# oceanbase/oceanbase

Hardware: AMD Instinct MI355X
Metric: rows/sec, TPC-H lineitem scan->filter->agg (microblock decode + pushdown filter + group-by) (higher is better)
Workload: dtype int64; 1 GPU; tpch_q1_sf100_lineitem_scan_filter_agg; rows_per_gpu=600000000, total_rows=600000000, encoded_bytes_per_gpu=7341603792, n_blocks=453858, block_bytes=16384

## Files before the change

### include/obx.h

```cpp
#ifndef OBX_H_
#define OBX_H_

#include <stdint.h>
#include <stddef.h>

#ifdef __cplusplus
extern "C" {
#endif

enum {
  OBX_SUCCESS = 0,
  OBX_ITER_END = -4008,
  OBX_INVALID_ARGUMENT = -4002,
  OBX_NOT_SUPPORTED = -4007,
  OBX_BUF_NOT_ENOUGH = -4009,
  OBX_NO_GPU = -7001,
  OBX_INTERNAL_ERROR = -4016,
  OBX_PHYSIC_CHECKSUM_ERROR = -4108,
};

enum obx_encoding {
  OBX_ENC_RAW = 0,
  OBX_ENC_DICT = 1,
  OBX_ENC_RLE = 2,
  OBX_ENC_CONST = 3,
  OBX_ENC_INTEGER_BASE_DIFF = 4,
  OBX_ENC_STRING_DIFF = 5,
  OBX_ENC_HEX_PACKING = 6,
  OBX_ENC_STRING_PREFIX = 7,
  OBX_ENC_COLUMN_EQUAL = 8,
  OBX_ENC_COLUMN_SUBSTR = 9,
  OBX_ENC_MAX = 10,
  OBX_ENC_AUTO = 255,
};

enum obx_obj_type {
  OBX_T_INT = 5,
  OBX_T_INT32 = 4,
  OBX_T_DATE = 19,
  OBX_T_CHAR = 23,
  OBX_T_DECIMAL_INT = 50,
};

enum obx_white_op {
  OBX_OP_EQ = 0,
  OBX_OP_LE = 1,
  OBX_OP_LT = 2,
  OBX_OP_GE = 3,
  OBX_OP_GT = 4,
  OBX_OP_NE = 5,
  OBX_OP_BT = 6,
  OBX_OP_IN = 7,
  OBX_OP_NU = 8,
  OBX_OP_NN = 9,
  OBX_OP_BLACK = 10,
  OBX_OP_IN_SET = 11,
};

#define OBX_BX_MAX_PROG 24
#define OBX_BX_MAX_CONST 4
#define OBX_BX_MAX_COLS 4

enum obx_agg_kind {
  OBX_AGG_COUNT = 0,
  OBX_AGG_SUM = 1,
  OBX_AGG_MIN = 2,
  OBX_AGG_MAX = 3,
  OBX_AGG_SUM_PROD2 = 4,
  OBX_AGG_SUM_PROD3 = 5,
  OBX_AGG_SUM_MUL = 6,
};

typedef struct obx_col_schema {
  uint8_t obj_type;
  int8_t scale;
  uint8_t precision;
  uint8_t len;
} obx_col_schema;

typedef struct obx_blockset {
  const uint8_t *data;
  const uint64_t *block_offsets;
  uint32_t n_blocks;
  uint16_t n_cols;
  const obx_col_schema *cols;
  uint64_t total_rows;
} obx_blockset;

#define OBX_MAX_IN_LIST 8
typedef struct obx_filter_leaf {
  uint16_t col;
  uint8_t op;
  uint8_t n_in;
  int64_t lo;
  int64_t hi;
  int64_t in_list[OBX_MAX_IN_LIST];
  int64_t bconst[OBX_BX_MAX_CONST];
  uint16_t bcols[OBX_BX_MAX_COLS];
  uint8_t n_bprog;
  uint8_t n_bcols;
  uint8_t bprog[OBX_BX_MAX_PROG];
  uint8_t bpad[6];
} obx_filter_leaf;

#define OBX_TOK_AND 128
#define OBX_TOK_OR 129
#define OBX_MAX_PROG 15

typedef struct obx_filter_desc {
  uint16_t n_leaves;
  uint8_t n_prog;
  uint8_t prog[OBX_MAX_PROG];
  obx_filter_leaf leaves[8];
} obx_filter_desc;

typedef struct obx_agg_expr {
  uint8_t kind;
  uint16_t col_a;
  uint16_t col_b;
  uint16_t col_c;
} obx_agg_expr;

typedef struct obx_agg_desc {
  uint8_t n_group_cols;
  uint16_t group_cols[2];
  uint8_t n_aggs;
  obx_agg_expr aggs[8];
} obx_agg_desc;

typedef struct obx_agg_cell { uint64_t limb[4]; } obx_agg_cell;

#define OBX_MAX_GROUPS 64
#define OBX_MAX_KEY_BYTES 16
typedef struct obx_group_row {
  uint8_t key[OBX_MAX_KEY_BYTES];
  uint8_t key_len;
  uint64_t row_count;
  obx_agg_cell cells[8];
} obx_group_row;

typedef struct obx_agg_result {
  uint32_t n_groups;
  obx_group_row groups[OBX_MAX_GROUPS];
  uint64_t rows_scanned;
  uint64_t rows_passed;
} obx_agg_result;

typedef struct obx_batch {
  uint64_t *skip_bits;
  int64_t size;
  uint8_t end;
  uint8_t all_rows_active;
} obx_batch;


int64_t obx_encode_block(const obx_col_schema *cols, uint16_t n_cols,
                         const uint8_t *const *col_data,
                         const uint8_t *const *null_bitmaps,
                         uint32_t row_count, const uint8_t *enc_request,
                         uint8_t *out, int64_t out_cap);

uint64_t obx_crc32c(const uint8_t *buf, int64_t len);

int obx_decode_block(const obx_col_schema *cols, uint16_t n_cols,
                     const uint8_t *block, int64_t block_len,
                     const uint16_t *proj_cols, uint16_t n_proj,
                     uint8_t *const *out_cols, uint8_t *const *out_nulls,
                     uint32_t *row_count);

int obx_cpu_filter_block(const obx_col_schema *cols, uint16_t n_cols,
                         const uint8_t *block, int64_t block_len,
                         const obx_filter_desc *filter,
                         uint8_t *result_bits, uint32_t *row_count,
                         uint32_t *popcnt);

int obx_cpu_scan_filter_agg(const obx_blockset *bs,
                            const obx_filter_desc *filter,
                            const obx_agg_desc *agg,
                            int nthreads,
                            obx_agg_result *out);

int64_t obx_gen_lineitem(int config, uint64_t row_count, uint64_t seed,
                         uint32_t target_block_bytes,
                         uint64_t row_id_base,
                         uint8_t **out_data, uint64_t **out_offsets,
                         obx_col_schema *out_cols, uint16_t *out_n_cols);

typedef struct obx_gpu_ctx obx_gpu_ctx;

int obx_gpu_open(int device, obx_gpu_ctx **ctx);
int obx_gpu_close(obx_gpu_ctx *ctx);

int obx_gpu_load_blocks(obx_gpu_ctx *ctx, const obx_blockset *bs);

int obx_gpu_load_cs_blocks(obx_gpu_ctx *ctx, const obx_blockset *bs);

int obx_cs_host_parse(const uint8_t *buf, int64_t len, uint32_t *rows_out,
                      uint32_t *ncols_out);
int obx_gpu_free_blocks(obx_gpu_ctx *ctx, int handle);

int obx_gpu_filter(obx_gpu_ctx *ctx, int handle, const obx_filter_desc *filter,
                   int want_row_ids);
int obx_gpu_fetch_bitmap(obx_gpu_ctx *ctx, int handle, uint8_t *out, int64_t cap);
int obx_gpu_fetch_row_ids(obx_gpu_ctx *ctx, int handle, int32_t *out,
                          int64_t cap, uint64_t *n_out);
int obx_gpu_fetch_blk_counts(obx_gpu_ctx *ctx, int handle, uint32_t *out,
                             int64_t cap);

int obx_gpu_decode(obx_gpu_ctx *ctx, int handle, const uint16_t *proj_cols,
                   uint16_t n_proj);
int obx_gpu_fetch_col(obx_gpu_ctx *ctx, int handle, uint16_t col,
                      uint8_t *out, int64_t cap);

int obx_gpu_scan_project(obx_gpu_ctx *ctx, int handle,
                         const obx_filter_desc *filter,
                         const uint16_t *proj_cols, uint16_t n_proj,
                         int want_row_nos, uint64_t *n_rows);

int obx_gpu_fetch_proj(obx_gpu_ctx *ctx, int handle, uint16_t proj_idx,
                       uint64_t start, uint64_t count,
                       uint8_t *out, int64_t cap,
                       uint8_t *out_nulls, int64_t nulls_cap, uint64_t *n_out);

int obx_gpu_fetch_proj_row_nos(obx_gpu_ctx *ctx, int handle, uint64_t start,
                               uint64_t count, uint64_t *out, int64_t cap,
                               uint64_t *n_out);

double obx_gpu_last_proj_stage_ms(obx_gpu_ctx *ctx, int stage);

int obx_gpu_scan_filter_agg(obx_gpu_ctx *ctx, int handle,
                            const obx_filter_desc *filter,
                            const obx_agg_desc *agg,
                            obx_agg_result *out);

double obx_gpu_last_kernel_ms(obx_gpu_ctx *ctx);
double obx_gpu_last_prep_ms(obx_gpu_ctx *ctx);
int obx_gpu_last_jit(obx_gpu_ctx *ctx);
int obx_gpu_last_bdesc(obx_gpu_ctx *ctx);
int64_t obx_gpu_bdesc_builds(obx_gpu_ctx *ctx, int handle);
uint32_t obx_gpu_last_grid(obx_gpu_ctx *ctx);
uint64_t obx_gpu_total_rows(obx_gpu_ctx *ctx, int handle);
uint64_t obx_gpu_total_bytes(obx_gpu_ctx *ctx, int handle);
uint64_t obx_gpu_last_survivors(obx_gpu_ctx *ctx, int handle);

int obx_gpu_agg_fetch(obx_gpu_ctx *ctx, int handle, uint32_t start,
                      uint32_t count, obx_group_row *out, uint32_t *n_out,
                      uint64_t *n_total);
int obx_cpu_agg_fetch(uint32_t start, uint32_t count, obx_group_row *out,
                      uint32_t *n_out, uint64_t *n_total);

typedef struct obx_keyset_info {
  uint64_t n_keys_in;
  uint64_t n_distinct;
  uint64_t slots_or_bits;
  uint64_t bytes;
  int64_t min, max;
  uint8_t kind;
} obx_keyset_info;

int obx_gpu_keyset_create(obx_gpu_ctx *ctx, const int64_t *keys, uint64_t n,
                          int kind);
int obx_gpu_keyset_from_proj(obx_gpu_ctx *ctx, int handle, uint16_t proj_idx,
                             int kind);
int obx_gpu_keyset_free(obx_gpu_ctx *ctx, int set_id);
int obx_gpu_keyset_info(obx_gpu_ctx *ctx, int set_id, obx_keyset_info *out);
int obx_gpu_keyset_host_model(const int64_t *keys, uint64_t n, int kind,
                              const int64_t *probe, uint64_t m, uint8_t *hit,
                              obx_keyset_info *info);

#define OBX_COL_JOINED 0xFFF0u
typedef struct obx_keymap_info {
  uint64_t n_keys;
  uint64_t slots_or_span;
  uint64_t bytes;
  int64_t min, max;
  uint8_t kind;
  uint8_t payload_len, payload_type;
} obx_keymap_info;

int obx_gpu_keymap_create(obx_gpu_ctx *ctx, const int64_t *keys,
                          const uint8_t *payloads, uint64_t n,
                          const obx_col_schema *payload, int kind);
int obx_gpu_keymap_from_proj(obx_gpu_ctx *ctx, int handle, uint16_t key_idx,
                             uint16_t payload_idx, int kind);
int obx_gpu_keymap_free(obx_gpu_ctx *ctx, int map_id);
int obx_gpu_keymap_info(obx_gpu_ctx *ctx, int map_id, obx_keymap_info *out);
int obx_gpu_keymap_host_model(const int64_t *keys, const uint8_t *payloads,
                              uint64_t n, const obx_col_schema *payload,
                              int kind, const int64_t *probe, uint64_t m,
                              uint8_t *hit, uint64_t *out_payload,
                              obx_keymap_info *info);

typedef struct obx_join_desc { int32_t map_id; uint16_t probe_col; uint16_t pad; } obx_join_desc;
int obx_gpu_scan_join_agg(obx_gpu_ctx *ctx, int handle,
                          const obx_filter_desc *filter,
                          const obx_join_desc *join, const obx_agg_desc *agg,
                          obx_agg_result *out);

int64_t obx_jit_dump_src(const obx_filter_desc *filter,
                         const obx_agg_desc *agg,
                         const obx_col_schema *cols, uint16_t n_cols,
                         const uint8_t *col_flags, const int64_t *col_min,
                         const int64_t *col_max, const uint32_t *col_maxcnt,
                         const uint32_t *col_maxw, uint32_t max_block_rows,
                         int force_v1, char *out, int64_t cap);

#ifdef __cplusplus
}
#endif
#endif
```

### oceanbase_amd/csrc/obx_engine.cpp

```cpp
#include <cstdlib>
#include <cstring>
#include <algorithm>

#include "obx_host.h"

#define OBX_RESULT_BYTES(slots) (sizeof(gslot) * (slots) + 16 * 8)

extern "C" int obx_gpu_open(int device, obx_gpu_ctx **out) {
  int n = 0;
  hipError_t e = hipGetDeviceCount(&n);
  if (e != hipSuccess || n <= device) return OBX_NO_GPU;
  auto *ctx = new obx_gpu_ctx();
  ctx->device = device;
  HIP_TRY(hipSetDevice(device));
  HIP_TRY(hipStreamCreate(&ctx->stream));
  HIP_TRY(hipEventCreate(&ctx->ev_start));
  HIP_TRY(hipEventCreate(&ctx->ev_stop));
  HIP_TRY(hipEventCreate(&ctx->ev_p0));
  HIP_TRY(hipEventCreate(&ctx->ev_p1));
  HIP_TRY(hipEventCreate(&ctx->ev_mid));
  HIP_TRY(hipEventCreate(&ctx->ev_b0));
  HIP_TRY(hipEventCreate(&ctx->ev_b1));
  {
    hipDeviceProp_t prop;
    HIP_TRY(hipGetDeviceProperties(&prop, device));
    if (prop.multiProcessorCount > 0)
      ctx->n_cus = (uint32_t)prop.multiProcessorCount;
  }
  HIP_TRY(hipHostMalloc((void **)&ctx->h_result,
                        OBX_RESULT_BYTES(OBX_GTABLE_BIG), hipHostMallocDefault));
  *out = ctx;
  return OBX_SUCCESS;
}

extern "C" int obx_gpu_close(obx_gpu_ctx *ctx) {
  if (!ctx) return OBX_SUCCESS;
  (void)hipSetDevice(ctx->device);
  ctx->handles.clear();
  ctx->keysets.clear();
  ctx->keymaps.clear();
  (void)hipStreamDestroy(ctx->stream);
  for (hipEvent_t ev : {ctx->ev_start, ctx->ev_stop, ctx->ev_p0, ctx->ev_p1,
                        ctx->ev_mid, ctx->ev_b0, ctx->ev_b1})
    (void)hipEventDestroy(ev);
  (void)hipHostFree(ctx->h_result);
  delete ctx;
  return OBX_SUCCESS;
}

obx_handle::~obx_handle() {
  void *owned[] = {d_buf, d_blocks, d_bleaves, d_pleaves, d_gtable,
                   d_gtable_big, d_proj_scratch, d_bitmap, d_row_ids,
                   d_blk_counts, d_row_slot, d_minmax, d_sel_nulls,
                   d_sel_row_nos, d_blk_off, d_tile_sums, d_sel_bits};
  for (void *p : owned)
    if (p) (void)hipFree(p);
  for (uint8_t *p : d_decode_out)
    if (p) (void)hipFree(p);
  for (uint8_t *p : d_sel_out)
    if (p) (void)hipFree(p);
  for (bdesc_set &s : bdesc)
    if (s.d) (void)hipFree(s.d);
}

obx_handle *obx_handle_lookup(obx_gpu_ctx *ctx, int handle) {
  if (!ctx || handle < 0 || handle >= (int)ctx->handles.size()) return nullptr;
  return ctx->handles[handle].get();
}

__attribute__((target("sse4.2")))
static uint64_t host_crc32c(const uint8_t *buf, int64_t len) {
  uint64_t crc = 0;
  int64_t i = 0;
  for (; i + 8 <= len; i += 8) {
    uint64_t w;
    memcpy(&w, buf + i, 8);
    crc = __builtin_ia32_crc32di(crc, w);
  }
  for (; i < len; i++) crc = __builtin_ia32_crc32qi((uint32_t)crc, buf[i]);
  return crc;
}

#define OBX_JIT_GRID_WAVES 8
static uint32_t jit_grid_for(uint32_t n_blocks, uint32_t n_cus, int wpb) {
  uint64_t g = (uint64_t)(n_cus ? n_cus : 1) * (uint32_t)(wpb > 0 ? wpb : 1) *
               OBX_JIT_GRID_WAVES;
  if (const char *sg = getenv("OBX_JIT_SGRID")) {
    const long v = atol(sg);
    if (v >= 1 && (uint64_t)v < g) g = (uint64_t)v;
  }
  if (g > n_blocks) g = n_blocks;
  return g ? (uint32_t)g : 1;
}

static void gtable_init(gslot *gt, uint32_t n_slots, uint32_t tail_words,
                        uint32_t min_mask, uint32_t max_mask,
                        hipStream_t stream) {
  const uint32_t words =
      n_slots * (uint32_t)(sizeof(gslot) / 8) + tail_words;
  hipLaunchKernelGGL(k_gtable_init, dim3((words + OBX_WG_HOST - 1) / OBX_WG_HOST),
                     dim3(OBX_WG_HOST), 0, stream, (unsigned long long *)gt,
                     n_slots, tail_words, min_mask, max_mask);
}

static void summarize_col_classes(obx_handle &h) {
  const uint32_t nc = h.n_cols;
  const bool first = h.col_class.size() == nc;
  const uint8_t *cls = h.col_class.data() + h.col_class.size() - nc;
  const uint8_t *cnt = h.col_cnt.data() + h.col_cnt.size() - nc;
  for (uint32_t c = 0; c < nc; c++) {
    const uint8_t k = cls[c];
    if (first) h.col_grp16_every[c] = true;
    if ((k & 0xF) == 5) h.col_span_any[c] = true;
    if ((k & 0xF) != 1 || cnt[c] >= 16) h.col_grp16_every[c] = false;
    if ((k & 0xF) > 3 || (k & 0x10)) h.col_slow_any[c] = true;
    if (cnt[c] > h.col_cnt_max[c]) h.col_cnt_max[c] = cnt[c];
  }
}

void obx_fold_block(obx_handle &h, const dev_block &db) {
  const bool first = h.col_class.empty();
  if ((db.block_byte & 15) ||
      (uint64_t)db.block_len + 24 > OBX_LDS_STAGE_BYTES ||
      db.row_count > 4096 )
    h.lds_ok = false;
  for (uint16_t c = 0; c < h.n_cols; c++) {
    const dev_col &dc = db.cols[c];
    uint8_t cls;
    switch (dc.enc) {
      case OBX_D_RAW: cls = 0; break;
      case OBX_D_DICT: cls = 1; break;
      case OBX_D_INTDIFF: cls = 2; break;
      case OBX_D_CONST: cls = dc.runs == 0 ? 3 : 4; break;
      case OBX_D_EQUAL: case OBX_D_SUBSTR:
        cls = 5; break;
      default: cls = 4; break;
    }
    if (dc.flags & OBX_DF_STRING) cls |= 0x10;
    h.col_class.push_back(cls);
    h.col_cnt.push_back((uint8_t)(dc.count > 254 ? 255 : dc.count));
    if (first) {
      h.col_dict_every[c] = true;
      h.col_dict_any[c] = true;
      h.col_raw8_every[c] = true;
      h.col_rangefam_every[c] = true;
    }
    if ((cls & 0xF) != 1 || (cls & 0x10) || dc.count > 63)
      h.col_dict_every[c] = false;
    if ((cls & 0xF) != 1 || dc.count > 63)
      h.col_dict_any[c] = false;
    if (!(dc.enc == OBX_D_RAW && !(dc.flags & OBX_DF_BITPACK) &&
          !(dc.flags & OBX_DF_STRING) && !(dc.flags & OBX_DF_HAS_EXT) &&
          dc.width == 8 && (dc.data_bit & 63) == 0))
      h.col_raw8_every[c] = false;
    if (!((dc.enc == OBX_D_RAW || dc.enc == OBX_D_INTDIFF) &&
          !(dc.flags & OBX_DF_STRING) && !(dc.flags & OBX_DF_HAS_EXT)))
      h.col_rangefam_every[c] = false;
    if (dc.count > h.col_maxcnt[c]) h.col_maxcnt[c] = dc.count;
    if (dc.flags & OBX_DF_HAS_EXT) h.col_ext_any[c] = true;
    uint32_t w = 255;
    if (dc.enc == OBX_D_RAW || dc.enc == OBX_D_DICT || dc.enc == OBX_D_INTDIFF)
      w = (dc.flags & OBX_DF_BITPACK) ? dc.width : (uint32_t)dc.width * 8;
    if (w > h.col_maxw[c]) h.col_maxw[c] = w;
    uint64_t slot;
    if (!obx_bdesc_pack_col(&dc, db.block_byte, &slot))
      h.col_bdesc_unfit[c] = true;
  }
  summarize_col_classes(h);
  if (db.row_count > h.max_block_rows) h.max_block_rows = db.row_count;
  if (db.block_len > h.max_block_len) h.max_block_len = db.block_len;
  h.n_blocks++;
  h.total_rows += db.row_count;
}

static int parse_block(const obx_col_schema *cols, uint16_t n_cols,
                       const uint8_t *block, uint64_t dev_off,
                       uint64_t block_len, uint64_t row_start,
                       dev_block *out) {
  const obx_micro_header *h = (const obx_micro_header *)block;
  if (h->magic != OBX_MICRO_BLOCK_MAGIC) return OBX_INVALID_ARGUMENT;
  if (h->column_count != n_cols) return OBX_INVALID_ARGUMENT;
  if (h->data_zlength > (int64_t)block_len ||
      h->data_zlength < OBX_MICRO_HEADER_SIZE)
    return OBX_INVALID_ARGUMENT;
  if ((int64_t)host_crc32c(block + OBX_MICRO_HEADER_SIZE,
                           (int64_t)h->data_zlength - OBX_MICRO_HEADER_SIZE) !=
      h->data_checksum)
    return OBX_PHYSIC_CHECKSUM_ERROR;
  memset(out, 0, sizeof(*out));
  out->row_start_lo = (uint32_t)row_start;
  out->row_start_hi = (uint32_t)(row_start >> 32);
  out->row_count = h->row_count;
  out->block_len = (uint32_t)block_len;
  out->block_byte = dev_off;
  const uint64_t meta_base =
      dev_off + h->header_size + (uint64_t)n_cols * sizeof(obx_col_header);
  const obx_col_header *chp =
      (const obx_col_header *)(block + h->header_size);
  const uint8_t *meta_host = block + h->header_size +
                             (uint64_t)n_cols * sizeof(obx_col_header);
  const uint8_t evb = obx_hdr_extend_value_bit(h);

  for (uint16_t c = 0; c < n_cols; c++) {
    const obx_col_header *ch = &chp[c];
    dev_col *dc = &out->cols[c];
    const int sc = obx_store_class(ch->obj_type);
    const int64_t tss = obx_type_store_size(ch->obj_type);
    dc->enc = (uint8_t)ch->type;
    dc->datum_len = cols[c].len;
    dc->tss = (uint8_t)(tss > 0 ? tss : cols[c].len);
    dc->ext_width = evb;
    if (sc == OBX_SC_INT) dc->flags |= OBX_DF_SIGNED;
    if (sc == OBX_SC_STRING) dc->flags |= OBX_DF_STRING;
    const uint64_t col_base = meta_base + ch->offset;
    const uint8_t *col_host = meta_host + ch->offset;
    const int has_ext = (ch->attr & OBX_COL_ATTR_HAS_EXTEND_VALUE) ? 1 : 0;
    const int bp = (ch->attr & OBX_COL_ATTR_BIT_PACKING) ? 1 : 0;

    switch (ch->type) {
      case OBX_COL_RAW: {
        if (bp) dc->flags |= OBX_DF_BITPACK;
        dc->width = (uint8_t)ch->length;
        uint64_t ext_bits = has_ext ? (uint64_t)evb * h->row_count : 0;
        if (has_ext) {
          dc->flags |= OBX_DF_HAS_EXT;
          dc->ext_bit = col_base * 8;
        }
        if (bp) {
          dc->data_bit = col_base * 8 + ext_bits;
        } else {
          dc->data_bit = (col_base + (ext_bits + 7) / 8) * 8;
        }
        break;
      }
      case OBX_COL_DICT: {
        const obx_dict_meta *dm = (const obx_dict_meta *)col_host;
        if (bp) dc->flags |= OBX_DF_BITPACK;
        dc->width = dm->row_ref_size;
        dc->count = dm->count;
        dc->entry_len = (uint8_t)dm->data_size;
        dc->dict_byte = col_base + sizeof(obx_dict_meta);
        dc->data_bit = (col_base + ch->length) * 8;
        break;
      }
      case OBX_COL_RLE: {
        const obx_rle_meta *rm = (const obx_rle_meta *)col_host;
        dc->runs = rm->count;
        dc->rib = rm->attr & 7;
        dc->rfb = (rm->attr >> 3) & 7;
        dc->aux_byte = col_base + sizeof(obx_rle_meta);
        const obx_dict_meta *dm =
            (const obx_dict_meta *)(col_host + rm->offset);
        dc->count = dm->count;
        dc->entry_len = (uint8_t)dm->data_size;
        dc->dict_byte = col_base + rm->offset + sizeof(obx_dict_meta);
        break;
      }
      case OBX_COL_CONST: {
        const obx_const_meta *cm = (const obx_const_meta *)col_host;
        dc->runs = cm->count;
        dc->rib = cm->attr & 7;
        dc->rfb = cm->const_ref;
        if (cm->count == 0) {
          if (cm->const_ref > 0) {
            dc->count = 0;
          } else {
            dc->count = 1;
            int64_t cell = (sc == OBX_SC_INT) ? tss : cols[c].len;
            uint64_t v = 0;
            memcpy(&v, col_host + cm->offset, (size_t)cell);
            dc->base = (sc == OBX_SC_INT)
                           ? (int64_t)obx_sign_extend(v, tss, 1)
                           : (sc == OBX_SC_DECIMAL
                                  ? (int64_t)obx_sign_extend(v, cell, 1)
                                  : (int64_t)v);
          }
        } else {
          dc->aux_byte = col_base + sizeof(obx_const_meta);
          const obx_dict_meta *dm =
              (const obx_dict_meta *)(col_host + cm->offset);
          dc->count = dm->count;
          dc->entry_len = (uint8_t)dm->data_size;
          dc->dict_byte = col_base + cm->offset + sizeof(obx_dict_meta);
        }
        break;
      }
      case OBX_COL_INTEGER_BASE_DIFF: {
        const obx_intdiff_meta *im = (const obx_intdiff_meta *)col_host;
        if (bp) dc->flags |= OBX_DF_BITPACK;
        dc->width = im->length;
        uint64_t b = 0;
        memcpy(&b, col_host + sizeof(obx_intdiff_meta), (size_t)tss);
        dc->base = (int64_t)obx_sign_extend(b, tss, sc == OBX_SC_INT);
        uint64_t data0 = col_base + ch->length;
        uint64_t ext_bits = has_ext ? (uint64_t)evb * h->row_count : 0;
        if (has_ext) {
          dc->flags |= OBX_DF_HAS_EXT;
          dc->ext_bit = data0 * 8;
        }
        if (bp) dc->data_bit = data0 * 8 + ext_bits;
        else dc->data_bit = (data0 + (ext_bits + 7) / 8) * 8;
        break;
      }
      case OBX_COL_STRING_PREFIX: {
        const obx_sprefix_meta *pm = (const obx_sprefix_meta *)col_host;
        dc->count = pm->count;
        dc->entry_len = pm->hex_char_cnt;
        dc->rib = pm->pib;
        dc->dict_byte = col_base + sizeof(obx_sprefix_meta);
        dc->aux_byte = dc->dict_byte + pm->hex_char_cnt;
        {
          const uint8_t *ends = col_host + sizeof(obx_sprefix_meta) +
                                pm->hex_char_cnt;
          uint64_t prev = 0, min_pl = ~0ull;
          for (uint32_t j = 0; j < pm->count; j++) {
            uint64_t e2 = 0;
            memcpy(&e2, ends + (size_t)j * pm->pib, pm->pib);
            if (e2 - prev < min_pl) min_pl = e2 - prev;
            prev = e2;
          }
          uint32_t max_suffix = pm->string_size - (uint32_t)min_pl;
          dc->width = (uint8_t)(1 + (pm->hex_char_cnt
                                         ? (max_suffix + 1) / 2
                                         : max_suffix));
        }
        uint64_t data0 = col_base + ch->length;
        uint64_t ext_bits = has_ext ? (uint64_t)evb * h->row_count : 0;
        if (has_ext) {
          dc->flags |= OBX_DF_HAS_EXT;
          dc->ext_bit = data0 * 8;
        }
        dc->data_bit = (data0 + (ext_bits + 7) / 8) * 8;
        break;
      }
      case OBX_COL_SUBSTR: {
        const obx_substr_meta *sm3 = (const obx_substr_meta *)col_host;
        if (sm3->ref_col >= n_cols) return OBX_INVALID_ARGUMENT;
        dc->runs = sm3->exc_cnt;
        dc->rib = sm3->rib;
        dc->width = (uint8_t)sm3->ref_col;
        dc->base = sm3->start_pos;
        dc->dict_byte = col_base + sizeof(obx_substr_meta);
        dc->aux_byte = dc->dict_byte + (uint64_t)sm3->exc_cnt * sm3->rib;
        break;
      }
      case OBX_COL_EQUAL: {
        const obx_coleq_meta *em = (const obx_coleq_meta *)col_host;
        if (em->ref_col >= n_cols) return OBX_INVALID_ARGUMENT;
        dc->runs = em->exc_cnt;
        dc->rib = em->rib;
        dc->width = (uint8_t)em->ref_col;
        dc->dict_byte = col_base + sizeof(obx_coleq_meta);
        dc->aux_byte = dc->dict_byte + (uint64_t)em->exc_cnt * em->rib;
        break;
      }
      case OBX_COL_HEX_PACKING: {
        const obx_hex_meta *hm = (const obx_hex_meta *)col_host;
        dc->width = (uint8_t)((hm->string_size + 1) / 2);
        dc->count = hm->char_cnt;
        dc->dict_byte = col_base + sizeof(obx_hex_meta);
        uint64_t data0 = col_base + ch->length;
        uint64_t ext_bits = has_ext ? (uint64_t)evb * h->row_count : 0;
        if (has_ext) {
          dc->flags |= OBX_DF_HAS_EXT;
          dc->ext_bit = data0 * 8;
        }
        dc->data_bit = (data0 + (ext_bits + 7) / 8) * 8;
        break;
      }
      case OBX_COL_STRING_DIFF: {
        const obx_sdiff_meta *sm = (const obx_sdiff_meta *)col_host;
        dc->runs = sm->diff_desc_cnt;
        dc->entry_len = sm->hex_char_cnt;
        dc->dict_byte = col_base + sizeof(obx_sdiff_meta);
        const uint8_t *descs = col_host + sizeof(obx_sdiff_meta);
        uint32_t diff_len = 0;
        for (uint32_t i = 0; i < sm->diff_desc_cnt; i++)
          if (descs[i] & 1) diff_len += descs[i] >> 1;
        dc->rib = (uint8_t)diff_len;
        dc->width = (uint8_t)(sm->hex_char_cnt ? (diff_len + 1) / 2
                                               : diff_len);
        dc->aux_byte = dc->dict_byte + sm->diff_desc_cnt +
                       sm->hex_char_cnt;
        uint64_t data0 = col_base + ch->length;
        uint64_t ext_bits = has_ext ? (uint64_t)evb * h->row_count : 0;
        if (has_ext) {
          dc->flags |= OBX_DF_HAS_EXT;
          dc->ext_bit = data0 * 8;
        }
        dc->data_bit = (data0 + (ext_bits + 7) / 8) * 8;
        break;
      }
      default:
        return OBX_NOT_SUPPORTED;
    }
// ... 521 lines not shown
      ln[i] = (uint8_t)h.cols[c].len;
      po[i] = h.d_decode_out[c];
    }
    if (!h.d_proj_scratch)
      HIP_TRY(hipMalloc(&h.d_proj_scratch,
                        OBX_DEV_MAX_COLS * (8 + 2 + 1) + 16));
    uint8_t *base = (uint8_t *)h.d_proj_scratch;
    uint8_t *outp = base;
    uint8_t *pcp = base + OBX_DEV_MAX_COLS * 8;
    uint8_t *lnp = pcp + OBX_DEV_MAX_COLS * 2;
    HIP_TRY(hipMemcpy(outp, po, sizeof(void *) * n_proj,
                      hipMemcpyHostToDevice));
    HIP_TRY(hipMemcpy(pcp, pc, sizeof(uint16_t) * n_proj,
                      hipMemcpyHostToDevice));
    HIP_TRY(hipMemcpy(lnp, ln, n_proj, hipMemcpyHostToDevice));
    hipLaunchKernelGGL(k_decode_multi, dim3(grid_for(h.n_blocks)),
                       dim3(OBX_WG_HOST), 0, ctx->stream, h.d_buf,
                       h.d_blocks, h.n_blocks, (const uint16_t *)pcp,
                       lnp, (uint32_t)n_proj, (uint8_t *const *)outp,
                       (uint8_t *const *)nullptr);
  } else {
    for (uint16_t i = 0; i < n_proj; i++) {
      uint16_t c = proj_cols[i];
      if (c >= h.n_cols) return OBX_INVALID_ARGUMENT;
      if (!h.d_decode_out[c])
        HIP_TRY(hipMalloc(&h.d_decode_out[c], h.total_rows * h.cols[c].len));
      auto kfn = h.lds_ok ? k_decode_lds : k_decode;
      hipLaunchKernelGGL(kfn, dim3(grid_for(h.n_blocks)), dim3(OBX_WG_HOST), 0,
                         ctx->stream, h.d_buf, h.d_blocks, h.n_blocks,
                         (uint32_t)c, (uint32_t)h.cols[c].len,
                         h.d_decode_out[c], (uint8_t *)nullptr);
    }
  }
  return end_timed(ctx, false);
}

extern "C" int obx_gpu_fetch_col(obx_gpu_ctx *ctx, int handle, uint16_t col,
                                 uint8_t *out, int64_t cap) {
  obx_handle *hp = obx_handle_lookup(ctx, handle);
  if (!hp) return OBX_INVALID_ARGUMENT;
  obx_handle &h = *hp;
  if (col >= h.n_cols || !h.d_decode_out[col]) return OBX_INVALID_ARGUMENT;
  int64_t bytes = (int64_t)h.total_rows * h.cols[col].len;
  if (cap < bytes) return OBX_BUF_NOT_ENOUGH;
  HIP_TRY(hipMemcpy(out, h.d_decode_out[col], bytes, hipMemcpyDeviceToHost));
  return OBX_SUCCESS;
}

template <class T>
static int grow(T *&p, uint64_t &cap, uint64_t need, size_t unit) {
  if (need <= cap) return OBX_SUCCESS;
  (void)hipFree(p);
  p = nullptr;
  cap = 0;
  HIP_TRY(hipMalloc(&p, need * unit));
  cap = need;
  return OBX_SUCCESS;
}

extern "C" int obx_gpu_scan_project(obx_gpu_ctx *ctx, int handle,
                                    const obx_filter_desc *filter,
                                    const uint16_t *proj_cols, uint16_t n_proj,
                                    int want_row_nos, uint64_t *n_rows) {
  obx_handle *hp = obx_handle_lookup(ctx, handle);
  if (!hp) return OBX_INVALID_ARGUMENT;
  obx_handle &h = *hp;
  h.sel_n_proj = 0;
  if (!proj_cols || n_proj == 0 || n_proj > OBX_DEV_MAX_COLS)
    return OBX_INVALID_ARGUMENT;
  for (uint16_t i = 0; i < n_proj; i++)
    if (proj_cols[i] >= h.n_cols) return OBX_INVALID_ARGUMENT;
  HIP_TRY(hipSetDevice(ctx->device));

  const bool filtered = filter && filter->n_leaves;
  uint64_t total = h.total_rows;
  ctx->last_proj_ms[0] = ctx->last_proj_ms[1] = ctx->last_proj_ms[2] = 0.0;
  if (filtered) {
    int rc = run_filter(ctx, h, filter, 1);
    if (rc != OBX_SUCCESS) return rc;
    ctx->last_proj_ms[0] = ctx->last_ms;
    total = h.last_survivors;
  } else {
    ctx->last_jit = 0;
  }

  if (total > 0) {
    proj_args pa;
    memset(&pa, 0, sizeof(pa));
    pa.n_proj = n_proj;
    for (uint16_t i = 0; i < n_proj; i++) {
      const uint16_t c = proj_cols[i];
      int rc = grow(h.d_sel_out[i], h.sel_out_cap[i], total * h.cols[c].len, 1);
      if (rc != OBX_SUCCESS) return rc;
      pa.out[i] = h.d_sel_out[i];
      pa.col[i] = c;
      pa.len[i] = h.cols[c].len;
    }
    int rc = grow(h.d_sel_nulls, h.sel_nulls_cap, total, 1);
    if (rc != OBX_SUCCESS) return rc;
    if (want_row_nos) {
      rc = grow(h.d_sel_row_nos, h.sel_row_nos_cap, total, sizeof(uint64_t));
      if (rc != OBX_SUCCESS) return rc;
    }
    const uint32_t n_tiles = (h.n_blocks + OBX_PROJ_TILE - 1) / OBX_PROJ_TILE;
    if (filtered && !h.d_blk_off) {
      HIP_TRY(hipMalloc(&h.d_blk_off, ((uint64_t)h.n_blocks + 1) * 8));
      HIP_TRY(hipMalloc(&h.d_tile_sums, (uint64_t)n_tiles * 8));
    }

    HIP_TRY(hipEventRecord(ctx->ev_start, ctx->stream));
    if (filtered) {
      hipLaunchKernelGGL(k_project_tile_sums, dim3(n_tiles), dim3(OBX_WG_HOST),
                         0, ctx->stream, h.d_blk_counts, h.n_blocks,
                         h.d_tile_sums);
      hipLaunchKernelGGL(k_project_offsets, dim3(n_tiles), dim3(OBX_WG_HOST),
                         0, ctx->stream, h.d_blk_counts, h.n_blocks,
                         h.d_tile_sums, h.d_blk_off);
    }
    HIP_TRY(hipEventRecord(ctx->ev_mid, ctx->stream));
    hipLaunchKernelGGL(h.lds_ok ? k_project_sel_lds : k_project_sel,
                       dim3(grid_for(h.n_blocks)), dim3(OBX_WG_HOST), 0,
                       ctx->stream, h.d_buf, h.d_blocks, h.n_blocks,
                       filtered ? h.d_row_ids : (const int32_t *)nullptr,
                       filtered ? h.d_blk_counts : (const uint32_t *)nullptr,
                       filtered ? h.d_blk_off : (const uint64_t *)nullptr, pa,
                       h.d_sel_nulls,
                       want_row_nos ? h.d_sel_row_nos : (uint64_t *)nullptr,
                       total);
    rc = end_timed(ctx, false);
    if (rc != OBX_SUCCESS) return rc;
    float ms = 0;
    HIP_TRY(hipEventElapsedTime(&ms, ctx->ev_start, ctx->ev_mid));
    ctx->last_proj_ms[1] = ms;
    HIP_TRY(hipEventElapsedTime(&ms, ctx->ev_mid, ctx->ev_stop));
    ctx->last_proj_ms[2] = ms;
  }
  ctx->last_ms = ctx->last_proj_ms[0] + ctx->last_proj_ms[1] +
                 ctx->last_proj_ms[2];

  memcpy(h.sel_cols, proj_cols, sizeof(uint16_t) * n_proj);
  h.sel_has_row_nos = want_row_nos != 0;
  h.sel_rows = total;
  h.sel_n_proj = n_proj;
  if (n_rows) *n_rows = total;
  return OBX_SUCCESS;
}

static uint64_t sel_window(const obx_handle &h, uint64_t start,
                           uint64_t count) {
  if (start >= h.sel_rows) return 0;
  return count < h.sel_rows - start ? count : h.sel_rows - start;
}

extern "C" int obx_gpu_fetch_proj(obx_gpu_ctx *ctx, int handle,
                                  uint16_t proj_idx, uint64_t start,
                                  uint64_t count, uint8_t *out, int64_t cap,
                                  uint8_t *out_nulls, int64_t nulls_cap,
                                  uint64_t *n_out) {
  obx_handle *hp = obx_handle_lookup(ctx, handle);
  if (!hp) return OBX_INVALID_ARGUMENT;
  obx_handle &h = *hp;
  if (proj_idx >= h.sel_n_proj) return OBX_INVALID_ARGUMENT;
  const uint64_t n = sel_window(h, start, count);
  if (n_out) *n_out = n;
  if (n == 0) return OBX_SUCCESS;
  const uint64_t len = h.cols[h.sel_cols[proj_idx]].len;
  const uint64_t null_bytes = (n + 7) / 8;
  if (out && (cap < 0 || (uint64_t)cap < n * len)) return OBX_BUF_NOT_ENOUGH;
  if (out_nulls && (nulls_cap < 0 || (uint64_t)nulls_cap < null_bytes))
    return OBX_BUF_NOT_ENOUGH;
  HIP_TRY(hipSetDevice(ctx->device));
  if (out)
    HIP_TRY(hipMemcpyAsync(out, h.d_sel_out[proj_idx] + start * len, n * len,
                           hipMemcpyDeviceToHost, ctx->stream));
  if (out_nulls) {
    int rc = grow(h.d_sel_bits, h.sel_bits_cap, null_bytes, 1);
    if (rc != OBX_SUCCESS) return rc;
    uint64_t g = (null_bytes + OBX_WG_HOST - 1) / OBX_WG_HOST;
    if (g > 4096) g = 4096;
    hipLaunchKernelGGL(k_project_pack_nulls, dim3((uint32_t)g),
                       dim3(OBX_WG_HOST), 0, ctx->stream, h.d_sel_nulls,
                       start, n, (uint32_t)proj_idx, h.d_sel_bits);
    HIP_TRY(hipMemcpyAsync(out_nulls, h.d_sel_bits, null_bytes,
                           hipMemcpyDeviceToHost, ctx->stream));
  }
  HIP_TRY(hipStreamSynchronize(ctx->stream));
  return OBX_SUCCESS;
}

extern "C" int obx_gpu_fetch_proj_row_nos(obx_gpu_ctx *ctx, int handle,
                                          uint64_t start, uint64_t count,
                                          uint64_t *out, int64_t cap,
                                          uint64_t *n_out) {
  obx_handle *hp = obx_handle_lookup(ctx, handle);
  if (!hp) return OBX_INVALID_ARGUMENT;
  obx_handle &h = *hp;
  if (!h.sel_n_proj || !h.sel_has_row_nos) return OBX_INVALID_ARGUMENT;
  const uint64_t n = sel_window(h, start, count);
  if (n_out) *n_out = n;
  if (n == 0 || !out) return OBX_SUCCESS;
  if (cap < 0 || (uint64_t)cap < n) return OBX_BUF_NOT_ENOUGH;
  HIP_TRY(hipSetDevice(ctx->device));
  HIP_TRY(hipMemcpyAsync(out, h.d_sel_row_nos + start, n * sizeof(uint64_t),
                         hipMemcpyDeviceToHost, ctx->stream));
  HIP_TRY(hipStreamSynchronize(ctx->stream));
  return OBX_SUCCESS;
}

extern "C" double obx_gpu_last_proj_stage_ms(obx_gpu_ctx *ctx, int stage) {
  return ctx && stage >= 0 && stage < 3 ? ctx->last_proj_ms[stage] : -1.0;
}

static int table_to_rows(obx_handle &h, const gslot *gt, size_t n_gt,
                         const unsigned long long *cnt, uint8_t key_len,
                         const obx_agg_desc *agg, obx_agg_result *out) {
  unsigned long long passed = cnt[0];
  for (int i2 = 8; i2 < 16; i2++) passed += cnt[i2];

  memset(out, 0, sizeof(*out));
  out->rows_scanned = h.total_rows;
  out->rows_passed = passed;
  std::vector<const gslot *> live;
  for (size_t i = 0; i < n_gt; i++)
    if (gt[i].key != OBX_KEY_EMPTY) live.push_back(&gt[i]);
  std::sort(live.begin(), live.end(), [](const gslot *a, const gslot *b) {
    uint8_t ka[8], kb[8];
    memcpy(ka, &a->key, 8);
    memcpy(kb, &b->key, 8);
    return memcmp(ka, kb, 8) < 0;
  });
  h.last_rows.assign(live.size(), obx_group_row());
  for (size_t i = 0; i < live.size(); i++) {
    obx_group_row *g = &h.last_rows[i];
    memcpy(g->key, &live[i]->key, 8);
    g->key_len = key_len;
    g->row_count = live[i]->count;
    uint32_t na = agg ? agg->n_aggs : 0;
    for (uint32_t a = 0; a < na; a++) {
      uint8_t kind = agg->aggs[a].kind;
      if (kind == OBX_AGG_COUNT && agg->aggs[a].col_a == UINT16_MAX) {
        g->cells[a].limb[0] = live[i]->count;
        g->cells[a].limb[1] = g->cells[a].limb[2] = g->cells[a].limb[3] = 0;
      } else if (kind == OBX_AGG_MIN || kind == OBX_AGG_MAX) {
        int64_t v = live[i]->cells[a][1] ? (int64_t)live[i]->cells[a][0] : 0;
        g->cells[a].limb[0] = (uint64_t)v;
        uint64_t s = v < 0 ? ~0ull : 0ull;
        g->cells[a].limb[1] = g->cells[a].limb[2] = g->cells[a].limb[3] = s;
      } else {
        for (int l = 0; l < 4; l++)
          g->cells[a].limb[l] = live[i]->cells[a][l];
      }
    }
  }
  if (h.last_rows.size() > OBX_MAX_GROUPS) {
    out->n_groups = (uint32_t)h.last_rows.size();
    return OBX_BUF_NOT_ENOUGH;
  }
  out->n_groups = (uint32_t)h.last_rows.size();
  for (size_t i = 0; i < h.last_rows.size(); i++)
    out->groups[i] = h.last_rows[i];
  return OBX_SUCCESS;
}

template <class LAUNCH>
static int rerun_direct(obx_gpu_ctx *ctx, obx_handle &h,
                        const dev_plan_hdr &ph, uint32_t min_mask,
                        uint32_t max_mask, size_t *n_gt,
                        unsigned long long cnt[16], LAUNCH launch) {
  if (ph.n_prog != 0) return OBX_BUF_NOT_ENOUGH;
  if (!h.d_gtable_big)
    HIP_TRY(hipMalloc(&h.d_gtable_big, OBX_RESULT_BYTES(OBX_GTABLE_BIG)));
  unsigned long long *big_counters =
      (unsigned long long *)(h.d_gtable_big + OBX_GTABLE_BIG);
  gtable_init(h.d_gtable_big, OBX_GTABLE_BIG, 16, min_mask, max_mask,
              ctx->stream);
  launch(h.d_gtable_big, big_counters);
  HIP_TRY(hipMemcpyAsync(ctx->h_result, h.d_gtable_big,
                         OBX_RESULT_BYTES(OBX_GTABLE_BIG),
                         hipMemcpyDeviceToHost, ctx->stream));
  HIP_TRY(hipStreamSynchronize(ctx->stream));
  *n_gt = OBX_GTABLE_BIG;
  memcpy(cnt, (const gslot *)ctx->h_result + OBX_GTABLE_BIG,
         16 * sizeof(cnt[0]));
  if (cnt[2] != 0) return OBX_BUF_NOT_ENOUGH;
  return OBX_SUCCESS;
}


struct minmax_masks { uint32_t min = 0, max = 0; };
template <class KIND_OF>
static minmax_masks agg_minmax_masks(uint32_t n_aggs, KIND_OF kind_of) {
  minmax_masks m;
  for (uint32_t a = 0; a < n_aggs; a++) {
    if (kind_of(a) == OBX_AGG_MIN) m.min |= 1u << a;
    else if (kind_of(a) == OBX_AGG_MAX) m.max |= 1u << a;
  }
  return m;
}

static void reset_last_scan(obx_gpu_ctx *ctx) {
  ctx->last_jit = 0;
  ctx->last_grid = 0;
  ctx->last_bdesc = 0;
  ctx->bdesc_built = false;
}

template <class LAUNCH>
static int finish_agg_scan(obx_gpu_ctx *ctx, obx_handle &h,
                           const dev_plan_hdr &ph, minmax_masks mm,
                           uint8_t key_len, const obx_agg_desc *agg,
                           obx_agg_result *out, LAUNCH launch_direct) {
  int rc = end_timed(ctx, true, h.d_gtable,
                     OBX_RESULT_BYTES(OBX_GTABLE_SLOTS));
  if (rc != OBX_SUCCESS) return rc;
  const gslot *gt = (const gslot *)ctx->h_result;
  size_t n_gt = OBX_GTABLE_SLOTS;
  unsigned long long cnt[16];
  memcpy(cnt, gt + OBX_GTABLE_SLOTS, sizeof(cnt));
  if (cnt[1] != 0) {
    rc = rerun_direct(ctx, h, ph, mm.min, mm.max, &n_gt, cnt, launch_direct);
    if (rc != OBX_SUCCESS) return rc;
  }
  return table_to_rows(h, gt, n_gt, cnt, key_len, agg, out);
}

extern "C" int obx_gpu_scan_filter_agg(obx_gpu_ctx *ctx, int handle,
                                       const obx_filter_desc *filter,
                                       const obx_agg_desc *agg,
                                       obx_agg_result *out) {
  obx_handle *hp = obx_handle_lookup(ctx, handle);
  if (!hp || !out) return OBX_INVALID_ARGUMENT;
  obx_handle &h = *hp;
  HIP_TRY(hipSetDevice(ctx->device));
  h.last_rows.clear();
  dev_plan_hdr ph;
  dev_leaf plv[OBX_DEV_MAX_LEAVES];
  int rc = prep_query(ctx, h, filter, agg, ph, plv);
  if (rc != OBX_SUCCESS) return rc;
  reset_last_scan(ctx);

  const minmax_masks mm = agg_minmax_masks(
      ph.n_aggs, [&](uint32_t a) { return ph.aggs[a].kind; });
  gtable_init(h.d_gtable, OBX_GTABLE_SLOTS, 16, mm.min, mm.max, ctx->stream);

  const bool use_pipeline = getenv("OBX_PIPELINE_AGG") != nullptr;
  if (use_pipeline) {
    uint64_t bm_words = (h.total_rows + 63) / 64 + 1;
    if (!h.d_bitmap) HIP_TRY(hipMalloc(&h.d_bitmap, bm_words * 8));
    HIP_TRY(hipMemsetAsync(h.d_bitmap, 0, bm_words * 8, ctx->stream));
    if (!h.d_row_slot) HIP_TRY(hipMalloc(&h.d_row_slot, h.total_rows + 1));

    HIP_TRY(hipEventRecord(ctx->ev_start, ctx->stream));
    hipLaunchKernelGGL(generic_filter_kernel(h, ph),
                       dim3(grid_for(h.n_blocks)), dim3(OBX_WG_HOST), 0,
                       ctx->stream, h.d_buf, h.d_blocks, h.n_blocks,
                       h.d_pleaves, h.d_bleaves, ph, h.d_bitmap,
                       (int32_t *)nullptr, (uint32_t *)nullptr, h.d_counters);
    hipLaunchKernelGGL(k_group_pass, dim3(grid_for(h.n_blocks)),
                       dim3(OBX_WG_HOST), 0, ctx->stream, h.d_buf, h.d_blocks,
                       h.n_blocks, ph, h.d_bitmap, h.d_row_slot, h.d_gtable,
                       h.d_counters);
    for (uint32_t a = 0; a < ph.n_aggs;) {
      const dev_agg &ag = ph.aggs[a];
      if (ag.kind == OBX_AGG_COUNT && ag.ia == 0xFF) { a++; continue; }
      const bool fuse = obx_fuse_p3(ph.aggs, ph.n_aggs, a);
      hipLaunchKernelGGL(k_agg_pass, dim3(grid_for(h.n_blocks)),
                         dim3(OBX_WG_HOST), 0, ctx->stream, h.d_buf,
                         h.d_blocks, h.n_blocks, ph, a, h.d_bitmap,
                         h.d_row_slot, h.d_gtable);
      a += fuse ? 2 : 1;
    }
  } else {
    jit_entry *je = jit_prepare(h, ph, plv);
    ctx->last_jit = je ? g_jit_kind : 0;
    const obx_bdesc *bd = nullptr;
    if (je && je->bdesc) {
      HIP_TRY(hipEventRecord(ctx->ev_b0, ctx->stream));
      bd = bdesc_get(h, je->bd_cols, ctx->stream, &ctx->bdesc_built);
      if (!bd) return OBX_INTERNAL_ERROR;
      HIP_TRY(hipEventRecord(ctx->ev_b1, ctx->stream));
    }
    ctx->last_bdesc = bd != nullptr;
    HIP_TRY(hipEventRecord(ctx->ev_start, ctx->stream));
    if (je) {
      if (jit_launch(je, h, bd, ctx->stream, &ctx->last_grid) != 0)
        return OBX_INTERNAL_ERROR;
    } else {
      auto kfn = h.lds_ok
                     ? (ph.n_prog ? k_scan_filter_agg_prog_lds
                                  : k_scan_filter_agg_lds)
                     : (ph.n_prog ? k_scan_filter_agg_prog : k_scan_filter_agg);
      hipLaunchKernelGGL(kfn, dim3(grid_for(h.n_blocks)), dim3(OBX_WG_HOST), 0,
                         ctx->stream, h.d_buf, h.d_blocks, h.n_blocks,
                         h.d_pleaves, h.d_bleaves, ph, h.d_gtable,
                         h.d_counters);
    }
  }
  uint8_t key_len = 0;
  if (agg)
    for (int g = 0; g < agg->n_group_cols; g++)
      key_len += h.cols[agg->group_cols[g]].len;
  return finish_agg_scan(
      ctx, h, ph, mm, key_len, agg, out,
      [&](gslot *big, unsigned long long *big_counters) {
        hipLaunchKernelGGL(k_scan_agg_direct, dim3(grid_for(h.n_blocks)),
                           dim3(OBX_WG_HOST), 0, ctx->stream, h.d_buf,
                           h.d_blocks, h.n_blocks, h.d_pleaves, h.d_bleaves,
                           ph, big, big_counters);
      });
}

extern "C" int obx_gpu_scan_join_agg(obx_gpu_ctx *ctx, int handle,
                                     const obx_filter_desc *filter,
                                     const obx_join_desc *join,
                                     const obx_agg_desc *agg,
                                     obx_agg_result *out) {
  obx_handle *hp = obx_handle_lookup(ctx, handle);
  if (!hp || !out || !join) return OBX_INVALID_ARGUMENT;
  obx_handle &h = *hp;
  h.last_rows.clear();
  const obx_keymap *km = obx_keymap_lookup(ctx, join->map_id);
  if (!km || join->probe_col >= h.n_cols) return OBX_INVALID_ARGUMENT;
  const uint8_t probe_len = h.cols[join->probe_col].len;
  if (probe_len == 0 || probe_len > 8) return OBX_NOT_SUPPORTED;

  dev_join dj;
  memset(&dj, 0, sizeof(dj));
  dj.km = km->view;
  dj.pay_len = km->info.payload_len;
  obx_agg_desc plan, eff;
  memset(&plan, 0, sizeof(plan));
  memset(&eff, 0, sizeof(eff));
  uint8_t key_len = 0;
  if (agg) {
    if (agg->n_group_cols > 2 || agg->n_aggs > OBX_DEV_MAX_AGGS)
      return OBX_INVALID_ARGUMENT;
    eff = *agg;
    for (int g = 0; g < agg->n_group_cols; g++) {
      if (agg->group_cols[g] == OBX_COL_JOINED) {
        if (dj.pay_group) return OBX_INVALID_ARGUMENT;
        dj.pay_group = 1;
        dj.pay_pos = (uint8_t)g;
        key_len += dj.pay_len;
      } else {
        if (agg->group_cols[g] >= h.n_cols) return OBX_INVALID_ARGUMENT;
        plan.group_cols[plan.n_group_cols++] = agg->group_cols[g];
        key_len += h.cols[agg->group_cols[g]].len;
      }
    }
    if (dj.pay_group) {
      dj.real_len = plan.n_group_cols ? h.cols[plan.group_cols[0]].len : 0;
      if (dj.pay_len + dj.real_len > 7) return OBX_NOT_SUPPORTED;
    }
    plan.n_aggs = agg->n_aggs;
    for (int a = 0; a < agg->n_aggs; a++) {
      const obx_agg_expr &e = agg->aggs[a];
      plan.aggs[a] = e;
      const bool prod = e.kind == OBX_AGG_SUM_PROD2 ||
                        e.kind == OBX_AGG_SUM_PROD3 ||
                        e.kind == OBX_AGG_SUM_MUL;
      if (e.col_b == OBX_COL_JOINED || e.col_c == OBX_COL_JOINED)
        return OBX_INVALID_ARGUMENT;
      if (e.col_a != OBX_COL_JOINED) continue;
      if (prod || e.kind > OBX_AGG_SUM_MUL) return OBX_INVALID_ARGUMENT;
      plan.aggs[a].kind = OBX_AGG_COUNT;
      plan.aggs[a].col_a = UINT16_MAX;
      if (e.kind == OBX_AGG_COUNT) {
        eff.aggs[a].col_a = UINT16_MAX;
      } else {
        dj.own_mask |= (uint8_t)(1u << a);
      }
    }
  }

  HIP_TRY(hipSetDevice(ctx->device));
  dev_plan_hdr ph;
  int rc = prep_query(ctx, h, filter, &plan, ph);
  if (rc != OBX_SUCCESS) return rc;
  uint32_t pi = 0;
  while (pi < ph.n_need && ph.need_cols[pi] != join->probe_col) pi++;
  if (pi == ph.n_need) {
    if (ph.n_need >= OBX_DEV_MAX_NEED) return OBX_NOT_SUPPORTED;
    ph.need_cols[ph.n_need++] = join->probe_col;
  }
  dj.probe_idx = (uint8_t)pi;
  for (uint32_t a = 0; a < ph.n_aggs; a++)
    dj.kind[a] = ((dj.own_mask >> a) & 1) ? agg->aggs[a].kind : ph.aggs[a].kind;
  reset_last_scan(ctx);

  const minmax_masks mm = agg_minmax_masks(
      ph.n_aggs, [&](uint32_t a) { return dj.kind[a]; });
  gtable_init(h.d_gtable, OBX_GTABLE_SLOTS, 16, mm.min, mm.max, ctx->stream);
  HIP_TRY(hipEventRecord(ctx->ev_start, ctx->stream));
  auto kfn = h.lds_ok
                 ? (ph.n_prog ? k_scan_join_agg_prog_lds : k_scan_join_agg_lds)
                 : (ph.n_prog ? k_scan_join_agg_prog : k_scan_join_agg);
  hipLaunchKernelGGL(kfn, dim3(grid_for(h.n_blocks)), dim3(OBX_WG_HOST), 0,
                     ctx->stream, h.d_buf, h.d_blocks, h.n_blocks, h.d_pleaves,
                     h.d_bleaves, ph, dj, h.d_gtable, h.d_counters);
  return finish_agg_scan(
      ctx, h, ph, mm, key_len, agg ? &eff : nullptr, out,
      [&](gslot *big, unsigned long long *big_counters) {
        hipLaunchKernelGGL(k_scan_join_agg_direct, dim3(grid_for(h.n_blocks)),
                           dim3(OBX_WG_HOST), 0, ctx->stream, h.d_buf,
                           h.d_blocks, h.n_blocks, h.d_pleaves, h.d_bleaves,
                           ph, dj, big, big_counters);
      });
}

extern "C" uint64_t obx_crc32c(const uint8_t *buf, int64_t len) {
  return host_crc32c(buf, len);
}

extern "C" int64_t obx_jit_dump_src_ex(
    const obx_filter_desc *filter, const obx_agg_desc *agg,
    const obx_col_schema *cols, uint16_t n_cols, const uint8_t *col_flags,
    const int64_t *col_min, const int64_t *col_max,
    const uint32_t *col_maxcnt, const uint32_t *col_maxw,
    uint32_t max_block_rows, int force_v1, uint32_t n_blocks, uint32_t n_cus,
    uint32_t *grid_out, char *out, int64_t cap) {
  if (!cols || n_cols > OBX_DEV_MAX_COLS) return OBX_INVALID_ARGUMENT;
  if (grid_out) *grid_out = 0;
  for (uint16_t i = 0; filter && i < filter->n_leaves && i < 8; i++)
    if (filter->leaves[i].op == OBX_OP_IN_SET) return 0;
  obx_handle h;
  h.n_cols = n_cols;
  h.n_blocks = n_blocks ? n_blocks : 1;
  if (n_cus) h.n_cus = n_cus;
  h.max_block_rows = max_block_rows ? max_block_rows : 4096;
  h.max_block_len = OBX_LDS_STAGE_BYTES - 32;
  memcpy(h.cols, cols, sizeof(obx_col_schema) * n_cols);
  for (uint16_t c = 0; c < n_cols; c++) {
    h.col_dict_every[c] = (col_flags[c] & 1) != 0;
    h.col_ext_any[c] = (col_flags[c] & 2) != 0;
    h.col_known[c] = (col_flags[c] & 4) != 0;
    h.col_raw8_every[c] = (col_flags[c] & 8) != 0;
    h.col_rangefam_every[c] = (col_flags[c] & 16) != 0;
    h.col_dict_any[c] = h.col_dict_every[c] ||
        (obx_store_class(cols[c].obj_type) == OBX_SC_STRING &&
         (col_flags[c] & 1));
    h.col_dict_stable[c] = (col_flags[c] & 32) != 0 && h.col_dict_any[c];
    h.col_min[c] = col_min[c];
    h.col_max[c] = col_max[c];
    h.col_maxcnt[c] = col_maxcnt[c];
    h.col_maxw[c] = col_maxw ? col_maxw[c] : 255;
    h.col_bdesc_unfit[c] = col_maxcnt[c] > 0xFFFFu;
    uint8_t cls = h.col_dict_every[c] ? 1 : 0;
    if (obx_store_class(cols[c].obj_type) == OBX_SC_STRING) cls |= 0x10;
    h.col_class.push_back(cls);
    h.col_cnt.push_back(
        (uint8_t)(h.col_maxcnt[c] > 254 ? 255 : h.col_maxcnt[c]));
  }
  summarize_col_classes(h);
  dev_plan_hdr ph;
  dev_leaf pl[OBX_DEV_MAX_LEAVES];
  int rc = build_plan(nullptr, h, filter, agg, ph, pl);
  if (rc != OBX_SUCCESS) return rc;
  if (!agg) {
    jit_fstrategy fst;
    if (!jit_build_fstrategy(h, ph, pl, fst)) return 0;
    if (getenv("OBX_DUMP_RID") && fst.fstage) {
      fst.frid = 1;
      fst.fnch = (uint16_t)((h.max_block_rows + 63) / 64);
    }
    std::string fsrc = jit_gen_source_filter(ph, fst);
    if (out && cap > (int64_t)fsrc.size()) {
      memcpy(out, fsrc.data(), fsrc.size());
      out[fsrc.size()] = 0;
    }
    return (int64_t)fsrc.size();
  }
  jit_scan_choice c;
  if (!jit_scan_choose(h, ph, pl, force_v1 != 0, c)) return 0;
  if (c.kind == 2 && grid_out)
    *grid_out = jit_grid_for(h.n_blocks, h.n_cus, c.st.wpb);
  std::string src = jit_scan_source(ph, c);
  if (out && cap > (int64_t)src.size()) {
    memcpy(out, src.data(), src.size());
    out[src.size()] = 0;
  }
  return (int64_t)src.size();
}

extern "C" int64_t obx_jit_dump_src(
    const obx_filter_desc *filter, const obx_agg_desc *agg,
    const obx_col_schema *cols, uint16_t n_cols, const uint8_t *col_flags,
    const int64_t *col_min, const int64_t *col_max,
    const uint32_t *col_maxcnt, const uint32_t *col_maxw,
    uint32_t max_block_rows, int force_v1,
    char *out, int64_t cap) {
  return obx_jit_dump_src_ex(filter, agg, cols, n_cols, col_flags, col_min,
                             col_max, col_maxcnt, col_maxw, max_block_rows,
                             force_v1, 1, 0, nullptr, out, cap);
}

extern "C" int obx_jit_probe_blocks(
    const obx_filter_desc *filter, const obx_agg_desc *agg,
    const obx_col_schema *cols, uint16_t n_cols, const uint8_t *col_class,
    const uint8_t *col_cnt, uint32_t n_blocks) {
  if (!cols || !col_class || !col_cnt || n_cols > OBX_DEV_MAX_COLS)
    return OBX_INVALID_ARGUMENT;
  obx_handle h;
  h.n_cols = n_cols;
  h.n_blocks = n_blocks;
  memcpy(h.cols, cols, sizeof(obx_col_schema) * n_cols);
  for (size_t b = 0; b < n_blocks; b++) {
    h.col_class.insert(h.col_class.end(), col_class + b * n_cols,
                       col_class + (b + 1) * n_cols);
    h.col_cnt.insert(h.col_cnt.end(), col_cnt + b * n_cols,
                     col_cnt + (b + 1) * n_cols);
    summarize_col_classes(h);
  }
  dev_plan_hdr ph;
  dev_leaf pl[OBX_DEV_MAX_LEAVES];
  int rc = build_plan(nullptr, h, filter, agg, ph, pl);
  if (rc != OBX_SUCCESS) return rc;
  jit_shape js;
  return jit_plan_shape(ph, js) && jit_blocks_ok(h, ph, js) ? 1 : 0;
}

extern "C" int obx_probe_load_facts(const obx_blockset *bs, int is_cs,
                                    uint64_t *handle_out, uint32_t *col_out) {
  if (!bs || !handle_out || !col_out) return OBX_INVALID_ARGUMENT;
  obx_handle h;
  std::vector<dev_block> blocks;
  int rc = is_cs ? obx_cs_host_load(bs, h, blocks, nullptr)
                 : obx_pax_host_load(bs, h, blocks);
  if (rc != OBX_SUCCESS) return rc;
  const uint64_t hf[7] = {h.n_blocks, h.n_cols, h.total_rows, h.total_bytes,
                          h.lds_ok, h.max_block_rows, h.max_block_len};
  memcpy(handle_out, hf, sizeof(hf));
  for (uint16_t c = 0; c < h.n_cols; c++) {
    const bool f[10] = {h.col_dict_every[c], h.col_dict_any[c],
                        h.col_dict_stable[c], h.col_grp16_every[c],
                        h.col_raw8_every[c], h.col_rangefam_every[c],
                        h.col_ext_any[c], h.col_slow_any[c], h.col_span_any[c],
                        h.col_bdesc_unfit[c]};
    uint32_t *o = col_out + 4 * c;
    o[0] = 0;
    for (int i = 0; i < 10; i++) o[0] |= (uint32_t)f[i] << i;
    o[1] = h.col_maxcnt[c];
    o[2] = h.col_maxw[c];
    o[3] = h.col_cnt_max[c];
  }
  return OBX_SUCCESS;
}

extern "C" double obx_gpu_last_kernel_ms(obx_gpu_ctx *ctx) {
  return ctx ? ctx->last_ms : -1.0;
}

extern "C" double obx_gpu_last_prep_ms(obx_gpu_ctx *ctx) {
  return ctx ? ctx->last_prep_ms : -1.0;
}

extern "C" int obx_gpu_last_jit(obx_gpu_ctx *ctx) {
  return ctx ? ctx->last_jit : 0;
}

extern "C" int obx_gpu_last_bdesc(obx_gpu_ctx *ctx) {
  return ctx ? ctx->last_bdesc : 0;
}

extern "C" int64_t obx_gpu_bdesc_builds(obx_gpu_ctx *ctx, int handle) {
  obx_handle *h = obx_handle_lookup(ctx, handle);
  return h ? (int64_t)h->bdesc_builds : -1;
}

extern "C" int obx_bdesc_probe(const dev_block *blk, const uint16_t *cols,
                               uint32_t n_cols, obx_bdesc *out) {
  if (!blk || !cols || !out || n_cols > OBX_DEV_MAX_NEED)
    return OBX_INVALID_ARGUMENT;
  for (uint32_t i = 0; i < n_cols; i++)
    if (cols[i] >= OBX_DEV_MAX_COLS) return OBX_INVALID_ARGUMENT;
  return obx_bdesc_pack(blk, cols, n_cols, out);
}

extern "C" uint32_t obx_gpu_last_grid(obx_gpu_ctx *ctx) {
  return ctx ? ctx->last_grid : 0;
}

extern "C" uint64_t obx_gpu_total_rows(obx_gpu_ctx *ctx, int handle) {
  const obx_handle *h = obx_handle_lookup(ctx, handle);
  return h ? h->total_rows : 0;
}
extern "C" uint64_t obx_gpu_total_bytes(obx_gpu_ctx *ctx, int handle) {
  const obx_handle *h = obx_handle_lookup(ctx, handle);
  return h ? h->total_bytes : 0;
}
extern "C" uint64_t obx_gpu_last_survivors(obx_gpu_ctx *ctx, int handle) {
  const obx_handle *h = obx_handle_lookup(ctx, handle);
  return h ? h->last_survivors : 0;
}

extern "C" int obx_gpu_agg_fetch(obx_gpu_ctx *ctx, int handle,
                                 uint32_t start, uint32_t count,
                                 obx_group_row *out, uint32_t *n_out,
                                 uint64_t *n_total) {
  obx_handle *hp = obx_handle_lookup(ctx, handle);
  if (!hp || !out) return OBX_INVALID_ARGUMENT;
  obx_handle &h = *hp;
  uint64_t total = h.last_rows.size();
  if (n_total) *n_total = total;
  uint32_t n = 0;
  for (; n < count && start + n < total; n++) out[n] = h.last_rows[start + n];
  if (n_out) *n_out = n;
  return OBX_SUCCESS;
}
```

### oceanbase_amd/csrc/obx_host.h

```cpp
#ifndef OBX_HOST_H_
#define OBX_HOST_H_

#include <hip/hip_runtime.h>

#include <cstddef>
#include <cstdio>
#include <map>
#include <memory>
#include <vector>

#include "obx_dev.h"
#include "obx_keymap.h"
#include "obx_keyset.h"
#include "obx_project.h"

#define OBX_WG_HOST 256

#include "../../include/obx.h"
#include "../../oracle/obx_format.h"

extern "C" __global__ void k_decode_lds(
    const uint8_t *, const dev_block *, uint32_t, uint32_t, uint32_t,
    uint8_t *, uint8_t *);
extern "C" __global__ void k_decode_multi(
    const uint8_t *, const dev_block *, uint32_t, const uint16_t *,
    const uint8_t *, uint32_t, uint8_t *const *, uint8_t *const *);
extern "C" __global__ void k_scan_agg_direct(
    const uint8_t *, const dev_block *, uint32_t, const dev_leaf *,
    const blk_leaf *, const dev_plan_hdr, gslot *, unsigned long long *);
extern "C" __global__ void k_scan_filter_agg(
    const uint8_t *, const dev_block *, uint32_t, const dev_leaf *,
    const blk_leaf *, const dev_plan_hdr, gslot *, unsigned long long *);
extern "C" __global__ void k_scan_filter_agg_lds(
    const uint8_t *, const dev_block *, uint32_t, const dev_leaf *,
    const blk_leaf *, const dev_plan_hdr, gslot *, unsigned long long *);
extern "C" __global__ void k_filter(
    const uint8_t *, const dev_block *, uint32_t, const dev_leaf *,
    const blk_leaf *, const dev_plan_hdr, uint64_t *, int32_t *, uint32_t *,
    unsigned long long *);
extern "C" __global__ void k_filter_lds(
    const uint8_t *, const dev_block *, uint32_t, const dev_leaf *,
    const blk_leaf *, const dev_plan_hdr, uint64_t *, int32_t *, uint32_t *,
    unsigned long long *);
extern "C" __global__ void k_scan_filter_agg_prog(
    const uint8_t *, const dev_block *, uint32_t, const dev_leaf *,
    const blk_leaf *, const dev_plan_hdr, gslot *, unsigned long long *);
extern "C" __global__ void k_scan_filter_agg_prog_lds(
    const uint8_t *, const dev_block *, uint32_t, const dev_leaf *,
    const blk_leaf *, const dev_plan_hdr, gslot *, unsigned long long *);
extern "C" __global__ void k_filter_prog(
    const uint8_t *, const dev_block *, uint32_t, const dev_leaf *,
    const blk_leaf *, const dev_plan_hdr, uint64_t *, int32_t *, uint32_t *,
    unsigned long long *);
extern "C" __global__ void k_filter_prog_lds(
    const uint8_t *, const dev_block *, uint32_t, const dev_leaf *,
    const blk_leaf *, const dev_plan_hdr, uint64_t *, int32_t *, uint32_t *,
    unsigned long long *);
extern "C" __global__ void k_decode(
    const uint8_t *, const dev_block *, uint32_t, uint32_t, uint32_t,
    uint8_t *, uint8_t *);
extern "C" __global__ void k_group_pass(
    const uint8_t *, const dev_block *, uint32_t, const dev_plan_hdr,
    const uint64_t *, uint8_t *, gslot *, unsigned long long *);
extern "C" __global__ void k_agg_pass(
    const uint8_t *, const dev_block *, uint32_t, const dev_plan_hdr,
    uint32_t, const uint64_t *, const uint8_t *, gslot *);
extern "C" __global__ void k_lower_leaves(
    const uint8_t *, const dev_block *, uint32_t, const dev_leaf *, uint32_t,
    uint32_t, const int64_t *, blk_leaf *);
extern "C" __global__ void k_col_minmax(
    const uint8_t *, const dev_block *, uint32_t, uint32_t, int64_t *);
extern "C" __global__ void k_gtable_init(
    unsigned long long *, uint32_t, uint32_t, uint32_t, uint32_t);
extern "C" __global__ void k_pack_bdesc(const dev_block *, uint32_t,
                                        const obx_bdesc_cols, obx_bdesc *);
static_assert(sizeof(obx_bdesc) == 128 && alignof(obx_bdesc) == 128 &&
                  offsetof(obx_bdesc, slot) == 16,
              "k_pack_bdesc writes obx_bdesc as 16 u64 words");

extern "C" __global__ void k_project_tile_sums(const uint32_t *, uint32_t,
                                               uint64_t *);
extern "C" __global__ void k_project_offsets(const uint32_t *, uint32_t,
                                             const uint64_t *, uint64_t *);
extern "C" __global__ void k_project_sel(
    const uint8_t *, const dev_block *, uint32_t, const int32_t *,
    const uint32_t *, const uint64_t *, const proj_args, uint8_t *,
    uint64_t *, uint64_t);
extern "C" __global__ void k_project_sel_lds(
    const uint8_t *, const dev_block *, uint32_t, const int32_t *,
    const uint32_t *, const uint64_t *, const proj_args, uint8_t *,
    uint64_t *, uint64_t);
extern "C" __global__ void k_project_pack_nulls(const uint8_t *, uint64_t,
                                                uint64_t, uint32_t, uint8_t *);

extern "C" __global__ void k_keyset_minmax(
    const uint8_t *, uint32_t, uint32_t, const uint8_t *, uint32_t, uint64_t,
    unsigned long long *);
extern "C" __global__ void k_keyset_insert(
    const uint8_t *, uint32_t, uint32_t, const uint8_t *, uint32_t, uint64_t,
    uint64_t *, uint64_t, int64_t, uint32_t, uint32_t, unsigned long long *);

extern "C" __global__ void k_keymap_minmax(
    const uint8_t *, uint32_t, uint32_t, const uint8_t *, uint32_t, uint32_t,
    uint64_t, unsigned long long *);
extern "C" __global__ void k_keymap_insert(
    const uint8_t *, uint32_t, uint32_t, const uint8_t *, uint32_t, uint32_t,
    const uint8_t *, uint32_t, uint64_t, uint64_t *, uint64_t *, uint64_t,
    int64_t, uint32_t, uint32_t, unsigned long long *);

extern "C" __global__ void k_scan_join_agg(
    const uint8_t *, const dev_block *, uint32_t, const dev_leaf *,
    const blk_leaf *, const dev_plan_hdr, const dev_join, gslot *,
    unsigned long long *);
extern "C" __global__ void k_scan_join_agg_lds(
    const uint8_t *, const dev_block *, uint32_t, const dev_leaf *,
    const blk_leaf *, const dev_plan_hdr, const dev_join, gslot *,
    unsigned long long *);
extern "C" __global__ void k_scan_join_agg_prog(
    const uint8_t *, const dev_block *, uint32_t, const dev_leaf *,
    const blk_leaf *, const dev_plan_hdr, const dev_join, gslot *,
    unsigned long long *);
extern "C" __global__ void k_scan_join_agg_prog_lds(
    const uint8_t *, const dev_block *, uint32_t, const dev_leaf *,
    const blk_leaf *, const dev_plan_hdr, const dev_join, gslot *,
    unsigned long long *);
extern "C" __global__ void k_scan_join_agg_direct(
    const uint8_t *, const dev_block *, uint32_t, const dev_leaf *,
    const blk_leaf *, const dev_plan_hdr, const dev_join, gslot *,
    unsigned long long *);

#define HIP_TRY(x)                                        \
  do {                                                    \
    hipError_t _e = (x);                                  \
    if (_e != hipSuccess) {                               \
      fprintf(stderr, "obx: HIP error %s at %s:%d\n",     \
              hipGetErrorString(_e), __FILE__, __LINE__); \
      return OBX_INTERNAL_ERROR;                          \
    }                                                     \
  } while (0)

template <class T>
struct dev_tmp {
  T *p = nullptr;
  dev_tmp() = default;
  dev_tmp(const dev_tmp &) = delete;
  dev_tmp &operator=(const dev_tmp &) = delete;
  ~dev_tmp() { if (p) (void)hipFree(p); }
};

struct obx_handle {
  obx_handle() = default;
  obx_handle(const obx_handle &) = delete;
  obx_handle &operator=(const obx_handle &) = delete;
  ~obx_handle();

  uint8_t *d_buf = nullptr;
  dev_block *d_blocks = nullptr;
  uint32_t n_blocks = 0;
  uint16_t n_cols = 0;
  uint64_t total_rows = 0;
  uint64_t total_bytes = 0;
  obx_col_schema cols[OBX_DEV_MAX_COLS];
  blk_leaf *d_bleaves = nullptr;
  uint32_t bleaves_cap = 0;
  dev_leaf *d_pleaves = nullptr;
  gslot *d_gtable = nullptr;
  unsigned long long *d_counters = nullptr;
  uint64_t *d_bitmap = nullptr;
  int32_t *d_row_ids = nullptr;
  uint32_t *d_blk_counts = nullptr;
  uint8_t *d_row_slot = nullptr;
  uint8_t *d_decode_out[OBX_DEV_MAX_COLS] = {};
  uint64_t last_survivors = 0;
  gslot *d_gtable_big = nullptr;
  void *d_proj_scratch = nullptr;
  uint8_t *d_sel_out[OBX_DEV_MAX_COLS] = {};
  uint64_t sel_out_cap[OBX_DEV_MAX_COLS] = {};
  uint8_t *d_sel_nulls = nullptr;
  uint64_t *d_sel_row_nos = nullptr;
  uint64_t sel_nulls_cap = 0, sel_row_nos_cap = 0;
  uint64_t *d_blk_off = nullptr;
  uint64_t *d_tile_sums = nullptr;
  uint8_t *d_sel_bits = nullptr;
  uint64_t sel_bits_cap = 0;
  uint16_t sel_cols[OBX_DEV_MAX_COLS] = {};
  uint16_t sel_n_proj = 0;
  bool sel_has_row_nos = false;
  uint64_t sel_rows = 0;
  std::vector<obx_group_row> last_rows;
  uint32_t n_cus = 256;

  bool lds_ok = true;
  uint32_t max_block_rows = 0;
  uint32_t max_block_len = 0;
  std::vector<uint8_t> col_class, col_cnt;
  bool col_span_any[OBX_DEV_MAX_COLS] = {};
  bool col_grp16_every[OBX_DEV_MAX_COLS] = {};
  bool col_slow_any[OBX_DEV_MAX_COLS] = {};
  uint32_t col_cnt_max[OBX_DEV_MAX_COLS] = {};
  mutable std::map<uint32_t, uint32_t> pair_cells_max;
  bool col_dict_every[OBX_DEV_MAX_COLS] = {};
  bool col_dict_any[OBX_DEV_MAX_COLS] = {};
  bool col_dict_stable[OBX_DEV_MAX_COLS] = {};
  bool col_ext_any[OBX_DEV_MAX_COLS] = {};
  bool col_raw8_every[OBX_DEV_MAX_COLS] = {};
  bool col_rangefam_every[OBX_DEV_MAX_COLS] = {};
  uint32_t col_maxcnt[OBX_DEV_MAX_COLS] = {};
  uint32_t col_maxw[OBX_DEV_MAX_COLS] = {};
  bool col_bdesc_unfit[OBX_DEV_MAX_COLS] = {};

#define OBX_BDESC_SETS 4
  struct bdesc_set {
    obx_bdesc_cols cols = {};
    obx_bdesc *d = nullptr;
    uint64_t born = 0;
  } bdesc[OBX_BDESC_SETS];
  uint64_t bdesc_builds = 0;

  int64_t *d_minmax = nullptr;
  int64_t col_min[OBX_DEV_MAX_COLS] = {};
  int64_t col_max[OBX_DEV_MAX_COLS] = {};
  bool col_known[OBX_DEV_MAX_COLS] = {};
};

struct obx_keyset {
  obx_keyset() = default;
  obx_keyset(const obx_keyset &) = delete;
  obx_keyset &operator=(const obx_keyset &) = delete;
  ~obx_keyset() { if (d_words) (void)hipFree(d_words); }

  uint64_t *d_words = nullptr;
  obx_keyset_dev view = {};
  obx_keyset_info info = {};
};

struct obx_keymap {
  obx_keymap() = default;
  obx_keymap(const obx_keymap &) = delete;
  obx_keymap &operator=(const obx_keymap &) = delete;
  ~obx_keymap() { if (d_table) (void)hipFree(d_table); }

  uint64_t *d_table = nullptr;
  obx_keymap_dev view = {};
  obx_keymap_info info = {};
};

struct obx_gpu_ctx {
  int device = 0;
  hipStream_t stream = nullptr;
  hipEvent_t ev_start = nullptr, ev_stop = nullptr;
  hipEvent_t ev_p0 = nullptr, ev_p1 = nullptr;
  hipEvent_t ev_mid = nullptr;
  hipEvent_t ev_b0 = nullptr, ev_b1 = nullptr;
  bool bdesc_built = false;
  double last_ms = 0.0;
  double last_prep_ms = 0.0;
  int last_jit = 0;
  int last_bdesc = 0;
  double last_proj_ms[3] = {0.0, 0.0, 0.0};
  uint32_t last_grid = 0;
  uint32_t n_cus = 256;
  uint8_t *h_result = nullptr;
  std::vector<std::unique_ptr<obx_handle>> handles;
  std::vector<std::unique_ptr<obx_keyset>> keysets;
  std::vector<std::unique_ptr<obx_keymap>> keymaps;
};

const obx_keyset *obx_keyset_lookup(const obx_gpu_ctx *ctx, int64_t set_id);
const obx_keymap *obx_keymap_lookup(const obx_gpu_ctx *ctx, int64_t map_id);
obx_handle *obx_handle_lookup(obx_gpu_ctx *ctx, int handle);

static inline uint32_t grid_for(uint32_t n_blocks) {
  uint32_t g = n_blocks < 4096u ? n_blocks : 4096u;
  return g ? g : 1;
}


void obx_fold_block(obx_handle &h, const dev_block &db);

int obx_finish_load(obx_gpu_ctx *ctx, std::unique_ptr<obx_handle> h,
                    const std::vector<dev_block> &blocks);

int obx_pax_host_load(const obx_blockset *bs, obx_handle &h,
                      std::vector<dev_block> &blocks);
struct obx_cs_plan;
int obx_cs_host_load(const obx_blockset *bs, obx_handle &h,
                     std::vector<dev_block> &blocks,
                     obx_cs_plan *plan );

#endif
```

### oceanbase_amd/csrc/obx_jit.inc

```

#include <hip/hiprtc.h>

#include <cstdarg>
#include <map>
#include <string>

__attribute__((format(printf, 2, 0))) static void jit_vemit(std::string &s,
                                                            const char *fmt,
                                                            va_list ap) {
  va_list ap2;
  va_copy(ap2, ap);
  const int n = vsnprintf(nullptr, 0, fmt, ap2);
  va_end(ap2);
  if (n <= 0) return;
  const size_t at = s.size();
  s.resize(at + (size_t)n + 1);
  vsnprintf(&s[at], (size_t)n + 1, fmt, ap);
  s.resize(at + (size_t)n);
}

__attribute__((format(printf, 2, 3))) static void jit_emit(std::string &s,
                                                           const char *fmt,
                                                           ...) {
  va_list ap;
  va_start(ap, fmt);
  jit_vemit(s, fmt, ap);
  va_end(ap);
}

__attribute__((format(printf, 1, 2))) static std::string jit_fmt(
    const char *fmt, ...) {
  std::string s;
  va_list ap;
  va_start(ap, fmt);
  jit_vemit(s, fmt, ap);
  va_end(ap);
  return s;
}

struct jit_entry {
  hipModule_t mod = nullptr;
  hipFunction_t fn = nullptr;
  int wpb = 0;
  bool bdesc = false;
  obx_bdesc_cols bd_cols = {};
};

struct jit_shape {
  int n_vc = 0;
  uint8_t vcol[4] = {0xFF, 0xFF, 0xFF, 0xFF};
  int n_wa = 0;
  uint8_t agg_wa[OBX_DEV_MAX_AGGS];
  uint8_t agg_f2 = 0;
  bool has_mm = false;
  int slot(const dev_plan_hdr &ph, uint8_t need_idx) const {
    if (need_idx == 0xFF) return -1;
    for (int j = 0; j < n_vc; j++)
      if (vcol[j] == ph.need_cols[need_idx]) return j;
    return -1;
  }
};

enum { JL_NONE = 0, JL_RANGE = 1, JL_MASK = 2, JL_SET = 3 };
static uint8_t jit_leaf_kind(const obx_handle &h, const dev_leaf &lf) {
  const bool mask_ok = lf.op != OBX_OP_BLACK || lf.n_bcols == 1;
  if (h.col_dict_any[lf.col] && mask_ok) return JL_MASK;
  if (!h.col_rangefam_every[lf.col]) return JL_NONE;
  if (lf.op <= OBX_OP_BT) return JL_RANGE;
  return lf.op == OBX_OP_IN_SET ? JL_SET : JL_NONE;
}

struct jit_stream {
  std::string w, W, m, base, off;
  std::string field(bool packed) const {
    return packed ? jit_fmt("((%s >> (k * %s)) & %s)", w.c_str(), W.c_str(),
                            m.c_str())
                  : jit_fmt("jit_bread(%1$s, %2$s + r * %3$s, %3$s)",
                            base.c_str(), off.c_str(), W.c_str());
  }
};

struct jit_leaf_ops {
  int i;
  std::string mask, lo, hi, inv, none;
};

static void jit_emit_range_test(std::string &s, int pad,
                                const jit_leaf_ops &o,
                                const std::string &field, bool chain) {
  const std::string in(pad, ' ');
  if (chain)
    jit_emit(s,
             "%1$sif (live && !l%2$d_all) {\n"
             "%1$s  uint64_t v = %3$s ^ %4$s;\n"
             "%1$s  live = ((v - %5$s) <= (%6$s - %5$s)) != (bool)%7$s;\n"
             "%1$s}\n",
             in.c_str(), o.i, field.c_str(), o.mask.c_str(), o.lo.c_str(),
             o.hi.c_str(), o.inv.c_str());
  else
    jit_emit(s,
             "%1$suint64_t v%2$d = %3$s ^ %4$s;\n"
             "%1$sconst bool lf%2$d = !%8$s &&\n"
             "%1$s    (l%2$d_all || (((v%2$d - %5$s) <= (%6$s - %5$s)) != "
             "(bool)%7$s));\n",
             in.c_str(), o.i, field.c_str(), o.mask.c_str(), o.lo.c_str(),
             o.hi.c_str(), o.inv.c_str(), o.none.c_str());
}

static void jit_emit_mask_test(std::string &s, int pad, const jit_leaf_ops &o,
                               const std::string &field, bool chain) {
  const std::string in(pad, ' ');
  if (chain)
    jit_emit(s,
             "%1$sif (live)\n"
             "%1$s  live = (%2$s >>\n"
             "%1$s          (uint32_t)%3$s) & 1;\n",
             in.c_str(), o.mask.c_str(), field.c_str());
  else
    jit_emit(s,
             "%1$sconst bool lf%4$d = (%2$s >>\n"
             "%1$s    (uint32_t)%3$s) & 1;\n",
             in.c_str(), o.mask.c_str(), field.c_str(), o.i);
}

#include "obx_jit_scan_v1.inc"
#include "obx_jit_scan.inc"
#include "obx_jit_filter.inc"

static const char *OBX_JIT_SRC_DEV_H =
#include "obx_embed_dev_h.inc"
    ;
static const char *OBX_JIT_SRC_COMMON_H =
#include "obx_embed_common_h.inc"
    ;
static const char *OBX_JIT_SRC_JIT_DEV_H =
#include "obx_embed_jit_dev_h.inc"
    ;
static const char *OBX_JIT_SRC_KEYSET_H =
#include "obx_embed_keyset_h.inc"
    ;

static std::map<std::string, jit_entry> g_jit_cache;
static int g_jit_kind = 0;

static bool jit_plan_shape(const dev_plan_hdr &ph, jit_shape &js) {
  if (ph.n_prog || ph.n_aggs == 0) return false;
  auto vc_add = [&](uint8_t need_idx) -> bool {
    if (need_idx == 0xFF) return true;
    uint8_t col = ph.need_cols[need_idx];
    for (int j = 0; j < js.n_vc; j++)
      if (js.vcol[j] == col) return true;
    if (js.n_vc >= 4) return false;
    js.vcol[js.n_vc++] = col;
    return true;
  };
  for (uint32_t a = 0; a < ph.n_aggs; a++) {
    const dev_agg &g = ph.aggs[a];
    js.agg_wa[a] = 0xFF;
    if (g.kind == OBX_AGG_COUNT && g.ia == 0xFF) continue;
    if (g.kind == OBX_AGG_MIN || g.kind == OBX_AGG_MAX) {
      js.has_mm = true;
      if (!vc_add(g.ia)) return false;
      continue;
    }
    if (g.kind != OBX_AGG_COUNT && g.kind != OBX_AGG_SUM &&
        g.kind != OBX_AGG_SUM_PROD2 && g.kind != OBX_AGG_SUM_PROD3 &&
        g.kind != OBX_AGG_SUM_MUL)
      return false;
    bool f2 = (g.kind == OBX_AGG_SUM_PROD2 && a + 1 < ph.n_aggs &&
               ph.aggs[a + 1].kind == OBX_AGG_SUM_PROD3 &&
               ph.aggs[a + 1].ia == g.ia && ph.aggs[a + 1].ib == g.ib);
    js.agg_wa[a] = (uint8_t)js.n_wa;
    if (!vc_add(g.ia) || !vc_add(g.ib) ||
        !vc_add(f2 ? ph.aggs[a + 1].ic : g.ic))
      return false;
    if (f2) {
      js.agg_f2 |= (uint8_t)(1u << a);
      js.agg_wa[a + 1] = (uint8_t)(js.n_wa + 1);
      a++;
    }
    js.n_wa += f2 ? 2 : 1;
  }
  return js.n_wa <= 8;
}

static uint32_t jit_pair_cells_max(const obx_handle &h, uint8_t c0,
                                   uint8_t c1) {
  const uint32_t key = ((uint32_t)c0 << 16) | c1;
  auto it = h.pair_cells_max.find(key);
  if (it != h.pair_cells_max.end()) return it->second;
  const uint32_t nc = h.n_cols;
  uint32_t mx = 0;
  for (uint32_t b = 0; b < h.n_blocks; b++) {
    const uint8_t *cnt = &h.col_cnt[(size_t)b * nc];
    uint32_t cells = ((uint32_t)cnt[c0] + 1) * ((uint32_t)cnt[c1] + 1);
    if (cells > mx) mx = cells;
  }
  h.pair_cells_max[key] = mx;
  return mx;
}

static bool jit_blocks_ok(const obx_handle &h, const dev_plan_hdr &ph,
                          const jit_shape &js) {
  if (!h.lds_ok || h.col_class.empty()) return false;
  uint8_t gcol[2] = {0xFF, 0xFF};
  uint32_t cells = 1;
  for (uint32_t g = 0; g < ph.n_group_cols; g++) {
    gcol[g] = ph.need_cols[ph.group_idx[g]];
    if (!h.col_grp16_every[gcol[g]]) return false;
    cells *= h.col_cnt_max[gcol[g]] + 1;
  }
  if (cells > 16 && (ph.n_group_cols < 2 ||
                     jit_pair_cells_max(h, gcol[0], gcol[1]) > 16))
    return false;
  for (int j = 0; j < js.n_vc; j++)
    if (h.col_slow_any[js.vcol[j]]) return false;
  return true;
}

template <class GenSrc>
static jit_entry *jit_get(const std::string &key, GenSrc &&gen_src,
                          const char *kernel, const char *dump_name,
                          int wpb) {
  auto it = g_jit_cache.find(key);
  if (it != g_jit_cache.end())
    return it->second.fn ? &it->second : nullptr;
  jit_entry &ent = g_jit_cache[key];
  ent.wpb = wpb;
  const std::string src = gen_src();
  if (const char *dump_dir = getenv("OBX_JIT_DUMP")) {
    FILE *f = fopen((std::string(dump_dir) + "/" + dump_name).c_str(), "w");
    if (!f) f = fopen((std::string("/tmp/") + dump_name).c_str(), "w");
    if (f) { fwrite(src.data(), 1, src.size(), f); fclose(f); }
  }
  hiprtcProgram prog;
  const char *hdrs[4] = {OBX_JIT_SRC_COMMON_H, OBX_JIT_SRC_DEV_H,
                         OBX_JIT_SRC_JIT_DEV_H, OBX_JIT_SRC_KEYSET_H};
  const char *hdr_names[4] = {"obx_dev_common.h", "obx_dev.h",
                              "obx_jit_dev.h", "obx_keyset.h"};
  if (hiprtcCreateProgram(&prog, src.c_str(), dump_name, 4, hdrs,
                          hdr_names) != HIPRTC_SUCCESS)
    return nullptr;
  const char *opts[] = {"--offload-arch=gfx950", "-O3", "-std=c++17",
                        "-DOBX_HIPRTC=1"};
  if (hiprtcCompileProgram(prog, 4, opts) != HIPRTC_SUCCESS) {
    size_t lsz = 0;
    hiprtcGetProgramLogSize(prog, &lsz);
    if (lsz > 1) {
      std::string log(lsz, '\0');
      hiprtcGetProgramLog(prog, &log[0]);
      fprintf(stderr, "obx: JIT compile failed (%s):\n%s\n", kernel,
              log.c_str());
    }
    hiprtcDestroyProgram(&prog);
    return nullptr;
  }
  size_t csz = 0;
  hiprtcGetCodeSize(prog, &csz);
  std::string code(csz, '\0');
  hiprtcGetCode(prog, &code[0]);
  hiprtcDestroyProgram(&prog);
  if (hipModuleLoadData(&ent.mod, code.data()) != hipSuccess ||
      hipModuleGetFunction(&ent.fn, ent.mod, kernel) != hipSuccess) {
    fprintf(stderr, "obx: JIT module load failed (%s)\n", kernel);
    ent.fn = nullptr;
    return nullptr;
  }
  return &ent;
}

struct jit_scan_choice {
  int kind = 0;
  jit_shape js;
  jit_strategy st;
  jit_v1_strategy v1;
};

static int jit_scan_choose(const obx_handle &h, const dev_plan_hdr &ph,
                           const dev_leaf *pl, bool force_v1,
                           jit_scan_choice &c) {
  if (!jit_plan_shape(ph, c.js) || !jit_blocks_ok(h, ph, c.js)) return 0;
  if (!force_v1) jit_build_strategy(h, ph, c.js, pl, c.st);
  if (!c.st.ok && c.js.has_mm) return 0;
  if (!c.st.ok)
    if (const char *w = getenv("OBX_JIT_WPB")) c.v1.wpb = w;
  return c.kind = c.st.ok ? 2 : 1;
}

static std::string jit_scan_key(const dev_plan_hdr &ph,
                                const jit_scan_choice &c) {
  return jit_plan_sig(ph) +
         (c.kind == 2 ? jit_strategy_sig(ph, c.st) : jit_v1_sig(c.v1));
}

static std::string jit_scan_source(const dev_plan_hdr &ph,
                                   const jit_scan_choice &c) {
  return c.kind == 2 ? jit_gen_source_v2(ph, c.js, c.st)
                     : jit_gen_source(ph, c.js, c.v1);
}

static jit_entry *jit_prepare(const obx_handle &h, const dev_plan_hdr &ph,
                              const dev_leaf *pl) {
  const char *e = getenv("OBX_JIT");
  if (e && e[0] == '0') return nullptr;
  jit_scan_choice c;
  if (!jit_scan_choose(h, ph, pl, false, c)) return nullptr;
  g_jit_kind = c.kind;
  jit_entry *je = jit_get(
      jit_scan_key(ph, c), [&] { return jit_scan_source(ph, c); },
      "k_jit_scan", "obx_jit_src.hip", c.kind == 2 ? c.st.wpb : 0);
  if (je && c.kind == 2) {
    je->bdesc = c.st.bdesc != 0;
    je->bd_cols = c.st.bd_cols;
  }
  return je;
}

static jit_entry *jit_prepare_filter(const obx_handle &h,
                                     const dev_plan_hdr &ph,
                                     const dev_leaf *pl, int want_row_ids) {
  const char *e = getenv("OBX_JIT");
  if (e && e[0] == '0') return nullptr;
  jit_fstrategy st;
  if (!jit_build_fstrategy(h, ph, pl, st)) return nullptr;
  if (want_row_ids) {
    uint32_t nch = ((h.max_block_rows ? h.max_block_rows : 4096) + 63) / 64;
    if (!st.fstage || nch > 256) return nullptr;
    st.frid = 1;
    st.fnch = (uint16_t)nch;
  }
  return jit_get(
      jit_fstrategy_sig(ph, st), [&] { return jit_gen_source_filter(ph, st); },
      "k_jit_filter", "obx_jit_filter_src.hip", 0);
}

static int jit_launch(jit_entry *je, obx_handle &h, const obx_bdesc *bd,
                      hipStream_t stream, uint32_t *grid_out) {
  const uint32_t grid = je->wpb ? jit_grid_for(h.n_blocks, h.n_cus, je->wpb)
                                : grid_for(h.n_blocks);
  *grid_out = grid;
  void *args[8] = {&h.d_buf,     &h.d_blocks, &h.n_blocks,   &h.d_pleaves,
                   &h.d_bleaves, &h.d_gtable, &h.d_counters, &bd};
  return hipModuleLaunchKernel(je->fn, grid, 1, 1, OBX_WG_HOST, 1, 1, 0,
                               stream, args, nullptr) == hipSuccess
             ? 0
             : -1;
}
```

### oceanbase_amd/csrc/obx_jit_scan.inc

```

enum { JV_CTX = 0, JV_REF = 1 };
enum {
  JA_COUNT_STAR = 0,
  JA_I64 = 1,
  JA_HIST = 2,
  JA_HCOUNT = 3,
  JA_I64_COUNT = 4,
  JA_MM = 5,
  JA_HISTMM = 6,
};

struct jit_vtab {
  uint8_t vc = 0;
  uint8_t kind = 0;
  int64_t one = 0;
  uint32_t dim = 0;
};

struct jit_agg_ids {
  int8_t v[OBX_DEV_MAX_AGGS];
  jit_agg_ids() { for (int8_t &x : v) x = -1; }
  int8_t &operator[](size_t a) { return v[a]; }
  const int8_t &operator[](size_t a) const { return v[a]; }
};

struct jit_strategy {
  bool ok = false;
  uint8_t vmode[4] = {};
  uint8_t vext[4] = {};
  uint8_t vraw8[4] = {};
  uint32_t vdim[4] = {};
  uint8_t astrat[OBX_DEV_MAX_AGGS] = {};
  jit_agg_ids wa64;
  jit_agg_ids amm;
  int n_mm = 0;
  jit_agg_ids ahist;
  jit_agg_ids atab_b;
  jit_agg_ids atab_c;
  jit_agg_ids aval_a;
  jit_agg_ids atab_a;
  int n_w64 = 0;
  int n_hist = 0;
  uint8_t hist_vc[4] = {};
  int8_t hist_tab[4] = {};
  uint32_t hist_off[4] = {};
  uint32_t hist_total = 0;
  int n_tab = 0;
  jit_vtab tabs[6] = {};
  uint8_t leaf_inline = 0;
  uint8_t leaf_kind[8] = {};
  uint16_t leaf_cols[8] = {};
  uint8_t r = 1;
  uint8_t stripes = 4;
  uint32_t stage_bytes = OBX_LDS_STAGE_BYTES + 32;
  uint8_t leaf_multi[8] = {};
  uint8_t g_multi[2] = {};
  uint8_t v_multi[4] = {};
  uint8_t leaf_m32[8] = {};
  uint8_t g_m32[2] = {};
  uint8_t v_m32[4] = {};
  int8_t cnt_hist = -1;
  uint32_t jcells = 16;
  uint8_t jws_on = 0;
  int8_t jws_ja = -1;
  int8_t jws_a0 = -1, jws_a1 = -1;
  uint32_t jws_d0 = 1, jws_d1 = 1;
  uint32_t jws_cells = 16;
  uint8_t jws_member[OBX_DEV_MAX_AGGS] = {};
  jit_agg_ids jws_f0;
  jit_agg_ids jws_f1;
  int8_t ctab_agg = -1;
  uint32_t ctab_db = 0, ctab_dc = 0;
  uint32_t lds_bytes = 0;
  int wpb = 7;
  uint8_t bdesc = 0;
  obx_bdesc_cols bd_cols = {};
};

static int jit_bd_slot(const jit_strategy &st, uint16_t col) {
  for (uint32_t i = 0; i < st.bd_cols.n; i++)
    if (st.bd_cols.c[i] == col) return (int)i;
  return -1;
}

static bool jit_col_maxabs(const obx_handle &h, uint16_t col, uint64_t *out) {
  if (!h.col_known[col]) return false;
  if (h.col_min[col] > h.col_max[col]) { *out = 0; return true; }
  uint64_t a = h.col_min[col] == INT64_MIN
                   ? (uint64_t)INT64_MAX + 1
                   : (uint64_t)(h.col_min[col] < 0 ? -h.col_min[col]
                                                   : h.col_min[col]);
  uint64_t b2 = (uint64_t)(h.col_max[col] < 0 ? -h.col_max[col]
                                              : h.col_max[col]);
  *out = a > b2 ? a : b2;
  return true;
}

static uint64_t jit_sat_mul(uint64_t a, uint64_t b2) {
  if (a == 0 || b2 == 0) return 0;
  unsigned __int128 p = (unsigned __int128)a * b2;
  const uint64_t SAT = 1ull << 63;
  return p > SAT ? SAT : (uint64_t)p;
}

static int jit_tab_get(jit_strategy &st, uint8_t vc, uint8_t kind,
                       int64_t one, uint32_t dim) {
  for (int t = 0; t < st.n_tab; t++)
    if (st.tabs[t].vc == vc && st.tabs[t].kind == kind &&
        st.tabs[t].one == one)
      return t;
  if (st.n_tab >= 6) return -1;
  st.tabs[st.n_tab] = {vc, kind, one, dim};
  return st.n_tab++;
}

static int jit_hist_get(jit_strategy &st, uint8_t vc, uint32_t dim) {
  for (int t = 0; t < st.n_hist; t++)
    if (st.hist_vc[t] == vc) return t;
  if (st.n_hist >= 4) return -1;
  st.hist_vc[st.n_hist] = vc;
  st.hist_off[st.n_hist] = st.hist_total;
  st.hist_tab[st.n_hist] = -1;
  st.hist_total += st.jcells * dim;
  return st.n_hist++;
}

static bool jit_build_strategy(const obx_handle &h, const dev_plan_hdr &ph,
                               const jit_shape &js, const dev_leaf *pl,
                               jit_strategy &st) {
  const char *e = getenv("OBX_JIT_V2");
  if (e && e[0] == '0') return false;
  if (pl && ph.n_leaves >= 1 && ph.n_leaves <= 4) {
    st.leaf_inline = 1;
    for (uint32_t i = 0; i < ph.n_leaves; i++) {
      const uint8_t kind = jit_leaf_kind(h, pl[i]);
      if (kind != JL_RANGE && kind != JL_MASK) { st.leaf_inline = 0; break; }
      st.leaf_kind[i] = kind;
      st.leaf_cols[i] = pl[i].col;
    }
    if (!st.leaf_inline)
      for (uint32_t i = 0; i < 8; i++) st.leaf_kind[i] = 0;
  }
  uint64_t max_term = 0;
  const uint64_t BOUND = 1ull << 62;

  {
    uint32_t cells = 1;
    for (uint32_t g2 = 0; g2 < ph.n_group_cols; g2++)
      cells *= h.col_maxcnt[ph.need_cols[ph.group_idx[g2]]] + 1;
    if (cells < 1) cells = 1;
    if (cells > 16) cells = 16;
    st.jcells = cells;
  }

  for (int j = 0; j < js.n_vc; j++) {
    uint16_t col = js.vcol[j];
    if (h.col_dict_stable[col] && h.col_dict_every[col]) {
      st.vmode[j] = JV_REF;
      st.vdim[j] = h.col_maxcnt[col] + 1;
    } else {
      st.vmode[j] = JV_CTX;
      st.vext[j] = h.col_ext_any[col] ? 1 : 0;
      st.vraw8[j] = h.col_raw8_every[col] ? 1 : 0;
    }
  }
  for (uint32_t g2 = 0; g2 < ph.n_group_cols; g2++)
    if (!h.col_dict_stable[ph.need_cols[ph.group_idx[g2]]]) return false;
  auto maxabs_of = [&](uint8_t need_idx, uint64_t *out) -> bool {
    if (need_idx == 0xFF) return false;
    return jit_col_maxabs(h, ph.need_cols[need_idx], out);
  };

  for (uint32_t a = 0; a < ph.n_aggs; a++) {
    const dev_agg &g = ph.aggs[a];
    const int ja = js.slot(ph, g.ia), jb = js.slot(ph, g.ib),
              jc = js.slot(ph, g.ic);
    uint64_t ma = 0, mb = 0, mc = 0;
    switch (g.kind) {
      case OBX_AGG_COUNT:
        if (g.ia == 0xFF) { st.astrat[a] = JA_COUNT_STAR; break; }
        if (ja >= 0 && st.vmode[ja] == JV_REF) {
          int hid = jit_hist_get(st, (uint8_t)ja, st.vdim[ja]);
          if (hid < 0) return false;
          st.astrat[a] = JA_HCOUNT;
          st.ahist[a] = (int8_t)hid;
        } else if (ja >= 0 && !st.vext[ja]) {
          st.astrat[a] = JA_COUNT_STAR;
        } else if (ja >= 0) {
          st.astrat[a] = JA_I64_COUNT;
          st.wa64[a] = (int8_t)st.n_w64++;
          st.aval_a[a] = (int8_t)ja;
        } else {
          return false;
        }
        break;
      case OBX_AGG_SUM:
        if (ja < 0) return false;
        if (st.vmode[ja] == JV_REF) {
          int hid = jit_hist_get(st, (uint8_t)ja, st.vdim[ja]);
          if (hid < 0) return false;
          st.astrat[a] = JA_HIST;
          st.ahist[a] = (int8_t)hid;
        } else {
          if (!maxabs_of(g.ia, &ma)) return false;
          if (ma > max_term) max_term = ma;
          st.astrat[a] = JA_I64;
          st.wa64[a] = (int8_t)st.n_w64++;
          st.aval_a[a] = (int8_t)ja;
        }
        break;
      case OBX_AGG_SUM_PROD2:
      case OBX_AGG_SUM_PROD3:
      case OBX_AGG_SUM_MUL: {
        if (ja < 0 || jb < 0) return false;
        if (!maxabs_of(g.ia, &ma) || !maxabs_of(g.ib, &mb)) return false;
        uint64_t oneb = (uint64_t)(g.one_b < 0 ? -g.one_b : g.one_b);
        uint64_t onec = (uint64_t)(g.one_c < 0 ? -g.one_c : g.one_c);
        uint64_t term;
        if (g.kind == OBX_AGG_SUM_MUL) {
          term = jit_sat_mul(ma, mb);
        } else {
          term = jit_sat_mul(ma, oneb + mb);
          if (g.kind == OBX_AGG_SUM_PROD3) {
            if (jc < 0 || !maxabs_of(g.ic, &mc)) return false;
            term = jit_sat_mul(term, onec + mc);
          }
        }
        if (term > max_term) max_term = term;
        st.astrat[a] = JA_I64;
        st.wa64[a] = (int8_t)st.n_w64++;
        st.aval_a[a] = (int8_t)ja;
        if (st.vmode[ja] == JV_REF) {
          int t = jit_tab_get(st, (uint8_t)ja, 0, 0, st.vdim[ja]);
          if (t < 0) return false;
          st.atab_a[a] = (int8_t)t;
        }
        if (st.vmode[jb] == JV_REF) {
          uint8_t kind = (g.kind == OBX_AGG_SUM_MUL) ? 0 : 1;
          int t = jit_tab_get(st, (uint8_t)jb, kind,
                              kind ? g.one_b : 0, st.vdim[jb]);
          if (t < 0) return false;
          st.atab_b[a] = (int8_t)t;
        }
        if (g.kind == OBX_AGG_SUM_PROD3 && st.vmode[jc] == JV_REF) {
          int t = jit_tab_get(st, (uint8_t)jc, 2, g.one_c, st.vdim[jc]);
          if (t < 0) return false;
          st.atab_c[a] = (int8_t)t;
        }
        break;
      }
      case OBX_AGG_MIN:
      case OBX_AGG_MAX:
        if (ja < 0) return false;
        if (st.vmode[ja] == JV_REF) {
          int hid = jit_hist_get(st, (uint8_t)ja, st.vdim[ja]);
          if (hid < 0) return false;
          st.astrat[a] = JA_HISTMM;
          st.ahist[a] = (int8_t)hid;
          int tt = jit_tab_get(st, (uint8_t)ja, 0, 0, st.vdim[ja]);
          if (tt < 0) return false;
          st.atab_a[a] = (int8_t)tt;
        } else {
          st.astrat[a] = JA_MM;
          st.amm[a] = (int8_t)st.n_mm++;
          st.aval_a[a] = (int8_t)ja;
        }
        break;
      default:
        return false;
    }
    if (st.n_w64 > 8 || st.n_mm > 8) return false;
  }

  for (uint32_t a = 0; a < ph.n_aggs; a++) {
    if (st.astrat[a] != JA_HIST) continue;
    int t2 = st.ahist[a];
    if (st.hist_tab[t2] < 0) {
      int tt = jit_tab_get(st, st.hist_vc[t2], 0, 0,
                           st.vdim[st.hist_vc[t2]]);
      if (tt < 0) return false;
      st.hist_tab[t2] = (int8_t)tt;
    }
  }

  {
    const char *je = getenv("OBX_JIT_JWS");
    bool allow = !je || je[0] != '0';
    int8_t axes[2] = {-1, -1};
    uint8_t cand[OBX_DEV_MAX_AGGS] = {};
    int n_cand = 0, n_axed = 0;
    int8_t wja = -1;
    bool ok2 = true;
    for (uint32_t a = 0; allow && a < ph.n_aggs; a++) {
      if (st.astrat[a] != JA_I64 || st.aval_a[a] < 0 || st.atab_a[a] >= 0)
        continue;
      const dev_agg &g = ph.aggs[a];
      bool m = false;
      if (g.kind == OBX_AGG_SUM) m = true;
      else if (g.kind == OBX_AGG_SUM_MUL || g.kind == OBX_AGG_SUM_PROD2)
        m = st.atab_b[a] >= 0;
      else if (g.kind == OBX_AGG_SUM_PROD3)
        m = st.atab_b[a] >= 0 && st.atab_c[a] >= 0;
      if (!m) continue;
      if (wja < 0) wja = st.aval_a[a];
      else if (wja != st.aval_a[a]) continue;
      cand[a] = 1;
      n_cand++;
      int8_t tb[2] = {st.atab_b[a], g.kind == OBX_AGG_SUM_PROD3
                                        ? st.atab_c[a] : (int8_t)-1};
      for (int q = 0; q < 2; q++) {
        if (tb[q] < 0) continue;
        int8_t vc = (int8_t)st.tabs[tb[q]].vc;
        if (axes[0] < 0) axes[0] = vc;
        else if (axes[0] != vc && axes[1] < 0) axes[1] = vc;
        else if (axes[0] != vc && axes[1] != vc) ok2 = false;
      }
      if (tb[0] >= 0 || tb[1] >= 0) n_axed++;
    }
    if (allow && axes[1] >= 0) {
      auto adim = [&](int8_t vc) {
        uint32_t d = st.vdim[vc];
        return d ? d : 1;
      };
      const uint32_t cells0 = st.jcells;
      if ((uint64_t)cells0 * adim(axes[0]) * adim(axes[1]) * 8 > 2048) {
        int use[2] = {0, 0};
        for (uint32_t a = 0; a < ph.n_aggs; a++) {
          if (!cand[a]) continue;
          const dev_agg &g = ph.aggs[a];
          int8_t tb2[2] = {st.atab_b[a], g.kind == OBX_AGG_SUM_PROD3
                                             ? st.atab_c[a] : (int8_t)-1};
          bool on[2] = {false, false};
          for (int q = 0; q < 2; q++)
            if (tb2[q] >= 0)
              on[(int8_t)st.tabs[tb2[q]].vc == axes[1] ? 1 : 0] = true;
          if (on[0] && !on[1]) use[0]++;
          if (on[1] && !on[0]) use[1]++;
        }
        int8_t keep = use[1] > use[0] ? axes[1] : axes[0];
        n_cand = 0; n_axed = 0;
        for (uint32_t a = 0; a < ph.n_aggs; a++) {
          if (!cand[a]) continue;
          const dev_agg &g = ph.aggs[a];
          int8_t tb2[2] = {st.atab_b[a], g.kind == OBX_AGG_SUM_PROD3
                                             ? st.atab_c[a] : (int8_t)-1};
          bool ok3 = true, axed = false;
          for (int q = 0; q < 2; q++) {
            if (tb2[q] < 0) continue;
            if ((int8_t)st.tabs[tb2[q]].vc != keep) ok3 = false;
            else axed = true;
          }
          if (!ok3) { cand[a] = 0; continue; }
          n_cand++;
          if (axed) n_axed++;
        }
        axes[0] = keep;
        axes[1] = -1;
      }
    }
    if (allow && ok2 && n_cand >= 2 && n_axed >= 1 && axes[0] >= 0) {
      auto axis_dim = [&](int8_t vc) -> uint32_t {
        uint32_t d = st.vdim[vc];
        return d ? d : 1;
      };
      uint32_t d0 = axis_dim(axes[0]);
      uint32_t d1 = axes[1] >= 0 ? axis_dim(axes[1]) : 1;
      const uint32_t cells = st.jcells;
      if ((uint64_t)cells * d0 * d1 * 8 <= 24u * 1024u) {
        st.jws_on = 1;
        st.jws_ja = wja;
        st.jws_a0 = axes[0];
        st.jws_a1 = axes[1];
        st.jws_d0 = d0;
        st.jws_d1 = d1;
        st.jws_cells = cells;
        for (uint32_t a = 0; a < ph.n_aggs; a++) {
          if (!cand[a]) continue;
          st.jws_member[a] = 1;
          const dev_agg &g = ph.aggs[a];
          int8_t tb2[2] = {st.atab_b[a], g.kind == OBX_AGG_SUM_PROD3
                                             ? st.atab_c[a] : (int8_t)-1};
          for (int q = 0; q < 2; q++) {
            if (tb2[q] < 0) continue;
            if ((int8_t)st.tabs[tb2[q]].vc == st.jws_a0)
              st.jws_f0[a] = tb2[q];
            else
              st.jws_f1[a] = tb2[q];
          }
        }
        int nn = 0;
        for (uint32_t a = 0; a < ph.n_aggs; a++) {
          if (st.jws_member[a]) { st.wa64[a] = -1; continue; }
          if (st.wa64[a] >= 0) st.wa64[a] = (int8_t)nn++;
        }
        st.n_w64 = nn;
      }
    }
  }

  {
    const char *ce = getenv("OBX_JIT_CTAB");
    const bool allow = !ce || ce[0] != '0';
    for (uint32_t a = 0; allow && a < ph.n_aggs && st.ctab_agg < 0; a++) {
      const dev_agg &g = ph.aggs[a];
      if (g.kind != OBX_AGG_SUM_PROD3 || st.astrat[a] != JA_I64 ||
          st.jws_member[a] || st.wa64[a] < 0 || st.atab_a[a] >= 0 ||
          st.atab_b[a] < 0 || st.atab_c[a] < 0)
        continue;
      if (a > 0 && (js.agg_f2 & (1u << (a - 1))) && !st.jws_member[a - 1])
        continue;
      const uint16_t ca = ph.need_cols[g.ia], cb = ph.need_cols[g.ib],
                     cc = ph.need_cols[g.ic];
      if (!h.col_known[ca] || !h.col_known[cb] || !h.col_known[cc]) continue;
      const bool empty_b = h.col_min[cb] > h.col_max[cb],
                 empty_c = h.col_min[cc] > h.col_max[cc];
      if (h.col_min[ca] > h.col_max[ca] || empty_b || empty_c) continue;
      if (h.col_min[ca] < 0 || h.col_max[ca] > (int64_t)0xffffffffll)
        continue;
      const __int128 fb_lo = (__int128)g.one_b - h.col_max[cb],
                     fb_hi = (__int128)g.one_b - h.col_min[cb],
                     fc_lo = (__int128)g.one_c + h.col_min[cc],
                     fc_hi = (__int128)g.one_c + h.col_max[cc];
      if (fb_lo < 0 || fc_lo < 0 || fb_hi > 0xffffffffll ||
          fc_hi > 0xffffffffll || fb_hi * fc_hi > 0xffffffffll)
        continue;
      const uint32_t db = st.tabs[st.atab_b[a]].dim,
                     dc = st.tabs[st.atab_c[a]].dim;
      if ((uint64_t)db * dc > 1024) continue;
      st.ctab_agg = (int8_t)a;
      st.ctab_db = db;
      st.ctab_dc = dc;
    }
  }

  if (st.leaf_inline || ph.n_leaves == 0) {
    const char *re = getenv("OBX_JIT_R");
    int r = re ? atoi(re) : 4;
    if (r != 1 && r != 2 && r != 4 && r != 8) r = 4;
    st.r = (uint8_t)r;
    if (st.r > 1) {
      const char *ne = getenv("OBX_JIT_M32");
      const uint32_t w32 = (ne && ne[0] == '0') ? 0 : 32;
      for (uint32_t i = 0; i < ph.n_leaves; i++) {
        const uint32_t rw = h.col_maxw[st.leaf_cols[i]] * st.r;
        st.leaf_multi[i] = rw <= 64 ? 1 : 0;
        st.leaf_m32[i] = rw <= w32 ? 1 : 0;
      }
      for (uint32_t g2 = 0; g2 < ph.n_group_cols; g2++) {
        const uint32_t rw =
            h.col_maxw[ph.need_cols[ph.group_idx[g2]]] * st.r;
        st.g_multi[g2] = rw <= 64 ? 1 : 0;
        st.g_m32[g2] = rw <= w32 ? 1 : 0;
      }
      for (int j = 0; j < js.n_vc; j++) {
        const uint32_t rw = h.col_maxw[js.vcol[j]] * st.r;
        st.v_multi[j] = (st.vmode[j] == JV_REF && rw <= 64) ? 1 : 0;
        st.v_m32[j] = (st.vmode[j] == JV_REF && rw <= w32) ? 1 : 0;
      }
    }
  }
  for (int t = 0; t < st.n_hist; t++)
    if (st.cnt_hist < 0 ||
        st.vdim[st.hist_vc[t]] < st.vdim[st.hist_vc[st.cnt_hist]])
      st.cnt_hist = (int8_t)t;

  if (ph.n_leaves > 0 && !st.leaf_inline) return false;

  {
    const char *se = getenv("OBX_JIT_STRIPES");
    int sn = se ? atoi(se) : 4;
    if (sn != 1 && sn != 2 && sn != 4 && sn != 8 && sn != 16) sn = 4;
    st.stripes = (uint8_t)sn;
  }
  st.stage_bytes = ((h.max_block_len + 24 + 63) / 64) * 64;
  if (st.stage_bytes > OBX_LDS_STAGE_BYTES + 32)
    st.stage_bytes = OBX_LDS_STAGE_BYTES + 32;
  if (st.stage_bytes < st.jcells * ph.n_aggs * 16)
    st.stage_bytes = ((st.jcells * ph.n_aggs * 16 + 63) / 64) * 64;
  uint32_t lds = st.stage_bytes;
  lds += (uint32_t)st.n_w64 * st.jcells * 8 * st.stripes;
  lds += (uint32_t)st.n_mm * st.jcells * 16;
  lds += st.hist_total * 4;
  for (int t = 0; t < st.n_tab; t++) lds += st.tabs[t].dim * 8;
  if (st.ctab_agg >= 0) lds += st.ctab_db * st.ctab_dc * 4;
  lds += 16 * 8 + 16 * 4;
  if (st.jws_on)
    lds += st.jws_cells * st.jws_d0 * st.jws_d1 * 8;
  if (st.cnt_hist < 0) lds += st.jcells * 4 * st.stripes;
  lds += 64;
  st.lds_bytes = lds;
  st.wpb = (int)(163840 / (lds > 1 ? lds : 1));
  if (st.wpb > 8) st.wpb = 8;
  const char *we = getenv("OBX_JIT_WPB");
  if (we) {
    int w = atoi(we);
    if (w >= 2 && w <= 8 && w < st.wpb) st.wpb = w;
  }
  if (st.wpb < 2) return false;
  {
    const uint32_t grid = jit_grid_for(h.n_blocks, h.n_cus, st.wpb);
    const uint64_t maxrows =
        (uint64_t)((h.n_blocks + grid - 1) / grid) *
        (h.max_block_rows ? h.max_block_rows : 4096);
    if (jit_sat_mul(max_term, maxrows) >= BOUND) return false;
  }
  {
    const char *be = getenv("OBX_JIT_BDESC");
    bool on = !be || be[0] != '0';
    obx_bdesc_cols bc = {};
    auto add = [&](uint16_t col) {
      for (uint32_t i = 0; i < bc.n; i++)
        if (bc.c[i] == col) return;
      if (bc.n >= OBX_DEV_MAX_NEED || h.col_bdesc_unfit[col]) {
        on = false;
        return;
      }
      bc.c[bc.n++] = col;
    };
    for (uint32_t i = 0; on && i < ph.n_need; i++) add(ph.need_cols[i]);
    for (uint32_t i = 0; on && i < ph.n_leaves; i++) add(st.leaf_cols[i]);
    if (on) {
      st.bdesc = 1;
      st.bd_cols = bc;
    }
  }
  st.ok = true;
  return true;
}

static std::string jit_strategy_sig(const dev_plan_hdr &ph,
                                    const jit_strategy &st) {
  std::string k = "V2|";
  jit_emit(k, "w%dh%dt%dp%dli%dr%dch%ds%du%uc%um%d|", st.n_w64, st.n_hist,
           st.n_tab, st.wpb, st.leaf_inline, st.r, st.cnt_hist, st.stripes,
           st.stage_bytes, st.jcells, st.n_mm);
  for (int i = 0; i < 8; i++)
    jit_emit(k, "m%d%d%d|", st.leaf_multi[i] + 2 * st.leaf_m32[i],
             i < 2 ? st.g_multi[i] + 2 * st.g_m32[i] : 0,
             i < 4 ? st.v_multi[i] + 2 * st.v_m32[i] : 0);
  for (int i = 0; i < 8; i++)
    jit_emit(k, "L%d:%u|", st.leaf_kind[i], st.leaf_cols[i]);
  for (int j = 0; j < 4; j++)
    jit_emit(k, "v%d:%u:%u:%u|", st.vmode[j], st.vdim[j], st.vext[j],
             st.vraw8[j]);
  for (uint32_t a = 0; a < ph.n_aggs; a++)
    jit_emit(k, "a%d:%d:%d:%d:%d:%d:%d:%d|", st.astrat[a], st.wa64[a],
             st.ahist[a], st.atab_b[a], st.atab_c[a], st.atab_a[a],
             st.amm[a], st.aval_a[a]);
  for (int t = 0; t < st.n_tab; t++)
    jit_emit(k, "T%u:%u:%lld:%u|", st.tabs[t].vc, st.tabs[t].kind,
             (long long)st.tabs[t].one, st.tabs[t].dim);
  for (int t = 0; t < st.n_hist; t++)
    jit_emit(k, "H%u:%d:%u|", st.hist_vc[t], st.hist_tab[t], st.hist_off[t]);
  jit_emit(k, "C%d:%u:%u|", st.ctab_agg, st.ctab_db, st.ctab_dc);
  jit_emit(k, "B%d", st.bdesc);
  for (uint32_t i = 0; i < st.bd_cols.n; i++)
    jit_emit(k, ":%u", st.bd_cols.c[i]);
  k += "|";
  if (st.jws_on) {
    jit_emit(k, "J%d:%d:%d:%u:%u:%u|", st.jws_ja, st.jws_a0, st.jws_a1,
             st.jws_d0, st.jws_d1, st.jws_cells);
    for (uint32_t a = 0; a < ph.n_aggs; a++)
      jit_emit(k, "j%d:%d:%d|", st.jws_member[a], st.jws_f0[a],
               st.jws_f1[a]);
  }
  return k;
}


static jit_stream jit_v2_leaf_stream(int i) {
  return {jit_fmt("wl%d", i), jit_fmt("l%dW", i), jit_fmt("lm%d", i),
          "bv.base", jit_fmt("l%do", i)};
}
static jit_stream jit_v2_group_stream(int g) {
  return {jit_fmt("wgr%d", g), jit_fmt("gW%d", g), jit_fmt("gm%d", g),
          "bv.base", jit_fmt("go%d", g)};
}
static jit_stream jit_v2_value_stream(int j) {
  return {jit_fmt("wx%d", j), jit_fmt("xW%d", j), jit_fmt("xm%d", j),
          "bv.base", jit_fmt("xo%d", j)};
}

static void jit_v2_emit_mask(std::string &s, const jit_stream &sm, bool m32) {
  jit_emit(s,
           m32 ? "    const uint32_t %s = (1u << %s) - 1;\n"
               : "    const uint64_t %s = (1ull << %s) - 1;\n",
           sm.m.c_str(), sm.W.c_str());
}

static void jit_v2_emit_packed_read(std::string &s, const jit_stream &sm,
                                    bool m32, int R) {
  if (m32)
    jit_emit(s,
             "      uint32_t %s = jit_bread32(bv.base, %s + rbase * %s);\n",
             sm.w.c_str(), sm.off.c_str(), sm.W.c_str());
  else
    jit_emit(s,
             "      uint64_t %1$s = jit_bread(bv.base, %2$s + rbase * %3$s, "
             "%4$d * %3$s);\n",
             sm.w.c_str(), sm.off.c_str(), sm.W.c_str(), R);
}

static void jit_v2_emit_ref(std::string &s, const std::string &name,
                            const std::string &count, const jit_stream &sm,
                            bool packed) {
  jit_emit(s,
           "        uint32_t %1$s = (uint32_t)%2$s;\n"
           "        if (%1$s > %3$s) %1$s = %3$s;\n",
           name.c_str(), sm.field(packed).c_str(), count.c_str());
}

static std::string jit_v2_operand(int tab, int j, char sign, int64_t one) {
  if (tab >= 0) return jit_fmt("vt%d[x%d]", tab, j);
  if (!sign) return jit_fmt("(nu%1$d ? 0ll : v%1$d)", j);
  return jit_fmt("(nu%1$d ? 0ll : (%2$lldll %3$c v%1$d))", j, (long long)one,
                 sign);
}

static const char *jit_v2_is_min(const dev_agg &g) {
  return g.kind == OBX_AGG_MIN ? "true" : "false";
}

struct jit_v2_facc {
  uint32_t sum = 0, min = 0, max = 0;
  bool any() const { return (sum | min | max) != 0; }
};
static jit_v2_facc jit_v2_facc_of(const dev_plan_hdr &ph,
                                  const jit_strategy &st) {
  jit_v2_facc f;
  for (uint32_t a = 0; a < ph.n_aggs; a++) {
    if (st.astrat[a] == JA_HIST || st.astrat[a] == JA_HCOUNT ||
        (st.jws_on && st.jws_member[a]))
      f.sum |= 1u << a;
    else if (st.astrat[a] == JA_HISTMM)
      (ph.aggs[a].kind == OBX_AGG_MIN ? f.min : f.max) |= 1u << a;
  }
  return f;
}


static void jit_v2_prologue(const dev_plan_hdr &ph, const jit_shape &,
                            const jit_strategy &st, std::string &s) {
  s += "#include \"obx_dev_common.h\"\n"
       "#include \"obx_jit_dev.h\"\n\n";
  jit_emit(s,
           "#define NL %d\n#define NG %d\n#define NW64 %d\n"
           "#define NAGGS %u\n#define HTOT %u\n#define NSTRIPE %u\n"
           "#define JSTAGE %u\n#define JC %u\n\n",
           (int)ph.n_leaves, (int)ph.n_group_cols,
           st.n_w64 > 0 ? st.n_w64 : 1, (unsigned)ph.n_aggs,
           st.hist_total > 0 ? st.hist_total : 1, (unsigned)st.stripes,
           (unsigned)st.stage_bytes, st.jcells);
  if (st.bdesc)
    jit_emit(s,
             "#define NBS %u\n"
             "/* what the block loop needs of one block, in registers: the\n"
             "   packed descriptor's header and column slots, and the\n"
             "   block's lowered leaf tests. Wave-uniform, whole words:\n"
             "   scalar loads. */\n"
             "struct jmeta {\n"
             "  uint64_t byte;\n"
             "  uint32_t len, rows;\n"
             "  uint64_t s[NBS];\n"
             "  jit_leafw lf[NL ? NL : 1];\n"
             "};\n"
             "__device__ __forceinline__ void jit_load_meta(\n"
             "    jmeta &m, const obx_bdesc *__restrict__ bdesc,\n"
             "    const blk_leaf *__restrict__ bleaves, uint32_t blk) {\n"
             "  const obx_bdesc &d = bdesc[blk];\n"
             "  m.byte = d.block_byte;\n"
             "  m.len = d.block_len;\n"
             "  m.rows = d.row_count;\n"
             "#pragma unroll\n"
             "  for (uint32_t i = 0; i < NBS; i++) m.s[i] = d.slot[i];\n"
             "#pragma unroll\n"
             "  for (uint32_t i = 0; i < NL; i++)\n"
             "    m.lf[i] = jit_load_leafw(bleaves + (uint64_t)blk * NL + "
             "i);\n"
             "}\n\n",
             st.bd_cols.n);
  jit_emit(s,
           "/* Persistent-accumulator scan (the whole-kernel generalization\n"
           "   of the storage group-by pushdown, ObVectorStore::do_group_by):\n"
           "   the dicts are byte-identical in every micro block (verified\n"
           "   at load), so histograms, value tables and group keys are\n"
           "   global-dict-keyed, live in LDS for the kernel's lifetime,\n"
           "   and merge into the global table exactly once. Per block:\n"
           "   stage to LDS, sweep rows, nothing else. */\n"
           "extern \"C\" __global__ __launch_bounds__(256, %d) void "
           "k_jit_scan(\n"
           "    const uint8_t *__restrict__ buf, const dev_block "
           "*__restrict__ blocks,\n"
           "    uint32_t n_blocks, const dev_leaf *__restrict__ "
           "plan_leaves,\n"
           "    const blk_leaf *__restrict__ bleaves, gslot *__restrict__ "
           "gtable,\n"
           "    unsigned long long *__restrict__ counters,\n"
           "    const obx_bdesc *__restrict__ bdesc) {\n",
           st.wpb);
}

static void jit_v2_lds(const dev_plan_hdr &ph, const jit_shape &,
                       const jit_strategy &st, std::string &s) {
  s += "  __shared__ __attribute__((aligned(16))) uint8_t "
       "lds_blk[JSTAGE];\n"
       "  __shared__ unsigned long long wacc64[NW64][JC][NSTRIPE];\n"
       "  __shared__ uint32_t hist[HTOT];\n";
  if (st.n_mm > 0)
    jit_emit(s,
             "  /* CAS min/max cells: [slot][cell][val, valid] */\n"
             "  __shared__ unsigned long long wmm[%d][JC][2];\n",
             st.n_mm);
  s += "  __shared__ uint64_t keytab[16];\n"
       "  __shared__ int cslot[16];\n";
  if (st.jws_on)
    jit_emit(s, "  __shared__ unsigned long long jws[%uu * %uu * %uu];\n",
             st.jws_cells, st.jws_d0, st.jws_d1);
  if (st.cnt_hist < 0)
    s += "  __shared__ uint32_t wcnt[JC][NSTRIPE];\n";
  for (int t = 0; t < st.n_tab; t++)
    jit_emit(s, "  __shared__ long long vt%d[%u];\n", t, st.tabs[t].dim);
  if (st.ctab_agg >= 0)
    jit_emit(s,
             "  /* combined factor table [xb][xc] of the narrowed PROD3 */\n"
             "  __shared__ uint32_t vtc[%uu * %uu];\n",
             st.ctab_db, st.ctab_dc);
  s += "  const uint32_t tid = threadIdx.x, lane = tid & 63, wv = tid >> "
       "6;\n"
       "  uint32_t lane_cnt = 0;\n"
       "  const uint32_t stripe = lane & (NSTRIPE - 1);\n"
       "\n"
       "  for (uint32_t i = tid; i < NW64 * JC * NSTRIPE; i += WG)\n"
       "    (&wacc64[0][0][0])[i] = 0;\n";
  for (uint32_t a = 0; a < ph.n_aggs; a++) {
    if (st.amm[a] < 0) continue;
    jit_emit(s,
             "  for (uint32_t i = tid; i < JC; i += WG) {\n"
             "    wmm[%1$d][i][0] = (unsigned long long)%2$s;\n"
             "    wmm[%1$d][i][1] = 0;\n"
             "  }\n",
             st.amm[a],
             ph.aggs[a].kind == OBX_AGG_MIN ? "INT64_MAX" : "INT64_MIN");
  }
  s += "  for (uint32_t i = tid; i < HTOT; i += WG) hist[i] = 0;\n";
  if (st.jws_on)
    jit_emit(s,
             "  for (uint32_t i = tid; i < %uu * %uu * %uu; i += WG)\n"
             "    jws[i] = 0;\n",
             st.jws_cells, st.jws_d0, st.jws_d1);
  if (st.cnt_hist < 0)
    s += "  for (uint32_t i = tid; i < JC * NSTRIPE; i += WG)\n"
         "    (&wcnt[0][0])[i] = 0;\n";
}

static void jit_v2_emit_key_part(const dev_plan_hdr &ph, int g,
                                 std::string &s) {
  const std::string keep =
      ph.group_len[g] >= 8
          ? "~0ull"
          : jit_fmt("((1ull << (8 * %u)) - 1)", (unsigned)ph.group_len[g]);
  if (g == 0)
    jit_emit(s,
             "    for (uint32_t cell = tid; cell < fcells; cell += WG) {\n"
             "      uint32_t r0 = %s;\n"
             "      uint64_t key = 0;\n"
             "      if (r0 >= gb0->count) key |= 1ull << 56;\n"
             "      else {\n"
             "        int64_t kv = dict_entry(bv0, *gb0, r0);\n"
             "        key |= (uint64_t)kv & %s;\n"
             "      }\n",
             ph.n_group_cols > 1 ? "cell % fdim0" : "cell", keep.c_str());
  else
    jit_emit(s,
             "      uint32_t r1 = cell / fdim0;\n"
             "      if (r1 >= gb1->count) key |= 1ull << 57;\n"
             "      else {\n"
             "        int64_t kv1 = dict_entry(bv0, *gb1, r1);\n"
             "        key |= ((uint64_t)kv1 & %s) << (8 * %u);\n"
             "      }\n",
             keep.c_str(), (unsigned)ph.group_len[0]);
}

static void jit_v2_tables(const dev_plan_hdr &ph, const jit_shape &js,
                          const jit_strategy &st, std::string &s) {
  const int NG = ph.n_group_cols;
  s += "  {\n"
       "    const dev_block &b0 = blocks[0];\n"
       "    blk_view bv0;\n"
       "    bv0.base = buf + b0.block_byte;\n"
       "    bv0.bit_bias = b0.block_byte * 8;\n"
       "    bv0.rbase_bit = 0;\n";
  for (int t = 0; t < st.n_tab; t++) {
    const jit_vtab &vt = st.tabs[t];
    const std::string ex =
        vt.kind == 0 ? "e2"
                     : jit_fmt("%lldll %c e2", (long long)vt.one,
                               vt.kind == 1 ? '-' : '+');
    jit_emit(s,
             "    {\n"
             "      const dev_col *tb = &b0.cols[%u];\n"
             "      for (uint32_t e = tid; e <= tb->count && e < %uu; e += "
             "WG) {\n"
             "        long long v2 = 0;\n"
             "        if (e < tb->count) {\n"
             "          long long e2 = dict_entry(bv0, *tb, e);\n"
             "          v2 = %s;\n"
             "        }\n"
             "        vt%d[e] = v2;\n"
             "      }\n"
             "    }\n",
             (unsigned)js.vcol[vt.vc], vt.dim, ex.c_str(), t);
  }
  if (st.ctab_agg >= 0) {
    const dev_agg &g = ph.aggs[st.ctab_agg];
    jit_emit(s,
             "    {\n"
             "      const dev_col *tb = &b0.cols[%1$u], *tc = &b0.cols[%2$u];\n"
             "      for (uint32_t e = tid; e < %3$uu * %4$uu; e += WG) {\n"
             "        const uint32_t eb = e / %4$uu, ec = e %% %4$uu;\n"
             "        long long fb = 0, fc = 0; /* null slots: factor 0 */\n"
             "        if (eb < tb->count) fb = %5$lldll - dict_entry(bv0, *tb, "
             "eb);\n"
             "        if (ec < tc->count) fc = %6$lldll + dict_entry(bv0, *tc, "
             "ec);\n"
             "        vtc[e] = (uint32_t)(fb * fc);\n"
             "      }\n"
             "    }\n",
             (unsigned)ph.need_cols[g.ib], (unsigned)ph.need_cols[g.ic],
             st.ctab_db, st.ctab_dc, (long long)g.one_b, (long long)g.one_c);
  }
  if (NG > 0) {
    jit_emit(s,
             "    const dev_col *gb0 = &b0.cols[%u];\n"
             "    const uint32_t fdim0 = gb0->count + 1;\n",
             (unsigned)ph.need_cols[ph.group_idx[0]]);
    if (NG > 1)
      jit_emit(s,
               "    const dev_col *gb1 = &b0.cols[%u];\n"
               "    const uint32_t fdim1 = gb1->count + 1;\n"
               "    const uint32_t fcells = fdim0 * fdim1;\n",
               (unsigned)ph.need_cols[ph.group_idx[1]]);
    else
      s += "    const uint32_t fcells = fdim0;\n";
    for (int g = 0; g < NG; g++) jit_v2_emit_key_part(ph, g, s);
    s += "      keytab[cell] = key;\n"
         "    }\n";
  } else {
    s += "    if (tid == 0) keytab[0] = 0;\n";
  }
  s += "  }\n"
       "  __syncthreads();\n"
       "\n";
}

static void jit_v2_block_head_bdesc(const dev_plan_hdr &ph,
                                    const jit_shape &js,
                                    const jit_strategy &st, std::string &s) {
  const int NG = ph.n_group_cols;
  const int NL = ph.n_leaves;
  s += "  for (uint32_t blk = blockIdx.x; blk < n_blocks; blk += "
       "gridDim.x) {\n"
       "    jmeta cm;\n"
       "    jit_load_meta(cm, bdesc, bleaves, blk);\n"
       "    uint8_t blk_verdict = 1;\n";
  for (int i = 0; i < NL; i++)
    jit_emit(s,
             "    {\n"
             "      const uint8_t c = jit_leaf_class(\n"
             "          cm.lf[%d], OBX_BD_FLAGS(cm.s[%d]));\n"
             "      if (c == 0) blk_verdict = 0;\n"
             "      else if (c == 2 && blk_verdict) blk_verdict = 2;\n"
             "    }\n",
             i, jit_bd_slot(st, st.leaf_cols[i]));
  s += "    if (blk_verdict == 0) continue;\n"
       "    __syncthreads(); /* drain previous block's LDS reads */\n"
       "    stage2(buf, cm.byte, cm.len, lds_blk);\n"
       "    asm volatile(\"s_waitcnt vmcnt(0)\" ::: \"memory\");\n"
       "    __syncthreads();\n"
       "    const uint64_t blk_bit = cm.byte * 8;\n"
       "    blk_view bv;\n"
       "    bv.base = lds_blk;\n"
       "    bv.bit_bias = blk_bit;\n"
       "    bv.rbase_bit = 0;\n"
       "    const uint32_t rows = cm.rows;\n"
       "\n";
  for (int g = 0; g < NG && g < 2; g++)
    jit_emit(s,
             "    const uint32_t go%1$d = OBX_BD_OFF(cm.s[%2$d]);\n"
             "    const uint32_t gW%1$d = OBX_BD_WIDTH(cm.s[%2$d]);\n"
             "    const uint32_t gn%1$d = OBX_BD_COUNT(cm.s[%2$d]);\n",
             g, jit_bd_slot(st, ph.need_cols[ph.group_idx[g]]));
  if (NG > 1) s += "    const uint32_t dim0 = gn0 + 1;\n";
  for (int j = 0; j < js.n_vc; j++) {
    const int k = jit_bd_slot(st, js.vcol[j]);
    if (st.vmode[j] == JV_REF)
      jit_emit(s,
               "    const uint32_t xo%1$d = OBX_BD_OFF(cm.s[%2$d]);\n"
               "    const uint32_t xW%1$d = OBX_BD_WIDTH(cm.s[%2$d]);\n"
               "    const uint32_t xn%1$d = OBX_BD_COUNT(cm.s[%2$d]);\n",
               j, k);
    else if (st.vraw8[j])
      jit_emit(s, "    const uint32_t vb%d = OBX_BD_OFF(cm.s[%d]) >> 3;\n", j,
               k);
    else
      jit_emit(s,
               "    const col_ctx c%d =\n"
               "        make_col_ctx(blocks[blk].cols[%u], blk_bit);\n",
               j, (unsigned)js.vcol[j]);
  }
}

static void jit_v2_block_head_blocks(const dev_plan_hdr &ph,
                                     const jit_shape &js,
                                     const jit_strategy &st, std::string &s) {
  const int NG = ph.n_group_cols;
  s += "  for (uint32_t blk = blockIdx.x; blk < n_blocks; blk += "
       "gridDim.x) {\n"
       "    const dev_block &cur = blocks[blk];\n"
       "    const blk_leaf *bl = bleaves + (uint64_t)blk * (NL ? NL : "
       "1);\n"
       "    uint8_t blk_verdict = 1;\n"
       "    for (uint32_t i = 0; i < NL; i++) {\n"
       "      uint8_t c = leaf_class(cur, plan_leaves[i], bl[i]);\n"
       "      if (c == 0) { blk_verdict = 0; break; }\n"
       "      if (c == 2) blk_verdict = 2;\n"
       "    }\n"
       "    if (blk_verdict == 0) continue;\n"
       "    __syncthreads(); /* drain previous block's LDS reads */\n"
       "    stage2(buf, cur, lds_blk);\n"
       "    asm volatile(\"s_waitcnt vmcnt(0)\" ::: \"memory\");\n"
       "    __syncthreads();\n"
       "    const uint64_t blk_bit = cur.block_byte * 8;\n"
       "    blk_view bv;\n"
       "    bv.base = lds_blk;\n"
       "    bv.bit_bias = blk_bit;\n"
       "    bv.rbase_bit = 0;\n"
       "    const uint32_t rows = cur.row_count;\n"
       "\n";
  for (int g = 0; g < NG && g < 2; g++) {
    jit_emit(s,
             "    const dev_col *gd%1$d = &cur.cols[%2$u];\n"
             "    const uint32_t go%1$d = (uint32_t)(gd%1$d->data_bit - "
             "blk_bit);\n"
             "    const uint32_t gW%1$d = PW(*gd%1$d);\n"
             "    const uint32_t gn%1$d = gd%1$d->count;\n",
             g, (unsigned)ph.need_cols[ph.group_idx[g]]);
    if (g == 1) s += "    const uint32_t dim0 = gn0 + 1;\n";
  }
  for (int j = 0; j < js.n_vc; j++) {
    const unsigned col = js.vcol[j];
    if (st.vmode[j] == JV_REF)
      jit_emit(s,
               "    const uint32_t xo%1$d =\n"
               "        (uint32_t)(cur.cols[%2$u].data_bit - blk_bit);\n"
               "    const uint32_t xW%1$d = PW(cur.cols[%2$u]);\n"
               "    const uint32_t xn%1$d = cur.cols[%2$u].count;\n",
               j, col);
    else if (st.vraw8[j])
      jit_emit(s,
               "    const uint32_t vb%d =\n"
               "        (uint32_t)((cur.cols[%u].data_bit >> 3) - "
               "cur.block_byte);\n",
               j, col);
    else
      jit_emit(s,
               "    const col_ctx c%d = make_col_ctx(cur.cols[%u], "
               "blk_bit);\n",
               j, col);
  }
}

static void jit_v2_leaf_preambles(const dev_plan_hdr &ph, const jit_shape &js,
                                  const jit_strategy &st, std::string &s) {
  const int NG = ph.n_group_cols;
  for (int i = 0; i < (int)ph.n_leaves; i++) {
    if (st.bdesc)
      jit_emit(s,
               "    const blk_leaf lb%1$d = jit_leaf_of(cm.lf[%1$d]);\n"
               "    const uint32_t l%1$do = OBX_BD_OFF(cm.s[%2$d]);\n"
               "    const uint32_t l%1$dW = OBX_BD_WIDTH(cm.s[%2$d]);\n",
               i, jit_bd_slot(st, st.leaf_cols[i]));
    else
      jit_emit(s,
               "    const blk_leaf lb%1$d = bl[%1$d];\n"
               "    const uint32_t l%1$do =\n"
               "        (uint32_t)(cur.cols[%2$u].data_bit - blk_bit);\n"
               "    const uint32_t l%1$dW = PW(cur.cols[%2$u]);\n",
               i, (unsigned)st.leaf_cols[i]);
    if (st.leaf_kind[i] == JL_RANGE)
      jit_emit(s,
               "    const bool l%1$d_all = lb%1$d.mode == OBX_LEAF_ALL;\n", i);
    if (st.r > 1 && st.leaf_multi[i])
      jit_v2_emit_mask(s, jit_v2_leaf_stream(i), st.leaf_m32[i]);
  }
  if (st.r <= 1) return;
  for (int g = 0; g < NG && g < 2; g++)
    if (st.g_multi[g])
      jit_v2_emit_mask(s, jit_v2_group_stream(g), st.g_m32[g]);
  for (int j = 0; j < js.n_vc; j++)
    if (st.v_multi[j])
      jit_v2_emit_mask(s, jit_v2_value_stream(j), st.v_m32[j]);
}

static void jit_v2_accumulate(const dev_plan_hdr &ph, const jit_shape &js,
                              const jit_strategy &st, std::string &s) {
  s += "        lane_cnt += live ? 1u : 0u;\n"
       "        if (live) {\n";
  if (st.cnt_hist < 0)
    s += "          atomicAdd(&wcnt[cell][stripe], 1u);\n";
  for (int t = 0; t < st.n_hist; t++) {
    const int j = st.hist_vc[t];
    jit_emit(s, "          atomicAdd(&hist[%uu + cell * %uu + x%d], 1u);\n",
             st.hist_off[t], st.vdim[j], j);
  }
  if (st.jws_on) {
    auto axis = [](int j, uint32_t d) {
      return jit_fmt("(x%1$d < %2$uu ? x%1$d : %3$uu)", j, d, d - 1);
    };
    const std::string idx =
        st.jws_a1 >= 0
            ? jit_fmt("cell * %uu + %s * %uu + %s", st.jws_d0 * st.jws_d1,
                      axis(st.jws_a0, st.jws_d0).c_str(), st.jws_d1,
                      axis(st.jws_a1, st.jws_d1).c_str())
            : jit_fmt("cell * %uu + %s", st.jws_d0,
                      axis(st.jws_a0, st.jws_d0).c_str());
    jit_emit(s,
             "          if (!nu%1$d)\n"
             "            atomicAdd(&jws[%2$s],\n"
             "                      (unsigned long long)v%1$d);\n",
             st.jws_ja, idx.c_str());
  }
  for (uint32_t a = 0; a < ph.n_aggs; a++) {
    const dev_agg &g = ph.aggs[a];
    if (st.jws_member[a]) continue;
    if (st.astrat[a] == JA_I64_COUNT) {
      jit_emit(s,
               "          if (!nu%d)\n"
               "            atomicAdd(&wacc64[%d][cell][stripe], 1ull);\n",
               st.aval_a[a], st.wa64[a]);
      continue;
    }
    if (st.astrat[a] == JA_MM) {
      jit_emit(s,
               "          if (!nu%1$d) {\n"
               "            cas_minmax(&wmm[%2$d][cell][0], v%1$d, %3$s);\n"
               "            wmm[%2$d][cell][1] = 1;\n"
               "          }\n",
               st.aval_a[a], st.amm[a], jit_v2_is_min(g));
      continue;
    }
    if (st.astrat[a] != JA_I64) continue;
    const int ja = st.aval_a[a], jb = js.slot(ph, g.ib),
              jc = js.slot(ph, g.ic);
    const std::string va = st.atab_a[a] >= 0
                               ? jit_fmt("vt%d[x%d]", st.atab_a[a], ja)
                               : jit_fmt("v%d", ja);
    switch (g.kind) {
      case OBX_AGG_SUM:
        jit_emit(s,
                 "          atomicAdd(&wacc64[%d][cell][stripe],\n"
                 "                    (unsigned long long)%s);\n",
                 st.wa64[a], va.c_str());
        break;
      case OBX_AGG_SUM_MUL:
        jit_emit(s,
                 "          atomicAdd(&wacc64[%d][cell][stripe],\n"
                 "                    (unsigned long long)((long long)%s * "
                 "%s));\n",
                 st.wa64[a], va.c_str(),
                 jit_v2_operand(st.atab_b[a], jb, 0, 0).c_str());
        break;
      case OBX_AGG_SUM_PROD2:
        jit_emit(s,
                 "          long long p2_%1$u = (long long)%2$s * %3$s;\n"
                 "          atomicAdd(&wacc64[%4$d][cell][stripe],\n"
                 "                    (unsigned long long)p2_%1$u);\n",
                 a, va.c_str(),
                 jit_v2_operand(st.atab_b[a], jb, '-', g.one_b).c_str(),
                 st.wa64[a]);
        if ((js.agg_f2 & (1u << a)) && !st.jws_member[a + 1]) {
          const dev_agg &g3 = ph.aggs[a + 1];
          jit_emit(s,
                   "          atomicAdd(&wacc64[%d][cell][stripe],\n"
                   "                    (unsigned long long)(p2_%u * "
                   "%s));\n",
                   st.wa64[a + 1], a,
                   jit_v2_operand(st.atab_c[a + 1], js.slot(ph, g3.ic), '+',
                                  g3.one_c)
                       .c_str());
        }
        break;
      case OBX_AGG_SUM_PROD3:
        if (a > 0 && (js.agg_f2 & (1u << (a - 1))) && !st.jws_member[a - 1])
          break;
        if (st.ctab_agg == (int)a) {
          jit_emit(s,
                   "          atomicAdd(&wacc64[%d][cell][stripe],\n"
                   "                    (unsigned long long)(uint32_t)v%d *\n"
                   "                        (unsigned long long)vtc[x%d * %uu "
                   "+ x%d]);\n",
                   st.wa64[a], ja, jb, st.ctab_dc, jc);
          break;
        }
        jit_emit(s,
                 "          atomicAdd(&wacc64[%d][cell][stripe],\n"
                 "                    (unsigned long long)((long long)%s * "
                 "%s * %s));\n",
                 st.wa64[a], va.c_str(),
                 jit_v2_operand(st.atab_b[a], jb, '-', g.one_b).c_str(),
                 jit_v2_operand(st.atab_c[a], jc, '+', g.one_c).c_str());
        break;
    }
  }
  s += "        }\n";
}

static void jit_v2_sweep(const dev_plan_hdr &ph, const jit_shape &js,
                         const jit_strategy &st, std::string &s) {
  const int NG = ph.n_group_cols;
  const int NL = ph.n_leaves;
  const int R = st.r > 0 ? st.r : 1;
  jit_emit(s,
           "    const uint32_t itersR = (rows + WG * %1$d - 1) / (WG * %1$d);\n"
           "    for (uint32_t it = 0; it < itersR; it++) {\n"
           "      const uint32_t rbase = (it * WG + tid) * %1$d;\n",
           R);
  for (int i = 0; i < NL; i++)
    if (st.leaf_multi[i])
      jit_v2_emit_packed_read(s, jit_v2_leaf_stream(i), st.leaf_m32[i], R);
  for (int g = 0; g < NG && g < 2; g++)
    if (st.g_multi[g])
      jit_v2_emit_packed_read(s, jit_v2_group_stream(g), st.g_m32[g], R);
  for (int j = 0; j < js.n_vc; j++)
    if (st.v_multi[j])
      jit_v2_emit_packed_read(s, jit_v2_value_stream(j), st.v_m32[j], R);
  for (int j = 0; j < js.n_vc; j++)
    if (st.vmode[j] == JV_CTX && st.vraw8[j])
      jit_emit(s,
               "      const uint8_t *ep%1$d = bv.base + vb%1$d + (rbase << "
               "3);\n",
               j);
  jit_emit(s,
           "#pragma unroll\n"
           "      for (uint32_t k = 0; k < %du; k++) {\n"
           "        const uint32_t r = rbase + k;\n"
           "        bool live = r < rows;\n",
           R);
  for (int i = 0; i < NL; i++) {
    const jit_leaf_ops lb = {i,
                             jit_fmt("lb%d.mask", i),
                             jit_fmt("lb%d.lo", i),
                             jit_fmt("lb%d.hi", i),
                             jit_fmt("lb%d.invert", i),
                             ""};
    const std::string f = jit_v2_leaf_stream(i).field(st.leaf_multi[i] != 0);
    if (st.leaf_kind[i] == JL_RANGE) jit_emit_range_test(s, 8, lb, f, true);
    else jit_emit_mask_test(s, 8, lb, f, true);
  }
  for (int g = 0; g < NG && g < 2; g++) {
    jit_v2_emit_ref(s, jit_fmt("ref%d", g), jit_fmt("gn%d", g),
                    jit_v2_group_stream(g), st.r > 1 && st.g_multi[g]);
    s += g ? "        cell += ref1 * dim0;\n" : "        uint32_t cell = ref0;\n";
  }
  if (NG == 0) s += "        const uint32_t cell = 0;\n";
  for (int j = 0; j < js.n_vc; j++) {
    if (st.vmode[j] == JV_REF)
      jit_v2_emit_ref(s, jit_fmt("x%d", j), jit_fmt("xn%d", j),
                      jit_v2_value_stream(j), st.v_multi[j] != 0);
    else if (st.vraw8[j])
      jit_emit(s,
               "        int64_t v%1$d = *(const int64_t *)(ep%1$d + (k << "
               "3));\n"
               "        const bool nu%1$d = false;\n"
               "        (void)nu%1$d;\n",
               j);
    else
      jit_emit(s,
               "        bool nu%1$d;\n"
               "        int64_t v%1$d = ctx_value(bv, c%1$d, r, nu%1$d);\n"
               "        (void)nu%1$d;\n",
               j);
  }
  jit_v2_accumulate(ph, js, st, s);
  s += "      }\n"
       "    } /* row sweep */\n"
       "  } /* blocks */\n";
}

static void jit_v2_flush_head(const dev_plan_hdr &ph, const jit_shape &,
                              const jit_strategy &st, std::string &s) {
  const int NG = ph.n_group_cols;
  s += "\n"
       "\n"
       "  /* survivor count: wave-reduce, then stripe the global atomic\n"
       "     over 8 slots (same-address atomics serialize at L2) */\n"
       "  for (int off = 32; off > 0; off >>= 1)\n"
       "    lane_cnt += (uint32_t)__shfl_xor((int)lane_cnt, off, 64);\n"
       "  if (lane == 0 && lane_cnt)\n"
       "    atomicAdd(&counters[8 + ((blockIdx.x * WAVES + wv) & 7)],\n"
       "              (unsigned long long)lane_cnt);\n"
       "  __syncthreads(); /* all accumulators final: flush once */\n"
       "\n"
       "  const dev_block &b0 = blocks[0];\n";
  if (NG > 0)
    jit_emit(s, "  const uint32_t fdim0 = b0.cols[%u].count + 1;\n",
             (unsigned)ph.need_cols[ph.group_idx[0]]);
  if (NG > 1)
    jit_emit(s, "  const uint32_t fcells = fdim0 * (b0.cols[%u].count + 1);\n",
             (unsigned)ph.need_cols[ph.group_idx[1]]);
  else
    s += NG == 1 ? "  const uint32_t fcells = fdim0;\n"
                 : "  const uint32_t fcells = 1;\n";
  const jit_v2_facc f = jit_v2_facc_of(ph, st);
  if (f.any())
    jit_emit(s,
             "  /* workgroup partials [cell][agg]: {lo, hi} of an int128\n"
             "     sum, or {value, valid} of a min/max */\n"
             "  unsigned long long (*facc)[NAGGS][2] =\n"
             "      (unsigned long long (*)[NAGGS][2])lds_blk;\n"
             "  for (uint32_t i = tid; i < JC * NAGGS; i += WG) {\n"
             "    const uint32_t a = i %% NAGGS;\n"
             "    facc[i / NAGGS][a][0] =\n"
             "        ((0x%xu >> a) & 1)   ? (unsigned long long)INT64_MAX\n"
             "        : ((0x%xu >> a) & 1) ? (unsigned long long)INT64_MIN\n"
             "                             : 0ull;\n"
             "    facc[i / NAGGS][a][1] = 0;\n"
             "  }\n",
             f.min, f.max);
}

static void jit_v2_flush_cells(const dev_plan_hdr &ph, const jit_shape &,
                               const jit_strategy &st, std::string &s) {
  s += "  /* flush pass 1: per-cell counts, keys -> global slots */\n"
       "  for (uint32_t cell = tid; cell < fcells; cell += WG) {\n"
       "    int ce = -1;\n";
  if (st.cnt_hist >= 0) {
    const int j = st.hist_vc[st.cnt_hist];
    jit_emit(s,
             "    unsigned long long cnt2 = 0;\n"
             "    for (uint32_t ref = 0; ref < %1$uu; ref++)\n"
             "      cnt2 += hist[%2$uu + cell * %1$uu + ref];\n",
             st.vdim[j], st.hist_off[st.cnt_hist]);
  } else {
    s += "    unsigned long long cnt2 = 0;\n"
         "    for (uint32_t s2 = 0; s2 < NSTRIPE; s2++)\n"
         "      cnt2 += wcnt[cell][s2];\n";
  }
  s += "    if (cnt2) {\n"
       "      int gi = jit_gslot(gtable, keytab[cell]);\n"
       "      if (gi >= 0) {\n"
       "        atomicAdd(&gtable[gi].count, cnt2);\n"
       "        ce = gi;\n";
  for (uint32_t a = 0; a < ph.n_aggs; a++)
    if (st.astrat[a] == JA_COUNT_STAR)
      jit_emit(s, "        g_acc_i128(gtable[gi].cells[%u], cnt2, 0);\n",
               (unsigned)a);
  for (uint32_t a = 0; a < ph.n_aggs; a++) {
    if (st.wa64[a] < 0) continue;
    jit_emit(s,
             "        {\n"
             "          unsigned long long t64 = 0;\n"
             "          for (uint32_t s2 = 0; s2 < NSTRIPE; s2++)\n"
             "            t64 += wacc64[%d][cell][s2];\n"
             "          int64_t v64 = (int64_t)t64;\n"
             "          if (v64)\n"
             "            g_acc_i128(gtable[gi].cells[%u], (uint64_t)v64,\n"
             "                       (uint64_t)(v64 >> 63));\n"
             "        }\n",
             st.wa64[a], (unsigned)a);
  }
  for (uint32_t a = 0; a < ph.n_aggs; a++) {
    if (st.amm[a] < 0) continue;
    jit_emit(s,
             "        if (wmm[%1$d][cell][1]) {\n"
             "          cas_minmax(&gtable[gi].cells[%2$u][0],\n"
             "                     (int64_t)wmm[%1$d][cell][0], %3$s);\n"
             "          gtable[gi].cells[%2$u][1] = 1;\n"
             "        }\n",
             st.amm[a], (unsigned)a, jit_v2_is_min(ph.aggs[a]));
  }
  s += "      } else {\n"
       "        atomicAdd(&counters[1], cnt2);\n"
       "      }\n"
       "    }\n"
       "    cslot[cell] = ce;\n"
       "  }\n"
       "  __syncthreads();\n";
}

static void jit_v2_flush_hists(const dev_plan_hdr &ph, const jit_shape &js,
                               const jit_strategy &st, std::string &s) {
  s += "  /* flush pass 2: histogram-weighted aggregates over (cell, ref) "
       "*/\n";
  for (int t = 0; t < st.n_hist; t++) {
    const int j = st.hist_vc[t];
    bool any = false, need_entry = false;
    for (uint32_t a = 0; a < ph.n_aggs; a++) {
      if (st.ahist[a] != t) continue;
      if (st.astrat[a] == JA_HIST || st.astrat[a] == JA_HCOUNT ||
          st.astrat[a] == JA_HISTMM)
        any = true;
      if (st.astrat[a] == JA_HIST) need_entry = true;
    }
    if (!any) continue;
    jit_emit(s,
             "  {\n"
             "    const uint32_t hcnt = b0.cols[%1$u].count;\n"
             "    for (uint32_t idx = tid; idx < fcells * %2$uu; idx += WG) "
             "{\n"
             "      uint32_t cell = idx / %2$uu, ref = idx %% %2$uu;\n"
             "      int ce = cslot[cell];\n"
             "      if (ce < 0 || ref >= hcnt) continue; /* excl. null "
             "bucket */\n"
             "      uint32_t c2 = hist[%3$uu + cell * %2$uu + ref];\n"
             "      if (!c2) continue;\n",
             (unsigned)js.vcol[j], st.vdim[j], st.hist_off[t]);
    if (need_entry)
      jit_emit(s, "      long long ev = vt%d[ref];\n", st.hist_tab[t]);
    for (uint32_t a = 0; a < ph.n_aggs; a++) {
      if (st.ahist[a] != t) continue;
      if (st.astrat[a] == JA_HIST)
        jit_emit(s,
                 "      {\n"
                 "        __int128 p = (__int128)ev * (long long)c2;\n"
                 "        i128v pv = {(uint64_t)p,\n"
                 "                    (uint64_t)((unsigned __int128)p >> "
                 "64)};\n"
                 "        lds_acc_i128(facc[cell][%u], pv);\n"
                 "      }\n",
                 (unsigned)a);
      else if (st.astrat[a] == JA_HISTMM)
        jit_emit(s,
                 "      {\n"
                 "        cas_minmax(&facc[cell][%1$u][0],\n"
                 "                   (int64_t)vt%2$d[ref], %3$s);\n"
                 "        facc[cell][%1$u][1] = 1;\n"
                 "      }\n",
                 (unsigned)a, st.atab_a[a], jit_v2_is_min(ph.aggs[a]));
      else
        jit_emit(s,
                 "      atomicAdd(&facc[cell][%u][0], (unsigned long "
                 "long)c2);\n",
                 (unsigned)a);
    }
    s += "    }\n"
         "  }\n";
  }
}

static void jit_v2_flush_joint(const dev_plan_hdr &ph, const jit_shape &,
                               const jit_strategy &st, std::string &s) {
  if (!st.jws_on) return;
  jit_emit(s,
           "  for (uint32_t idx = tid; idx < fcells * %1$uu; idx += WG) "
           "{\n"
           "    uint32_t cell = idx / %1$uu, d0 = idx %% %1$uu;\n"
           "    int ce = cslot[cell];\n"
           "    if (ce < 0) continue;\n"
           "    long long s_pl = 0;\n",
           st.jws_d0);
  int c_tabs[OBX_DEV_MAX_AGGS], n_ct = 0;
  for (uint32_t a = 0; a < ph.n_aggs; a++) {
    if (!st.jws_member[a] || st.jws_f1[a] < 0) continue;
    bool seen = false;
    for (int q = 0; q < n_ct; q++) seen |= c_tabs[q] == st.jws_f1[a];
    if (!seen) c_tabs[n_ct++] = st.jws_f1[a];
  }
  for (int q = 0; q < n_ct; q++)
    jit_emit(s, "    __int128 s_c%d = 0;\n", c_tabs[q]);
  jit_emit(s,
           "    for (uint32_t d1 = 0; d1 < %1$uu; d1++) {\n"
           "      long long w = (long long)jws[cell * %2$uu + d0 * %1$uu + "
           "d1];\n"
           "      if (!w) continue;\n"
           "      s_pl += w;\n",
           st.jws_d1, st.jws_d0 * st.jws_d1);
  for (int q = 0; q < n_ct; q++)
    jit_emit(s, "      s_c%1$d += (__int128)vt%1$d[d1] * w;\n", c_tabs[q]);
  s += "    }\n"
       "    if (s_pl";
  for (int q = 0; q < n_ct; q++) jit_emit(s, " || s_c%d != 0", c_tabs[q]);
  s += ") {\n";
  for (uint32_t a = 0; a < ph.n_aggs; a++) {
    if (!st.jws_member[a]) continue;
    const int f0 = st.jws_f0[a], f1 = st.jws_f1[a];
    const std::string sum = f1 >= 0 ? jit_fmt("s_c%d", f1) : "s_pl";
    const std::string expr =
        f0 >= 0   ? jit_fmt("(__int128)vt%d[d0] * %s", f0, sum.c_str())
        : f1 >= 0 ? sum
                  : "(__int128)s_pl";
    jit_emit(s,
             "      {\n"
             "        __int128 p = %s;\n"
             "        if (p != 0) {\n"
             "          i128v pv = {(uint64_t)p,\n"
             "                      (uint64_t)((unsigned __int128)p >> "
             "64)};\n"
             "          lds_acc_i128(facc[cell][%u], pv);\n"
             "        }\n"
             "      }\n",
             expr.c_str(), (unsigned)a);
  }
  s += "    }\n"
       "  }\n";
}

static void jit_v2_flush_partials(const dev_plan_hdr &ph, const jit_shape &,
                                  const jit_strategy &st, std::string &s) {
  const jit_v2_facc f = jit_v2_facc_of(ph, st);
  if (f.any())
    jit_emit(s,
             "  __syncthreads();\n"
             "  /* flush pass 4: one global accumulate per (cell, aggregate) "
             "*/\n"
             "  for (uint32_t idx = tid; idx < fcells * NAGGS; idx += WG) {\n"
             "    const uint32_t cell = idx / NAGGS, a = idx %% NAGGS;\n"
             "    const int ce = cslot[cell];\n"
             "    if (ce < 0) continue;\n"
             "    const unsigned long long lo = facc[cell][a][0],\n"
             "                             hi = facc[cell][a][1];\n"
             "    if ((0x%xu >> a) & 1) {\n"
             "      if (lo | hi) g_acc_i128(gtable[ce].cells[a], lo, hi);\n"
             "    } else if (((0x%xu >> a) & 1) && hi) {\n"
             "      cas_minmax(&gtable[ce].cells[a][0], (int64_t)lo,\n"
             "                 (0x%xu >> a) & 1);\n"
             "      gtable[ce].cells[a][1] = 1;\n"
             "    }\n"
             "  }\n",
             f.sum, f.min | f.max, f.min);
  s += "}\n";
}

static std::string jit_gen_source_v2(const dev_plan_hdr &ph,
                                     const jit_shape &js,
                                     const jit_strategy &st) {
  std::string s;
  jit_v2_prologue(ph, js, st, s);
  jit_v2_lds(ph, js, st, s);
  jit_v2_tables(ph, js, st, s);
  if (st.bdesc) jit_v2_block_head_bdesc(ph, js, st, s);
  else jit_v2_block_head_blocks(ph, js, st, s);
  jit_v2_leaf_preambles(ph, js, st, s);
  jit_v2_sweep(ph, js, st, s);
  jit_v2_flush_head(ph, js, st, s);
  jit_v2_flush_cells(ph, js, st, s);
  jit_v2_flush_hists(ph, js, st, s);
  jit_v2_flush_joint(ph, js, st, s);
  jit_v2_flush_partials(ph, js, st, s);
  return s;
}
```

### oceanbase_amd/engine.py

```python
import ctypes as C
import os

from . import abi

_PKG = os.path.dirname(os.path.abspath(__file__))
_SO = os.path.join(_PKG, "libobx.so")

OBX_NO_GPU = -7001


class EngineUnavailable(RuntimeError):
    pass


def _load():
    if not os.path.exists(_SO):
        raise EngineUnavailable(
            f"{_SO} not built — run oceanbase_amd/csrc/build.sh (the product "
            "path has no CPU fallback)")
    lib = C.CDLL(_SO)
    lib.obx_gpu_open.restype = C.c_int
    lib.obx_gpu_open.argtypes = [C.c_int, C.POINTER(C.c_void_p)]
    lib.obx_gpu_close.restype = C.c_int
    lib.obx_gpu_close.argtypes = [C.c_void_p]
    lib.obx_gpu_load_blocks.restype = C.c_int
    lib.obx_gpu_load_blocks.argtypes = [C.c_void_p, C.POINTER(abi.BlockSet)]
    lib.obx_gpu_load_cs_blocks.restype = C.c_int
    lib.obx_gpu_load_cs_blocks.argtypes = [C.c_void_p,
                                           C.POINTER(abi.BlockSet)]
    lib.obx_gpu_free_blocks.restype = C.c_int
    lib.obx_gpu_free_blocks.argtypes = [C.c_void_p, C.c_int]
    lib.obx_gpu_filter.restype = C.c_int
    lib.obx_gpu_filter.argtypes = [C.c_void_p, C.c_int,
                                   C.POINTER(abi.FilterDesc), C.c_int]
    lib.obx_gpu_fetch_bitmap.restype = C.c_int
    lib.obx_gpu_fetch_bitmap.argtypes = [C.c_void_p, C.c_int, C.c_void_p,
                                         C.c_int64]
    lib.obx_gpu_fetch_row_ids.restype = C.c_int
    lib.obx_gpu_fetch_row_ids.argtypes = [C.c_void_p, C.c_int, C.c_void_p,
                                          C.c_int64, C.POINTER(C.c_uint64)]
    lib.obx_gpu_fetch_blk_counts.restype = C.c_int
    lib.obx_gpu_fetch_blk_counts.argtypes = [C.c_void_p, C.c_int, C.c_void_p,
                                             C.c_int64]
    lib.obx_gpu_decode.restype = C.c_int
    lib.obx_gpu_decode.argtypes = [C.c_void_p, C.c_int,
                                   C.POINTER(C.c_uint16), C.c_uint16]
    lib.obx_gpu_fetch_col.restype = C.c_int
    lib.obx_gpu_fetch_col.argtypes = [C.c_void_p, C.c_int, C.c_uint16,
                                      C.c_void_p, C.c_int64]
    lib.obx_gpu_scan_project.restype = C.c_int
    lib.obx_gpu_scan_project.argtypes = [C.c_void_p, C.c_int,
                                         C.POINTER(abi.FilterDesc),
                                         C.POINTER(C.c_uint16), C.c_uint16,
                                         C.c_int, C.POINTER(C.c_uint64)]
    lib.obx_gpu_fetch_proj.restype = C.c_int
    lib.obx_gpu_fetch_proj.argtypes = [C.c_void_p, C.c_int, C.c_uint16,
                                       C.c_uint64, C.c_uint64, C.c_void_p,
                                       C.c_int64, C.c_void_p, C.c_int64,
                                       C.POINTER(C.c_uint64)]
    lib.obx_gpu_fetch_proj_row_nos.restype = C.c_int
    lib.obx_gpu_fetch_proj_row_nos.argtypes = [C.c_void_p, C.c_int,
                                               C.c_uint64, C.c_uint64,
                                               C.c_void_p, C.c_int64,
                                               C.POINTER(C.c_uint64)]
    lib.obx_gpu_last_proj_stage_ms.restype = C.c_double
    lib.obx_gpu_last_proj_stage_ms.argtypes = [C.c_void_p, C.c_int]
    lib.obx_gpu_scan_filter_agg.restype = C.c_int
    lib.obx_gpu_scan_filter_agg.argtypes = [C.c_void_p, C.c_int,
                                            C.POINTER(abi.FilterDesc),
                                            C.POINTER(abi.AggDesc),
                                            C.POINTER(abi.AggResult)]
    lib.obx_gpu_last_kernel_ms.restype = C.c_double
    lib.obx_gpu_last_kernel_ms.argtypes = [C.c_void_p]
    lib.obx_gpu_last_prep_ms.restype = C.c_double
    lib.obx_gpu_last_prep_ms.argtypes = [C.c_void_p]
    lib.obx_gpu_last_jit.restype = C.c_int
    lib.obx_gpu_last_jit.argtypes = [C.c_void_p]
    lib.obx_gpu_last_bdesc.restype = C.c_int
    lib.obx_gpu_last_bdesc.argtypes = [C.c_void_p]
    lib.obx_gpu_bdesc_builds.restype = C.c_int64
    lib.obx_gpu_bdesc_builds.argtypes = [C.c_void_p, C.c_int]
    lib.obx_gpu_keyset_create.restype = C.c_int
    lib.obx_gpu_keyset_create.argtypes = [C.c_void_p, C.c_void_p, C.c_uint64,
                                          C.c_int]
    lib.obx_gpu_keyset_from_proj.restype = C.c_int
    lib.obx_gpu_keyset_from_proj.argtypes = [C.c_void_p, C.c_int, C.c_uint16,
                                             C.c_int]
    lib.obx_gpu_keyset_free.restype = C.c_int
    lib.obx_gpu_keyset_free.argtypes = [C.c_void_p, C.c_int]
    lib.obx_gpu_keyset_info.restype = C.c_int
    lib.obx_gpu_keyset_info.argtypes = [C.c_void_p, C.c_int,
                                        C.POINTER(abi.KeysetInfo)]
    lib.obx_gpu_keyset_host_model.restype = C.c_int
    lib.obx_gpu_keyset_host_model.argtypes = [
        C.c_void_p, C.c_uint64, C.c_int, C.c_void_p, C.c_uint64, C.c_void_p,
        C.POINTER(abi.KeysetInfo)]
    lib.obx_gpu_keymap_create.restype = C.c_int
    lib.obx_gpu_keymap_create.argtypes = [C.c_void_p, C.c_void_p, C.c_void_p,
                                          C.c_uint64,
                                          C.POINTER(abi.ColSchema), C.c_int]
    lib.obx_gpu_keymap_from_proj.restype = C.c_int
    lib.obx_gpu_keymap_from_proj.argtypes = [C.c_void_p, C.c_int, C.c_uint16,
                                             C.c_uint16, C.c_int]
    lib.obx_gpu_keymap_free.restype = C.c_int
    lib.obx_gpu_keymap_free.argtypes = [C.c_void_p, C.c_int]
    lib.obx_gpu_keymap_info.restype = C.c_int
    lib.obx_gpu_keymap_info.argtypes = [C.c_void_p, C.c_int,
                                        C.POINTER(abi.KeymapInfo)]
    lib.obx_gpu_keymap_host_model.restype = C.c_int
    lib.obx_gpu_keymap_host_model.argtypes = [
        C.c_void_p, C.c_void_p, C.c_uint64, C.POINTER(abi.ColSchema), C.c_int,
        C.c_void_p, C.c_uint64, C.c_void_p, C.c_void_p,
        C.POINTER(abi.KeymapInfo)]
    lib.obx_gpu_scan_join_agg.restype = C.c_int
    lib.obx_gpu_scan_join_agg.argtypes = [C.c_void_p, C.c_int,
                                          C.POINTER(abi.FilterDesc),
                                          C.POINTER(abi.JoinDesc),
                                          C.POINTER(abi.AggDesc),
                                          C.POINTER(abi.AggResult)]
    for f in ("obx_gpu_total_rows", "obx_gpu_total_bytes",
              "obx_gpu_last_survivors"):
        getattr(lib, f).restype = C.c_uint64
        getattr(lib, f).argtypes = [C.c_void_p, C.c_int]
    return lib


_lib = None


def lib():
    global _lib
    if _lib is None:
        _lib = _load()
    return _lib


class KeysetError(RuntimeError):

    def __init__(self, what, rc):
        super().__init__(f"{what} failed: {rc}")
        self.rc = rc


def _i64(a):
    import numpy as np
    return np.ascontiguousarray(np.asarray(a, dtype=np.int64))


def keyset_host_model(keys, probe=(), kind=0):
    import numpy as np
    k, p = _i64(keys), _i64(probe)
    hit = np.zeros(p.size, dtype=np.uint8)
    info = abi.KeysetInfo()
    rc = lib().obx_gpu_keyset_host_model(
        k.ctypes.data_as(C.c_void_p), k.size, kind,
        p.ctypes.data_as(C.c_void_p), p.size,
        hit.ctypes.data_as(C.c_void_p), C.byref(info))
    if rc != 0:
        raise KeysetError("obx_gpu_keyset_host_model", rc)
    return hit.astype(bool), info


class KeymapError(RuntimeError):

    def __init__(self, what, rc):
        super().__init__(f"{what} failed: {rc}")
        self.rc = rc


def _payload_args(payloads, spec, n):
    import numpy as np
    cs = abi.ColSchema(*spec)
    p = np.asarray(payloads)
    if p.dtype == np.uint8 and p.ndim == 2:
        raw = np.ascontiguousarray(p)
        assert raw.shape == (n, cs.len)
    else:
        raw = np.ascontiguousarray(
            _i64(p).view(np.uint8).reshape(-1, 8)[:, :cs.len])
        assert raw.shape[0] == n
    return raw, cs


def keymap_host_model(keys, payloads, spec, probe=(), kind=0):
    import numpy as np
    k, p = _i64(keys), _i64(probe)
    raw, cs = _payload_args(payloads, spec, k.size)
    hit = np.zeros(p.size, dtype=np.uint8)
    pay = np.zeros(p.size, dtype=np.uint64)
    info = abi.KeymapInfo()
    rc = lib().obx_gpu_keymap_host_model(
        k.ctypes.data_as(C.c_void_p), raw.ctypes.data_as(C.c_void_p), k.size,
        C.byref(cs), kind, p.ctypes.data_as(C.c_void_p), p.size,
        hit.ctypes.data_as(C.c_void_p), pay.ctypes.data_as(C.c_void_p),
        C.byref(info))
    if rc != 0:
        raise KeymapError("obx_gpu_keymap_host_model", rc)
    return hit.astype(bool), pay, info


class GpuEngine:
    def __init__(self, device=0):
        self._lib = lib()
        self._ctx = C.c_void_p()
        rc = self._lib.obx_gpu_open(device, C.byref(self._ctx))
        if rc == OBX_NO_GPU:
            raise EngineUnavailable("no HIP device visible (product path "
                                    "refuses to run without a GPU)")
        if rc != 0:
            raise RuntimeError(f"obx_gpu_open failed: {rc}")

    def close(self):
        if self._ctx:
            self._lib.obx_gpu_close(self._ctx)
            self._ctx = None

    def __del__(self):
        try:
            self.close()
        except Exception:
            pass

    def load(self, bs):
        h = self._lib.obx_gpu_load_blocks(self._ctx, C.byref(bs))
        if h < 0:
            raise RuntimeError(f"obx_gpu_load_blocks failed: {h}")
        return h

    def load_cs(self, cs_blocks, schema):
        from . import cs as _cs
        bs, keep = _cs.make_blockset(cs_blocks, schema)
        h = self._lib.obx_gpu_load_cs_blocks(self._ctx, C.byref(bs))
        if h < 0:
            raise RuntimeError(f"obx_gpu_load_cs_blocks failed: {h}")
        return h

    def free(self, handle):
        self._lib.obx_gpu_free_blocks(self._ctx, handle)

    def keyset_create(self, keys, kind=0):
        k = _i64(keys)
        sid = self._lib.obx_gpu_keyset_create(
            self._ctx, k.ctypes.data_as(C.c_void_p), k.size, kind)
        if sid < 0:
            raise KeysetError("obx_gpu_keyset_create", sid)
        return sid

    def keyset_from_proj(self, handle, proj_idx, kind=0):
        sid = self._lib.obx_gpu_keyset_from_proj(self._ctx, handle, proj_idx,
                                                 kind)
        if sid < 0:
            raise KeysetError("obx_gpu_keyset_from_proj", sid)
        return sid

    def keyset_free(self, sid):
        rc = self._lib.obx_gpu_keyset_free(self._ctx, sid)
        if rc != 0:
            raise KeysetError("obx_gpu_keyset_free", rc)

    def keyset_info(self, sid):
        info = abi.KeysetInfo()
        rc = self._lib.obx_gpu_keyset_info(self._ctx, sid, C.byref(info))
        if rc != 0:
            raise KeysetError("obx_gpu_keyset_info", rc)
        return info

    def keymap_create(self, keys, payloads, spec, kind=0):
        k = _i64(keys)
        raw, cs = _payload_args(payloads, spec, k.size)
        mid = self._lib.obx_gpu_keymap_create(
            self._ctx, k.ctypes.data_as(C.c_void_p),
            raw.ctypes.data_as(C.c_void_p), k.size, C.byref(cs), kind)
        if mid < 0:
            raise KeymapError("obx_gpu_keymap_create", mid)
        return mid

    def keymap_from_proj(self, handle, key_idx, payload_idx, kind=0):
        mid = self._lib.obx_gpu_keymap_from_proj(self._ctx, handle, key_idx,
                                                 payload_idx, kind)
        if mid < 0:
            raise KeymapError("obx_gpu_keymap_from_proj", mid)
        return mid

    def keymap_free(self, mid):
        rc = self._lib.obx_gpu_keymap_free(self._ctx, mid)
        if rc != 0:
            raise KeymapError("obx_gpu_keymap_free", rc)

    def keymap_info(self, mid):
        info = abi.KeymapInfo()
        rc = self._lib.obx_gpu_keymap_info(self._ctx, mid, C.byref(info))
        if rc != 0:
            raise KeymapError("obx_gpu_keymap_info", rc)
        return info

    def _scan_join_agg(self, handle, filter_desc, map_id, probe_col,
                       agg_desc):
        res = abi.AggResult()
        join = abi.JoinDesc(map_id, probe_col, 0)
        rc = self._lib.obx_gpu_scan_join_agg(
            self._ctx, handle,
            C.byref(filter_desc) if filter_desc is not None else None,
            C.byref(join),
            C.byref(agg_desc) if agg_desc is not None else None,
            C.byref(res))
        return rc, res

    def scan_join_agg(self, handle, filter_desc, map_id, probe_col, agg_desc):
        rc, res = self._scan_join_agg(handle, filter_desc, map_id, probe_col,
                                      agg_desc)
        if rc != 0:
            raise KeymapError("obx_gpu_scan_join_agg", rc)
        return res

    def scan_join_agg_paged(self, handle, filter_desc, map_id, probe_col,
                            agg_desc):
        rc, res = self._scan_join_agg(handle, filter_desc, map_id, probe_col,
                                      agg_desc)
        if rc not in (0, abi.OBX_BUF_NOT_ENOUGH):
            raise KeymapError("obx_gpu_scan_join_agg", rc)
        return res, self.agg_fetch_all(handle)

    def filter(self, handle, filter_desc, want_row_ids=False):
        rc = self._lib.obx_gpu_filter(self._ctx, handle,
                                      C.byref(filter_desc),
                                      1 if want_row_ids else 0)
        if rc != 0:
            raise RuntimeError(f"obx_gpu_filter failed: {rc}")
        return self._lib.obx_gpu_last_survivors(self._ctx, handle)

    def fetch_bitmap(self, handle):
        import numpy as np
        rows = self._lib.obx_gpu_total_rows(self._ctx, handle)
        out = np.zeros((rows + 7) // 8, dtype=np.uint8)
        rc = self._lib.obx_gpu_fetch_bitmap(self._ctx, handle,
                                            out.ctypes.data_as(C.c_void_p),
                                            out.nbytes)
        if rc != 0:
            raise RuntimeError(f"fetch_bitmap failed: {rc}")
        return out

    def fetch_row_ids(self, handle):
        import numpy as np
        rows = self._lib.obx_gpu_total_rows(self._ctx, handle)
        out = np.zeros(rows, dtype=np.int32)
        n = C.c_uint64(0)
        rc = self._lib.obx_gpu_fetch_row_ids(self._ctx, handle,
                                             out.ctypes.data_as(C.c_void_p),
                                             rows, C.byref(n))
        if rc != 0:
            raise RuntimeError(f"fetch_row_ids failed: {rc}")
        return out, int(n.value)

    def fetch_blk_counts(self, handle, n_blocks):
        import numpy as np
        out = np.zeros(n_blocks, dtype=np.uint32)
        rc = self._lib.obx_gpu_fetch_blk_counts(
            self._ctx, handle, out.ctypes.data_as(C.c_void_p), n_blocks)
        if rc != 0:
            raise RuntimeError(f"fetch_blk_counts failed: {rc}")
        return out

    def decode(self, handle, cols):
        arr = (C.c_uint16 * len(cols))(*cols)
        rc = self._lib.obx_gpu_decode(self._ctx, handle, arr, len(cols))
        if rc != 0:
            raise RuntimeError(f"obx_gpu_decode failed: {rc}")

    def fetch_col(self, handle, col, datum_len):
        import numpy as np
        rows = self._lib.obx_gpu_total_rows(self._ctx, handle)
        out = np.zeros(rows * datum_len, dtype=np.uint8)
        rc = self._lib.obx_gpu_fetch_col(self._ctx, handle, col,
                                         out.ctypes.data_as(C.c_void_p),
                                         out.nbytes)
        if rc != 0:
            raise RuntimeError(f"fetch_col failed: {rc}")
        return out

    def scan_project(self, handle, filter_desc, cols, want_row_nos=False):
        arr = (C.c_uint16 * len(cols))(*cols)
        n = C.c_uint64(0)
        rc = self._lib.obx_gpu_scan_project(
            self._ctx, handle,
            C.byref(filter_desc) if filter_desc is not None else None,
            arr, len(cols), 1 if want_row_nos else 0, C.byref(n))
        if rc != 0:
            raise RuntimeError(f"obx_gpu_scan_project failed: {rc}")
        return int(n.value)

    def _proj_window(self, handle, proj_idx, start, count):
        n = C.c_uint64(0)
        rc = self._lib.obx_gpu_fetch_proj(
            self._ctx, handle, proj_idx, start,
            count if count is not None else 2**63, None, 0, None, 0,
            C.byref(n))
        if rc != 0:
            raise RuntimeError(f"obx_gpu_fetch_proj failed: {rc}")
        return int(n.value)

    def fetch_proj(self, handle, proj_idx, datum_len, start=0, count=None):
        import numpy as np
        n = self._proj_window(handle, proj_idx, start, count)
        out = np.zeros(n * datum_len, dtype=np.uint8)
        nulls = np.zeros((n + 7) // 8, dtype=np.uint8)
        got = C.c_uint64(0)
        rc = self._lib.obx_gpu_fetch_proj(
            self._ctx, handle, proj_idx, start, n,
            out.ctypes.data_as(C.c_void_p), out.nbytes,
            nulls.ctypes.data_as(C.c_void_p), nulls.nbytes, C.byref(got))
        if rc != 0:
            raise RuntimeError(f"obx_gpu_fetch_proj failed: {rc}")
        assert got.value == n
        return out, nulls

    def fetch_proj_row_nos(self, handle, start=0, count=None):
        import numpy as np
        n = C.c_uint64(0)
        rc = self._lib.obx_gpu_fetch_proj_row_nos(
            self._ctx, handle, start, count if count is not None else 2**63,
            None, 0, C.byref(n))
        if rc != 0:
            raise RuntimeError(f"obx_gpu_fetch_proj_row_nos failed: {rc}")
        out = np.zeros(n.value, dtype=np.uint64)
        rc = self._lib.obx_gpu_fetch_proj_row_nos(
            self._ctx, handle, start, n.value,
            out.ctypes.data_as(C.c_void_p), out.size, C.byref(n))
        if rc != 0:
            raise RuntimeError(f"obx_gpu_fetch_proj_row_nos failed: {rc}")
        return out

    def last_proj_stage_ms(self):
        return tuple(float(self._lib.obx_gpu_last_proj_stage_ms(self._ctx, s))
                     for s in range(3))

    def scan_filter_agg(self, handle, filter_desc, agg_desc):
        res = abi.AggResult()
        rc = self._lib.obx_gpu_scan_filter_agg(
            self._ctx, handle,
            C.byref(filter_desc) if filter_desc is not None else None,
            C.byref(agg_desc) if agg_desc is not None else None,
            C.byref(res))
        if rc != 0:
            raise RuntimeError(f"obx_gpu_scan_filter_agg failed: {rc}")
        return res

    def scan_filter_agg_paged(self, handle, filter_desc, agg_desc):
        res = abi.AggResult()
        rc = self._lib.obx_gpu_scan_filter_agg(
            self._ctx, handle,
            C.byref(filter_desc) if filter_desc is not None else None,
            C.byref(agg_desc) if agg_desc is not None else None,
            C.byref(res))
        if rc not in (0, abi.OBX_BUF_NOT_ENOUGH):
            raise RuntimeError(f"obx_gpu_scan_filter_agg failed: {rc}")
        return res, self.agg_fetch_all(handle)

    def agg_fetch_all(self, handle, page=256):
        rows, start = [], 0
        buf = (abi.GroupRow * page)()
        n_out = C.c_uint32()
        total = C.c_uint64()
        while True:
            rc = self._lib.obx_gpu_agg_fetch(self._ctx, handle, start, page,
                                             buf, C.byref(n_out),
                                             C.byref(total))
            if rc != 0:
                raise RuntimeError(f"obx_gpu_agg_fetch failed: {rc}")
            for i in range(n_out.value):
                rows.append(abi.GroupRow.from_buffer_copy(buf[i]))
            start += n_out.value
            if start >= total.value or n_out.value == 0:
                break
        return rows

    def last_kernel_ms(self):
        return float(self._lib.obx_gpu_last_kernel_ms(self._ctx))

    def last_jit(self):
        return bool(self._lib.obx_gpu_last_jit(self._ctx))

    def last_prep_ms(self):
        return float(self._lib.obx_gpu_last_prep_ms(self._ctx))

    def total_bytes(self, handle):
        return int(self._lib.obx_gpu_total_bytes(self._ctx, handle))

    def total_rows(self, handle):
        return int(self._lib.obx_gpu_total_rows(self._ctx, handle))
```

Baseline: 247.7 billion rows/s.

## Pack row count into high bits of joint-sum LDS accumulator

Adds a packed joint-histogram form to the JIT scan kernel. The weighted value and a row count share one 64-bit LDS atomic, with the count held in the high bits above a computed shift. Histograms on the joint axes, the per-cell wcnt atomics and the w64 accumulators can then be dropped and rebuilt at flush time from the packed cells. The aim is fewer LDS atomics and less LDS per row, which may allow more workgroups per CU. In exchange the flush becomes more complex, and the form needs value-range and overflow checks; when those fail it falls back to the unpacked strategy.

```diff
diff --git a/include/obx.h b/include/obx.h
--- a/include/obx.h
+++ b/include/obx.h
@@ -237,6 +237,7 @@
 double obx_gpu_last_prep_ms(obx_gpu_ctx *ctx);
 int obx_gpu_last_jit(obx_gpu_ctx *ctx);
 int obx_gpu_last_bdesc(obx_gpu_ctx *ctx);
+int obx_gpu_last_joint(obx_gpu_ctx *ctx);
 int64_t obx_gpu_bdesc_builds(obx_gpu_ctx *ctx, int handle);
 uint32_t obx_gpu_last_grid(obx_gpu_ctx *ctx);
 uint64_t obx_gpu_total_rows(obx_gpu_ctx *ctx, int handle);
diff --git a/oceanbase_amd/csrc/obx_engine.cpp b/oceanbase_amd/csrc/obx_engine.cpp
--- a/oceanbase_amd/csrc/obx_engine.cpp
+++ b/oceanbase_amd/csrc/obx_engine.cpp
@@ -91,6 +91,12 @@
   }
   if (g > n_blocks) g = n_blocks;
   return g ? (uint32_t)g : 1;
+}
+
+static uint64_t jit_wg_rows(const obx_handle &h, uint32_t grid) {
+  if (!grid) grid = 1;
+  return (uint64_t)((h.n_blocks + grid - 1) / grid) *
+         (h.max_block_rows ? h.max_block_rows : 4096);
 }
 
 static void gtable_init(gslot *gt, uint32_t n_slots, uint32_t tail_words,
@@ -1218,6 +1224,7 @@
   ctx->last_jit = 0;
   ctx->last_grid = 0;
   ctx->last_bdesc = 0;
+  ctx->last_joint = 0;
   ctx->bdesc_built = false;
 }
 
@@ -1297,6 +1304,7 @@
       HIP_TRY(hipEventRecord(ctx->ev_b1, ctx->stream));
     }
     ctx->last_bdesc = bd != nullptr;
+    ctx->last_joint = je ? je->joint : 0;
     HIP_TRY(hipEventRecord(ctx->ev_start, ctx->stream));
     if (je) {
       if (jit_launch(je, h, bd, ctx->stream, &ctx->last_grid) != 0)
@@ -1578,6 +1586,10 @@
   return ctx ? ctx->last_bdesc : 0;
 }
 
+extern "C" int obx_gpu_last_joint(obx_gpu_ctx *ctx) {
+  return ctx ? ctx->last_joint : 0;
+}
+
 extern "C" int64_t obx_gpu_bdesc_builds(obx_gpu_ctx *ctx, int handle) {
   obx_handle *h = obx_handle_lookup(ctx, handle);
   return h ? (int64_t)h->bdesc_builds : -1;
diff --git a/oceanbase_amd/csrc/obx_host.h b/oceanbase_amd/csrc/obx_host.h
--- a/oceanbase_amd/csrc/obx_host.h
+++ b/oceanbase_amd/csrc/obx_host.h
@@ -257,6 +257,7 @@
   double last_prep_ms = 0.0;
   int last_jit = 0;
   int last_bdesc = 0;
+  int last_joint = 0;
   double last_proj_ms[3] = {0.0, 0.0, 0.0};
   uint32_t last_grid = 0;
   uint32_t n_cus = 256;
diff --git a/oceanbase_amd/csrc/obx_jit.inc b/oceanbase_amd/csrc/obx_jit.inc
--- a/oceanbase_amd/csrc/obx_jit.inc
+++ b/oceanbase_amd/csrc/obx_jit.inc
@@ -44,6 +44,7 @@
   int wpb = 0;
   bool bdesc = false;
   obx_bdesc_cols bd_cols = {};
+  int joint = 0;
 };
 
 struct jit_shape {
@@ -312,6 +313,7 @@
   if (je && c.kind == 2) {
     je->bdesc = c.st.bdesc != 0;
     je->bd_cols = c.st.bd_cols;
+    je->joint = jit_joint_form_of(c.st);
   }
   return je;
 }
diff --git a/oceanbase_amd/csrc/obx_jit_scan.inc b/oceanbase_amd/csrc/obx_jit_scan.inc
--- a/oceanbase_amd/csrc/obx_jit_scan.inc
+++ b/oceanbase_amd/csrc/obx_jit_scan.inc
@@ -69,6 +69,10 @@
   uint8_t jws_member[OBX_DEV_MAX_AGGS] = {};
   jit_agg_ids jws_f0;
   jit_agg_ids jws_f1;
+  uint8_t jws_pack = 0;
+  uint8_t jws_shift = 0;
+  jit_agg_ids jws_cax;
+  jit_agg_ids jws_ctab;
   int8_t ctab_agg = -1;
   uint32_t ctab_db = 0, ctab_dc = 0;
   uint32_t lds_bytes = 0;
@@ -125,11 +129,14 @@
   return st.n_hist++;
 }
 
-static bool jit_build_strategy(const obx_handle &h, const dev_plan_hdr &ph,
-                               const jit_shape &js, const dev_leaf *pl,
-                               jit_strategy &st) {
+enum { JB_OK = 0, JB_NO_V2 = 1, JB_PACK_REFUSED = 2 };
+
+static int jit_build_strategy_form(const obx_handle &h,
+                                   const dev_plan_hdr &ph,
+                                   const jit_shape &js, const dev_leaf *pl,
+                                   bool want_pack, jit_strategy &st) {
   const char *e = getenv("OBX_JIT_V2");
-  if (e && e[0] == '0') return false;
+  if (e && e[0] == '0') return JB_NO_V2;
   if (pl && ph.n_leaves >= 1 && ph.n_leaves <= 4) {
     st.leaf_inline = 1;
     for (uint32_t i = 0; i < ph.n_leaves; i++) {
@@ -165,7 +172,7 @@
     }
   }
   for (uint32_t g2 = 0; g2 < ph.n_group_cols; g2++)
-    if (!h.col_dict_stable[ph.need_cols[ph.group_idx[g2]]]) return false;
+    if (!h.col_dict_stable[ph.need_cols[ph.group_idx[g2]]]) return JB_NO_V2;
   auto maxabs_of = [&](uint8_t need_idx, uint64_t *out) -> bool {
     if (need_idx == 0xFF) return false;
     return jit_col_maxabs(h, ph.need_cols[need_idx], out);
@@ -181,7 +188,7 @@
         if (g.ia == 0xFF) { st.astrat[a] = JA_COUNT_STAR; break; }
         if (ja >= 0 && st.vmode[ja] == JV_REF) {
           int hid = jit_hist_get(st, (uint8_t)ja, st.vdim[ja]);
-          if (hid < 0) return false;
+          if (hid < 0) return JB_NO_V2;
           st.astrat[a] = JA_HCOUNT;
           st.ahist[a] = (int8_t)hid;
         } else if (ja >= 0 && !st.vext[ja]) {
@@ -191,18 +198,18 @@
           st.wa64[a] = (int8_t)st.n_w64++;
           st.aval_a[a] = (int8_t)ja;
         } else {
-          return false;
+          return JB_NO_V2;
         }
         break;
       case OBX_AGG_SUM:
-        if (ja < 0) return false;
+        if (ja < 0) return JB_NO_V2;
         if (st.vmode[ja] == JV_REF) {
           int hid = jit_hist_get(st, (uint8_t)ja, st.vdim[ja]);
-          if (hid < 0) return false;
+          if (hid < 0) return JB_NO_V2;
           st.astrat[a] = JA_HIST;
           st.ahist[a] = (int8_t)hid;
         } else {
-          if (!maxabs_of(g.ia, &ma)) return false;
+          if (!maxabs_of(g.ia, &ma)) return JB_NO_V2;
           if (ma > max_term) max_term = ma;
           st.astrat[a] = JA_I64;
           st.wa64[a] = (int8_t)st.n_w64++;
@@ -212,8 +219,8 @@
       case OBX_AGG_SUM_PROD2:
       case OBX_AGG_SUM_PROD3:
       case OBX_AGG_SUM_MUL: {
-        if (ja < 0 || jb < 0) return false;
-        if (!maxabs_of(g.ia, &ma) || !maxabs_of(g.ib, &mb)) return false;
+        if (ja < 0 || jb < 0) return JB_NO_V2;
+        if (!maxabs_of(g.ia, &ma) || !maxabs_of(g.ib, &mb)) return JB_NO_V2;
         uint64_t oneb = (uint64_t)(g.one_b < 0 ? -g.one_b : g.one_b);
         uint64_t onec = (uint64_t)(g.one_c < 0 ? -g.one_c : g.one_c);
         uint64_t term;
@@ -222,7 +229,7 @@
         } else {
           term = jit_sat_mul(ma, oneb + mb);
           if (g.kind == OBX_AGG_SUM_PROD3) {
-            if (jc < 0 || !maxabs_of(g.ic, &mc)) return false;
+            if (jc < 0 || !maxabs_of(g.ic, &mc)) return JB_NO_V2;
             term = jit_sat_mul(term, onec + mc);
           }
         }
@@ -232,33 +239,33 @@
         st.aval_a[a] = (int8_t)ja;
         if (st.vmode[ja] == JV_REF) {
           int t = jit_tab_get(st, (uint8_t)ja, 0, 0, st.vdim[ja]);
-          if (t < 0) return false;
+          if (t < 0) return JB_NO_V2;
           st.atab_a[a] = (int8_t)t;
         }
         if (st.vmode[jb] == JV_REF) {
           uint8_t kind = (g.kind == OBX_AGG_SUM_MUL) ? 0 : 1;
           int t = jit_tab_get(st, (uint8_t)jb, kind,
                               kind ? g.one_b : 0, st.vdim[jb]);
-          if (t < 0) return false;
+          if (t < 0) return JB_NO_V2;
           st.atab_b[a] = (int8_t)t;
         }
         if (g.kind == OBX_AGG_SUM_PROD3 && st.vmode[jc] == JV_REF) {
           int t = jit_tab_get(st, (uint8_t)jc, 2, g.one_c, st.vdim[jc]);
-          if (t < 0) return false;
+          if (t < 0) return JB_NO_V2;
           st.atab_c[a] = (int8_t)t;
         }
         break;
       }
       case OBX_AGG_MIN:
       case OBX_AGG_MAX:
-        if (ja < 0) return false;
+        if (ja < 0) return JB_NO_V2;
         if (st.vmode[ja] == JV_REF) {
           int hid = jit_hist_get(st, (uint8_t)ja, st.vdim[ja]);
-          if (hid < 0) return false;
+          if (hid < 0) return JB_NO_V2;
           st.astrat[a] = JA_HISTMM;
           st.ahist[a] = (int8_t)hid;
           int tt = jit_tab_get(st, (uint8_t)ja, 0, 0, st.vdim[ja]);
-          if (tt < 0) return false;
+          if (tt < 0) return JB_NO_V2;
           st.atab_a[a] = (int8_t)tt;
         } else {
           st.astrat[a] = JA_MM;
@@ -267,9 +274,9 @@
         }
         break;
       default:
-        return false;
-    }
-    if (st.n_w64 > 8 || st.n_mm > 8) return false;
+        return JB_NO_V2;
+    }
+    if (st.n_w64 > 8 || st.n_mm > 8) return JB_NO_V2;
   }
 
   for (uint32_t a = 0; a < ph.n_aggs; a++) {
@@ -278,7 +285,7 @@
     if (st.hist_tab[t2] < 0) {
       int tt = jit_tab_get(st, st.hist_vc[t2], 0, 0,
                            st.vdim[st.hist_vc[t2]]);
-      if (tt < 0) return false;
+      if (tt < 0) return JB_NO_V2;
       st.hist_tab[t2] = (int8_t)tt;
     }
   }
@@ -316,6 +323,15 @@
         else if (axes[0] != vc && axes[1] != vc) ok2 = false;
       }
       if (tb[0] >= 0 || tb[1] >= 0) n_axed++;
+    }
+    if (want_pack) {
+      bool pack_ok = allow && ok2 && wja >= 0 && !st.vext[wja];
+      if (pack_ok) {
+        const uint16_t wc = js.vcol[wja];
+        pack_ok = h.col_known[wc] && h.col_min[wc] >= 0 &&
+                  h.col_min[wc] <= h.col_max[wc];
+      }
+      if (!pack_ok) return JB_PACK_REFUSED;
     }
     if (allow && axes[1] >= 0) {
       auto adim = [&](int8_t vc) {
@@ -396,6 +412,44 @@
         st.n_w64 = nn;
       }
     }
+    if (want_pack && !st.jws_on) return JB_PACK_REFUSED;
+    if (want_pack) {
+      st.jws_pack = 1;
+      uint8_t old_vc[4];
+      int8_t old_tab[4], remap[4];
+      const int old_n = st.n_hist;
+      for (int t = 0; t < 4; t++) {
+        old_vc[t] = st.hist_vc[t];
+        old_tab[t] = st.hist_tab[t];
+        remap[t] = -1;
+      }
+      st.n_hist = 0;
+      st.hist_total = 0;
+      for (int t = 0; t < old_n; t++) {
+        if ((int8_t)old_vc[t] == st.jws_a0 || (int8_t)old_vc[t] == st.jws_a1)
+          continue;
+        remap[t] = (int8_t)st.n_hist;
+        st.hist_vc[st.n_hist] = old_vc[t];
+        st.hist_tab[st.n_hist] = old_tab[t];
+        st.hist_off[st.n_hist] = st.hist_total;
+        st.hist_total += st.jcells * st.vdim[old_vc[t]];
+        st.n_hist++;
+      }
+      for (int t = st.n_hist; t < 4; t++) {
+        st.hist_vc[t] = 0;
+        st.hist_tab[t] = 0;
+        st.hist_off[t] = 0;
+      }
+      for (uint32_t a = 0; a < ph.n_aggs; a++) {
+        const int t = st.ahist[a];
+        if (t < 0) continue;
+        st.ahist[a] = remap[t];
+        if (remap[t] >= 0) continue;
+        st.jws_cax[a] = (int8_t)old_vc[t] == st.jws_a0 ? 0 : 1;
+        st.jws_ctab[a] =
+            st.astrat[a] == JA_HISTMM ? st.atab_a[a] : old_tab[t];
+      }
+    }
   }
 
   {
@@ -464,7 +518,7 @@
         st.vdim[st.hist_vc[t]] < st.vdim[st.hist_vc[st.cnt_hist]])
       st.cnt_hist = (int8_t)t;
 
-  if (ph.n_leaves > 0 && !st.leaf_inline) return false;
+  if (ph.n_leaves > 0 && !st.leaf_inline) return JB_NO_V2;
 
   {
     const char *se = getenv("OBX_JIT_STRIPES");
@@ -486,7 +540,8 @@
   lds += 16 * 8 + 16 * 4;
   if (st.jws_on)
     lds += st.jws_cells * st.jws_d0 * st.jws_d1 * 8;
-  if (st.cnt_hist < 0) lds += st.jcells * 4 * st.stripes;
+  if (st.cnt_hist < 0 && !st.jws_pack)
+    lds += st.jcells * 4 * st.stripes;
   lds += 64;
   st.lds_bytes = lds;
   st.wpb = (int)(163840 / (lds > 1 ? lds : 1));
@@ -496,13 +551,21 @@
     int w = atoi(we);
     if (w >= 2 && w <= 8 && w < st.wpb) st.wpb = w;
   }
-  if (st.wpb < 2) return false;
+  if (st.wpb < 2) return JB_NO_V2;
   {
     const uint32_t grid = jit_grid_for(h.n_blocks, h.n_cus, st.wpb);
-    const uint64_t maxrows =
-        (uint64_t)((h.n_blocks + grid - 1) / grid) *
-        (h.max_block_rows ? h.max_block_rows : 4096);
-    if (jit_sat_mul(max_term, maxrows) >= BOUND) return false;
+    const uint64_t maxrows = jit_wg_rows(h, grid);
+    if (jit_sat_mul(max_term, maxrows) >= BOUND) return JB_NO_V2;
+    if (st.jws_pack) {
+      uint32_t cbits = 0;
+      while (cbits < 64 && (maxrows >> cbits)) cbits++;
+      if (cbits < 1 || cbits > 56) return JB_PACK_REFUSED;
+      const uint32_t sh = 64 - cbits;
+      const unsigned __int128 wsum =
+          (unsigned __int128)(uint64_t)h.col_max[js.vcol[st.jws_ja]] * maxrows;
+      if (wsum >= ((unsigned __int128)1 << sh)) return JB_PACK_REFUSED;
+      st.jws_shift = (uint8_t)sh;
+    }
   }
   {
     const char *be = getenv("OBX_JIT_BDESC");
@@ -525,7 +588,29 @@
     }
   }
   st.ok = true;
-  return true;
+  return JB_OK;
+}
+
+static bool jit_build_strategy(const obx_handle &h, const dev_plan_hdr &ph,
+                               const jit_shape &js, const dev_leaf *pl,
+                               jit_strategy &st) {
+  const char *pe = getenv("OBX_JIT_JPACK");
+  bool pack = !pe || pe[0] != '0';
+  for (;;) {
+    st = jit_strategy();
+    const int rc = jit_build_strategy_form(h, ph, js, pl, pack, st);
+    if (rc == JB_OK) return true;
+    if (rc != JB_PACK_REFUSED || !pack) break;
+    pack = false;
+  }
+  st = jit_strategy();
+  return false;
+}
+
+static int jit_joint_form_of(const jit_strategy &st) {
+  if (!st.jws_on) return 0;
+  if (!st.jws_pack) return 1;
+  return st.jws_a1 >= 0 ? 3 : 2;
 }
 
 static std::string jit_strategy_sig(const dev_plan_hdr &ph,
@@ -563,6 +648,11 @@
     for (uint32_t a = 0; a < ph.n_aggs; a++)
       jit_emit(k, "j%d:%d:%d|", st.jws_member[a], st.jws_f0[a],
                st.jws_f1[a]);
+    if (st.jws_pack) {
+      jit_emit(k, "P%u|", st.jws_shift);
+      for (uint32_t a = 0; a < ph.n_aggs; a++)
+        jit_emit(k, "p%d:%d|", st.jws_cax[a], st.jws_ctab[a]);
+    }
   }
   return k;
 }
@@ -702,10 +792,13 @@
 
 static void jit_v2_lds(const dev_plan_hdr &ph, const jit_shape &,
                        const jit_strategy &st, std::string &s) {
+  const bool has_w64 = st.n_w64 > 0 || !st.jws_pack;
+  const bool has_wcnt = st.cnt_hist < 0 && !st.jws_pack;
   s += "  __shared__ __attribute__((aligned(16))) uint8_t "
-       "lds_blk[JSTAGE];\n"
-       "  __shared__ unsigned long long wacc64[NW64][JC][NSTRIPE];\n"
-       "  __shared__ uint32_t hist[HTOT];\n";
+       "lds_blk[JSTAGE];\n";
+  if (has_w64)
+    s += "  __shared__ unsigned long long wacc64[NW64][JC][NSTRIPE];\n";
+  s += "  __shared__ uint32_t hist[HTOT];\n";
   if (st.n_mm > 0)
     jit_emit(s,
              "  /* CAS min/max cells: [slot][cell][val, valid] */\n"
@@ -716,7 +809,7 @@
   if (st.jws_on)
     jit_emit(s, "  __shared__ unsigned long long jws[%uu * %uu * %uu];\n",
              st.jws_cells, st.jws_d0, st.jws_d1);
-  if (st.cnt_hist < 0)
+  if (has_wcnt)
     s += "  __shared__ uint32_t wcnt[JC][NSTRIPE];\n";
   for (int t = 0; t < st.n_tab; t++)
     jit_emit(s, "  __shared__ long long vt%d[%u];\n", t, st.tabs[t].dim);
@@ -729,9 +822,10 @@
        "6;\n"
        "  uint32_t lane_cnt = 0;\n"
        "  const uint32_t stripe = lane & (NSTRIPE - 1);\n"
-       "\n"
-       "  for (uint32_t i = tid; i < NW64 * JC * NSTRIPE; i += WG)\n"
-       "    (&wacc64[0][0][0])[i] = 0;\n";
+       "\n";
+  if (has_w64)
+    s += "  for (uint32_t i = tid; i < NW64 * JC * NSTRIPE; i += WG)\n"
+         "    (&wacc64[0][0][0])[i] = 0;\n";
   for (uint32_t a = 0; a < ph.n_aggs; a++) {
     if (st.amm[a] < 0) continue;
     jit_emit(s,
@@ -748,7 +842,7 @@
              "  for (uint32_t i = tid; i < %uu * %uu * %uu; i += WG)\n"
              "    jws[i] = 0;\n",
              st.jws_cells, st.jws_d0, st.jws_d1);
-  if (st.cnt_hist < 0)
+  if (has_wcnt)
     s += "  for (uint32_t i = tid; i < JC * NSTRIPE; i += WG)\n"
          "    (&wcnt[0][0])[i] = 0;\n";
 }
@@ -1006,7 +1100,7 @@
                               const jit_strategy &st, std::string &s) {
   s += "        lane_cnt += live ? 1u : 0u;\n"
        "        if (live) {\n";
-  if (st.cnt_hist < 0)
+  if (st.cnt_hist < 0 && !st.jws_pack)
     s += "          atomicAdd(&wcnt[cell][stripe], 1u);\n";
   for (int t = 0; t < st.n_hist; t++) {
     const int j = st.hist_vc[t];
@@ -1024,11 +1118,18 @@
                       axis(st.jws_a1, st.jws_d1).c_str())
             : jit_fmt("cell * %uu + %s", st.jws_d0,
                       axis(st.jws_a0, st.jws_d0).c_str());
-    jit_emit(s,
-             "          if (!nu%1$d)\n"
-             "            atomicAdd(&jws[%2$s],\n"
-             "                      (unsigned long long)v%1$d);\n",
-             st.jws_ja, idx.c_str());
+    if (st.jws_pack)
+      jit_emit(s,
+               "          atomicAdd(&jws[%2$s],\n"
+               "                    (nu%1$d ? 0ull : (unsigned long long)v%1$d) +\n"
+               "                        (1ull << %3$u));\n",
+               st.jws_ja, idx.c_str(), (unsigned)st.jws_shift);
+    else
+      jit_emit(s,
+               "          if (!nu%1$d)\n"
+               "            atomicAdd(&jws[%2$s],\n"
+               "                      (unsigned long long)v%1$d);\n",
+               st.jws_ja, idx.c_str());
   }
   for (uint32_t a = 0; a < ph.n_aggs; a++) {
     const dev_agg &g = ph.aggs[a];
@@ -1241,6 +1342,12 @@
              "    for (uint32_t ref = 0; ref < %1$uu; ref++)\n"
              "      cnt2 += hist[%2$uu + cell * %1$uu + ref];\n",
              st.vdim[j], st.hist_off[st.cnt_hist]);
+  } else if (st.jws_pack) {
+    jit_emit(s,
+             "    unsigned long long cnt2 = 0;\n"
+             "    for (uint32_t j2 = 0; j2 < %1$uu; j2++)\n"
+             "      cnt2 += jws[cell * %1$uu + j2] >> %2$u;\n",
+             st.jws_d0 * st.jws_d1, (unsigned)st.jws_shift);
   } else {
     s += "    unsigned long long cnt2 = 0;\n"
          "    for (uint32_t s2 = 0; s2 < NSTRIPE; s2++)\n"
@@ -1348,9 +1455,156 @@
   }
 }
 
-static void jit_v2_flush_joint(const dev_plan_hdr &ph, const jit_shape &,
+static void jit_v2_emit_facc_i128(std::string &s, int pad,
+                                  const std::string &expr, uint32_t a) {
+  const std::string in(pad, ' ');
+  jit_emit(s,
+           "%1$s{\n"
+           "%1$s  __int128 p = %2$s;\n"
+           "%1$s  if (p != 0) {\n"
+           "%1$s    i128v pv = {(uint64_t)p,\n"
+           "%1$s                (uint64_t)((unsigned __int128)p >> 64)};\n"
+           "%1$s    lds_acc_i128(facc[cell][%3$u], pv);\n"
+           "%1$s  }\n"
+           "%1$s}\n",
+           in.c_str(), expr.c_str(), (unsigned)a);
+}
+
+static int jit_v2_joint_ctabs(const dev_plan_hdr &ph, const jit_strategy &st,
+                              int *c_tabs) {
+  int n_ct = 0;
+  for (uint32_t a = 0; a < ph.n_aggs; a++) {
+    if (!st.jws_member[a] || st.jws_f1[a] < 0) continue;
+    bool seen = false;
+    for (int q = 0; q < n_ct; q++) seen |= c_tabs[q] == st.jws_f1[a];
+    if (!seen) c_tabs[n_ct++] = st.jws_f1[a];
+  }
+  return n_ct;
+}
+
+static void jit_v2_emit_joint_members(const dev_plan_hdr &ph,
+                                      const jit_strategy &st,
+                                      std::string &s) {
+  for (uint32_t a = 0; a < ph.n_aggs; a++) {
+    if (!st.jws_member[a]) continue;
+    const int f0 = st.jws_f0[a], f1 = st.jws_f1[a];
+    const std::string sum = f1 >= 0 ? jit_fmt("s_c%d", f1) : "s_pl";
+    jit_v2_emit_facc_i128(
+        s, 6,
+        f0 >= 0   ? jit_fmt("(__int128)vt%d[d0] * %s", f0, sum.c_str())
+        : f1 >= 0 ? sum
+                  : "(__int128)s_pl",
+        a);
+  }
+}
+
+static void jit_v2_flush_joint_packed(const dev_plan_hdr &ph,
+                                      const jit_shape &js,
+                                      const jit_strategy &st,
+                                      std::string &s) {
+  bool ax[2] = {false, false};
+  for (uint32_t a = 0; a < ph.n_aggs; a++)
+    if (st.jws_cax[a] >= 0) ax[st.jws_cax[a]] = true;
+  s += "  {\n";
+  if (ax[0])
+    jit_emit(s, "    const uint32_t hc0 = b0.cols[%u].count;\n",
+             (unsigned)js.vcol[st.jws_a0]);
+  if (ax[1])
+    jit_emit(s, "    const uint32_t hc1 = b0.cols[%u].count;\n",
+             (unsigned)js.vcol[st.jws_a1]);
+  jit_emit(s,
+           "    for (uint32_t idx = tid; idx < fcells * %1$uu; idx += WG) {\n"
+           "      uint32_t cell = idx / %1$uu, d0 = idx %% %1$uu;\n"
+           "      int ce = cslot[cell];\n"
+           "      if (ce < 0) continue;\n"
+           "      long long s_pl = 0;\n"
+           "      unsigned long long n_pl = 0;\n",
+           st.jws_d0);
+  int c_tabs[OBX_DEV_MAX_AGGS];
+  const int n_ct = jit_v2_joint_ctabs(ph, st, c_tabs);
+  for (int q = 0; q < n_ct; q++)
+    jit_emit(s, "      __int128 s_c%d = 0;\n", c_tabs[q]);
+  for (uint32_t a = 0; a < ph.n_aggs; a++) {
+    if (st.jws_cax[a] != 1) continue;
+    if (st.astrat[a] == JA_HIST)
+      jit_emit(s, "      __int128 h1_%u = 0;\n", (unsigned)a);
+    else if (st.astrat[a] == JA_HCOUNT)
+      jit_emit(s, "      unsigned long long h1_%u = 0;\n", (unsigned)a);
+  }
+  jit_emit(s,
+           "      for (uint32_t d1 = 0; d1 < %1$uu; d1++) {\n"
+           "        const unsigned long long jc =\n"
+           "            jws[cell * %2$uu + d0 * %1$uu + d1];\n"
+           "        if (!jc) continue;\n"
+           "        const long long w = (long long)(jc & ((1ull << %3$u) - 1));\n"
+           "        const unsigned long long c = jc >> %3$u;\n"
+           "        s_pl += w;\n"
+           "        n_pl += c;\n",
+           st.jws_d1, st.jws_d0 * st.jws_d1, (unsigned)st.jws_shift);
+  for (int q = 0; q < n_ct; q++)
+    jit_emit(s, "        s_c%1$d += (__int128)vt%1$d[d1] * w;\n", c_tabs[q]);
+  if (ax[1]) {
+    s += "        if (d1 < hc1) { /* excl. null bucket */\n";
+    for (uint32_t a = 0; a < ph.n_aggs; a++) {
+      if (st.jws_cax[a] != 1) continue;
+      if (st.astrat[a] == JA_HIST)
+        jit_emit(s, "          h1_%u += (__int128)vt%d[d1] * (long long)c;\n",
+                 (unsigned)a, st.jws_ctab[a]);
+      else if (st.astrat[a] == JA_HCOUNT)
+        jit_emit(s, "          h1_%u += c;\n", (unsigned)a);
+      else
+        jit_emit(s,
+                 "          cas_minmax(&facc[cell][%1$u][0],\n"
+                 "                     (int64_t)vt%2$d[d1], %3$s);\n"
+                 "          facc[cell][%1$u][1] = 1;\n",
+                 (unsigned)a, st.jws_ctab[a], jit_v2_is_min(ph.aggs[a]));
+    }
+    s += "        }\n";
+  }
+  s += "      }\n"
+       "      if (!n_pl) continue;\n";
+  jit_v2_emit_joint_members(ph, st, s);
+  if (ax[0]) {
+    s += "      if (d0 < hc0) { /* excl. null bucket */\n";
+    for (uint32_t a = 0; a < ph.n_aggs; a++) {
+      if (st.jws_cax[a] != 0) continue;
+      if (st.astrat[a] == JA_HIST)
+        jit_v2_emit_facc_i128(
+            s, 8,
+            jit_fmt("(__int128)vt%d[d0] * (long long)n_pl", st.jws_ctab[a]),
+            a);
+      else if (st.astrat[a] == JA_HCOUNT)
+        jit_emit(s, "        atomicAdd(&facc[cell][%u][0], n_pl);\n",
+                 (unsigned)a);
+      else
+        jit_emit(s,
+                 "        cas_minmax(&facc[cell][%1$u][0],\n"
+                 "                   (int64_t)vt%2$d[d0], %3$s);\n"
+                 "        facc[cell][%1$u][1] = 1;\n",
+                 (unsigned)a, st.jws_ctab[a], jit_v2_is_min(ph.aggs[a]));
+    }
+    s += "      }\n";
+  }
+  for (uint32_t a = 0; a < ph.n_aggs; a++) {
+    if (st.jws_cax[a] != 1) continue;
+    if (st.astrat[a] == JA_HIST)
+      jit_v2_emit_facc_i128(s, 6, jit_fmt("h1_%u", (unsigned)a), a);
+    else if (st.astrat[a] == JA_HCOUNT)
+      jit_emit(s,
+               "      if (h1_%1$u) atomicAdd(&facc[cell][%1$u][0], h1_%1$u);\n",
+               (unsigned)a);
+  }
+  s += "    }\n"
+       "  }\n";
+}
+
+static void jit_v2_flush_joint(const dev_plan_hdr &ph, const jit_shape &js,
                                const jit_strategy &st, std::string &s) {
   if (!st.jws_on) return;
+  if (st.jws_pack) {
+    jit_v2_flush_joint_packed(ph, js, st, s);
+    return;
+  }
   jit_emit(s,
            "  for (uint32_t idx = tid; idx < fcells * %1$uu; idx += WG) "
            "{\n"
@@ -1359,13 +1613,8 @@
            "    if (ce < 0) continue;\n"
            "    long long s_pl = 0;\n",
            st.jws_d0);
-  int c_tabs[OBX_DEV_MAX_AGGS], n_ct = 0;
-  for (uint32_t a = 0; a < ph.n_aggs; a++) {
-    if (!st.jws_member[a] || st.jws_f1[a] < 0) continue;
-    bool seen = false;
-    for (int q = 0; q < n_ct; q++) seen |= c_tabs[q] == st.jws_f1[a];
-    if (!seen) c_tabs[n_ct++] = st.jws_f1[a];
-  }
+  int c_tabs[OBX_DEV_MAX_AGGS];
+  const int n_ct = jit_v2_joint_ctabs(ph, st, c_tabs);
   for (int q = 0; q < n_ct; q++)
     jit_emit(s, "    __int128 s_c%d = 0;\n", c_tabs[q]);
   jit_emit(s,
@@ -1381,26 +1630,7 @@
        "    if (s_pl";
   for (int q = 0; q < n_ct; q++) jit_emit(s, " || s_c%d != 0", c_tabs[q]);
   s += ") {\n";
-  for (uint32_t a = 0; a < ph.n_aggs; a++) {
-    if (!st.jws_member[a]) continue;
-    const int f0 = st.jws_f0[a], f1 = st.jws_f1[a];
-    const std::string sum = f1 >= 0 ? jit_fmt("s_c%d", f1) : "s_pl";
-    const std::string expr =
-        f0 >= 0   ? jit_fmt("(__int128)vt%d[d0] * %s", f0, sum.c_str())
-        : f1 >= 0 ? sum
-                  : "(__int128)s_pl";
-    jit_emit(s,
-             "      {\n"
-             "        __int128 p = %s;\n"
-             "        if (p != 0) {\n"
-             "          i128v pv = {(uint64_t)p,\n"
-             "                      (uint64_t)((unsigned __int128)p >> "
-             "64)};\n"
-             "          lds_acc_i128(facc[cell][%u], pv);\n"
-             "        }\n"
-             "      }\n",
-             expr.c_str(), (unsigned)a);
-  }
+  jit_v2_emit_joint_members(ph, st, s);
   s += "    }\n"
        "  }\n";
 }
diff --git a/oceanbase_amd/engine.py b/oceanbase_amd/engine.py
--- a/oceanbase_amd/engine.py
+++ b/oceanbase_amd/engine.py
@@ -78,6 +78,8 @@
     lib.obx_gpu_last_jit.argtypes = [C.c_void_p]
     lib.obx_gpu_last_bdesc.restype = C.c_int
     lib.obx_gpu_last_bdesc.argtypes = [C.c_void_p]
+    lib.obx_gpu_last_joint.restype = C.c_int
+    lib.obx_gpu_last_joint.argtypes = [C.c_void_p]
     lib.obx_gpu_bdesc_builds.restype = C.c_int64
     lib.obx_gpu_bdesc_builds.argtypes = [C.c_void_p, C.c_int]
     lib.obx_gpu_keyset_create.restype = C.c_int
@@ -480,6 +482,9 @@
     def last_jit(self):
         return bool(self._lib.obx_gpu_last_jit(self._ctx))
 
+    def last_joint(self):
+        return int(self._lib.obx_gpu_last_joint(self._ctx))
+
     def last_prep_ms(self):
         return float(self._lib.obx_gpu_last_prep_ms(self._ctx))
 
```

New measurement: 266.7 billion rows/s (median of 6 runs). +7.7%, better.
